# szcompressor/sz

Measured on AMD Instinct MI355X. Metric: compression GB/s (input), 512^3 float32 ABS 1e-4, higher is better.
Workload: dtype f32

## Files before the change

### include/szhip.h

```cpp
#ifndef SZHIP_H
#define SZHIP_H
#include <stddef.h>
#include <stdint.h>
#ifdef __cplusplus
extern "C" {
#endif

#define SZHIP_OK            0
#define SZHIP_ERR_NODEVICE -1
#define SZHIP_ERR_ARG      -2
#define SZHIP_ERR_UNSUP    -3
#define SZHIP_ERR_STREAM   -4
#define SZHIP_ERR_INTERNAL -5
#define SZHIP_CONSTANT      1

#define SZHIP_F32 0
#define SZHIP_F64 1

typedef struct szhip_ctx szhip_ctx;

typedef struct szhip_params {
    int      sample_distance;
    float    pred_threshold;
    unsigned max_quant_intervals;
    unsigned quantization_intervals;
    unsigned flags;
} szhip_params;
#define SZHIP_RANGE_FROM_DATA 1u

typedef struct szhip_stats {
    double ms_total;
    double ms_prequant;
    double ms_quant;
    double ms_entropy;
    double ms_host;
    uint64_t n_elements, n_blocks, n_reg_blocks, n_unpred;
    unsigned intervals; int use_mean;
    uint64_t out_bytes;
    uint64_t quant_kernel_launches;
    double vmin, vmax;
    int chain_overlapped;
    int quant_kernel;
    int packing;
    int book_on_device;
} szhip_stats;

int  szhip_create(szhip_ctx **ctx, int device);
typedef struct szhip_pool szhip_pool;
int  szhip_pool_create(szhip_pool **pool, int device, int lanes);
void szhip_pool_destroy(szhip_pool *pool);
int  szhip_pool_submit(szhip_pool *pool, int dtype, const void *data, int data_on_device, size_t r0, size_t r1, size_t r2, double eb,
                       const szhip_params *params, const unsigned char *meta, size_t meta_len, int out_on_device,
                       unsigned char *out_buf, size_t out_cap, int *ticket);
int  szhip_pool_wait(szhip_pool *pool, int ticket, unsigned char **out, size_t *out_size, szhip_stats *stats);

void szhip_destroy(szhip_ctx *ctx);
const char *szhip_last_error(szhip_ctx *ctx);

int szhip_stage_input(szhip_ctx *ctx, const void *host_data, size_t bytes, void **device_ptr);

int szhip_minmax(szhip_ctx *ctx, int dtype, const void *data, int data_on_device, size_t n, double *vmin, double *vmax);

int szhip_compress(szhip_ctx *ctx, int dtype, const void *data, int data_on_device,
                   size_t r0, size_t r1, size_t r2, double eb, const szhip_params *params,
                   const unsigned char *meta, size_t meta_len,
                   int out_on_device, unsigned char **out, size_t *out_size, szhip_stats *stats);

int szhip_decompress(szhip_ctx *ctx, int dtype, const unsigned char *stream, int stream_on_device, size_t stream_len,
                     size_t body_off, size_t r0, size_t r1, size_t r2,
                     void *out, int out_on_device, szhip_stats *stats);

int szhip_compress_sz14(szhip_ctx *ctx, int dtype, const void *data, int data_on_device,
                        size_t r0, size_t r1, size_t r2, double eb, double value_range, double median,
                        const szhip_params *params, const unsigned char *meta, size_t meta_len,
                        int out_on_device, unsigned char **out, size_t *out_size, szhip_stats *stats);
int szhip_decompress_sz14(szhip_ctx *ctx, int dtype, const unsigned char *stream, int stream_on_device, size_t stream_len,
                          size_t body_off, size_t r0, size_t r1, size_t r2, void *out, int out_on_device, szhip_stats *stats);

int szhip_compress_omp(szhip_ctx *ctx, int dtype, const void *data, int data_on_device, size_t r0, size_t r1, size_t r2, double eb,
                       int thread_num, const szhip_params *params, const unsigned char *meta, size_t meta_len,
                       int out_on_device, unsigned char **out, size_t *out_size, szhip_stats *stats);
int szhip_decompress_omp(szhip_ctx *ctx, int dtype, const unsigned char *stream, int stream_on_device, size_t stream_len,
                         size_t body_off, size_t r0, size_t r1, size_t r2, void *out, int out_on_device, szhip_stats *stats);

typedef struct szhip_pwr {
    uint64_t segment_size;
    const unsigned char *signs_blob;
    uint32_t signs_blob_size;
    double min_log_value;
    unsigned char rad_expo;
    unsigned char msst19;
    unsigned char plus_bits;
    double median_stored;
} szhip_pwr;
int szhip_pwr_prepare(szhip_ctx *ctx, int dtype, const void *data, int data_on_device, size_t n, double vmin, double vmax, double pwr_ratio,
                      void **d_log, unsigned char *signs_host, int *positive, double *real_precision, double *value_range, double *median,
                      double *min_log_value);
int szhip_msst_prepare(szhip_ctx *ctx, int dtype, const void *data, int data_on_device, size_t n, double vmax, double pwr_ratio,
                       void **d_prepared, unsigned char *signs_host, int *positive, double *near_zero, double *median_log, double *min_log_value);
int szhip_compress_sz14_pwr(szhip_ctx *ctx, int dtype, const void *data, int data_on_device,
                            size_t r0, size_t r1, size_t r2, double eb, double value_range, double median,
                            const szhip_params *params, const unsigned char *meta, size_t meta_len, const szhip_pwr *pwr,
                            int out_on_device, unsigned char **out, size_t *out_size, szhip_stats *stats);
int szhip_sz14_pwr_locate(int dtype, const unsigned char *stream, size_t stream_len, size_t body_off, size_t *blob_off, size_t *blob_size,
                          double *min_log_value);
int szhip_decompress_sz14_pwr(szhip_ctx *ctx, int dtype, const unsigned char *stream, int stream_on_device, size_t stream_len,
                              size_t body_off, size_t r0, size_t r1, size_t r2, const unsigned char *signs_host, void *out,
                              int out_on_device, szhip_stats *stats);

typedef struct szhip_book_record {
// ... 17 lines not shown
```

### sz_amd/api.py

```python
import ctypes
import os
import subprocess

import numpy as np

ABS, REL, VR_REL, ABS_AND_REL, ABS_OR_REL, PSNR, NORM, PW_REL = 0, 1, 1, 2, 3, 4, 5, 10
SZ_FLOAT, SZ_DOUBLE = 0, 1
SZ_BEST_SPEED, SZ_BEST_COMPRESSION, SZ_DEFAULT_COMPRESSION = 0, 1, 2
SZ_SCES, SZ_NSCS = 0, -1

_HERE = os.path.dirname(os.path.abspath(__file__))
_CSRC = os.path.join(_HERE, "csrc")


def lib_path():
    return os.environ.get("SZ_AMD_LIB") or os.path.join(_CSRC, "libszhip.so")


class SZError(RuntimeError):
    pass


class sz_params(ctypes.Structure):
    _fields_ = [("dataType", ctypes.c_int), ("max_quant_intervals", ctypes.c_uint),
# ... 29 lines not shown
class szhip_book_record(ctypes.Structure):
    _fields_ = [("n_nodes", ctypes.c_uint32), ("tree_bytes", ctypes.c_uint32), ("max_len", ctypes.c_uint32), ("status", ctypes.c_uint32),
                ("total_bits", ctypes.c_uint64), ("total_unpred", ctypes.c_uint64)]


class szhost_meta(ctypes.Structure):
    _fields_ = [("data_type", ctypes.c_int), ("err_mode", ctypes.c_int), ("abs_bound", ctypes.c_double),
                ("rel_ratio", ctypes.c_double), ("psnr", ctypes.c_double), ("pwr_ratio", ctypes.c_double), ("vmin", ctypes.c_double),
                ("vmax", ctypes.c_double), ("opt_quant_mode", ctypes.c_int), ("data_endian", ctypes.c_int),
                ("sz_mode", ctypes.c_int), ("gzip_mode", ctypes.c_int), ("sample_distance", ctypes.c_int),
                ("pred_threshold", ctypes.c_float), ("sol_id", ctypes.c_int), ("max_quant_intervals", ctypes.c_uint),
                ("quantization_intervals", ctypes.c_uint), ("protect_value_range", ctypes.c_int)]


def build_library(force=False):
    if force:
        subprocess.check_call(["make", "-s", "-C", _CSRC, "clean"])
    subprocess.check_call(["make", "-s", "-C", _CSRC])
    return lib_path()


_lib = None


def lib():
    global _lib
    if _lib is not None:
        return _lib
    p = lib_path()
    if not os.path.exists(p):
        raise SZError(f"{p} is missing: build it with `python -c 'import __graft_entry__ as g; g.build()'` "
                      "(hipcc --offload-arch=gfx950); there is no CPU fallback")
    _lib = _bind(ctypes.CDLL(p))
    return _lib


def _bind(L):
    sz = ctypes.c_size_t
    L.SZ_Init.argtypes = [ctypes.c_char_p]; L.SZ_Init.restype = ctypes.c_int
    L.SZ_Init_Params.argtypes = [ctypes.POINTER(sz_params)]; L.SZ_Init_Params.restype = ctypes.c_int
    L.SZ_Finalize.argtypes = []; L.SZ_Finalize.restype = None
    L.SZ_compress.argtypes = [ctypes.c_int, ctypes.c_void_p, ctypes.POINTER(sz)] + [sz] * 5
    L.SZ_compress.restype = ctypes.c_void_p
    L.SZ_compress_args.argtypes = [ctypes.c_int, ctypes.c_void_p, ctypes.POINTER(sz), ctypes.c_int,
                                   ctypes.c_double, ctypes.c_double, ctypes.c_double] + [sz] * 5
    L.SZ_compress_args.restype = ctypes.c_void_p
    L.SZ_decompress.argtypes = [ctypes.c_int, ctypes.c_void_p, sz] + [sz] * 5
    L.SZ_decompress.restype = ctypes.c_void_p
    L.SZ_hip_last_stats.argtypes = [ctypes.POINTER(szhip_stats)]; L.SZ_hip_last_stats.restype = ctypes.c_int
    L.SZ_hip_set_device.argtypes = [ctypes.c_int]
    L.szhip_create.argtypes = [ctypes.POINTER(ctypes.c_void_p), ctypes.c_int]; L.szhip_create.restype = ctypes.c_int
    L.szhip_destroy.argtypes = [ctypes.c_void_p]; L.szhip_destroy.restype = None
    L.szhip_last_error.argtypes = [ctypes.c_void_p]; L.szhip_last_error.restype = ctypes.c_char_p
    L.szhip_minmax.argtypes = [ctypes.c_void_p, ctypes.c_int, ctypes.c_void_p, ctypes.c_int, sz,
                               ctypes.POINTER(ctypes.c_double), ctypes.POINTER(ctypes.c_double)]
    L.szhip_minmax.restype = ctypes.c_int
    L.szhip_compress.argtypes = [ctypes.c_void_p, ctypes.c_int, ctypes.c_void_p, ctypes.c_int, sz, sz, sz, ctypes.c_double,
                                 ctypes.POINTER(szhip_params), ctypes.c_char_p, sz, ctypes.c_int,
                                 ctypes.POINTER(ctypes.c_void_p), ctypes.POINTER(sz), ctypes.POINTER(szhip_stats)]
    L.szhip_compress.restype = ctypes.c_int
    if hasattr(L, "szhip_pool_create"):
        L.szhip_pool_create.argtypes = [ctypes.POINTER(ctypes.c_void_p), ctypes.c_int, ctypes.c_int]; L.szhip_pool_create.restype = ctypes.c_int
        L.szhip_pool_destroy.argtypes = [ctypes.c_void_p]; L.szhip_pool_destroy.restype = None
        L.szhip_pool_submit.argtypes = [ctypes.c_void_p, ctypes.c_int, ctypes.c_void_p, ctypes.c_int, sz, sz, sz, ctypes.c_double,
                                        ctypes.POINTER(szhip_params), ctypes.c_char_p, sz, ctypes.c_int, ctypes.c_void_p, sz, ctypes.POINTER(ctypes.c_int)]
        L.szhip_pool_submit.restype = ctypes.c_int
        L.szhip_pool_wait.argtypes = [ctypes.c_void_p, ctypes.c_int, ctypes.POINTER(ctypes.c_void_p), ctypes.POINTER(sz), ctypes.POINTER(szhip_stats)]
        L.szhip_pool_wait.restype = ctypes.c_int
    L.szhip_decompress.argtypes = [ctypes.c_void_p, ctypes.c_int, ctypes.c_void_p, ctypes.c_int, sz, sz, sz, sz, sz,
                                   ctypes.c_void_p, ctypes.c_int, ctypes.POINTER(szhip_stats)]
    L.szhip_decompress.restype = ctypes.c_int
    L.szhip_compress_sz14.argtypes = [ctypes.c_void_p, ctypes.c_int, ctypes.c_void_p, ctypes.c_int, sz, sz, sz, ctypes.c_double,
                                      ctypes.c_double, ctypes.c_double, ctypes.POINTER(szhip_params), ctypes.c_char_p, sz, ctypes.c_int,
                                      ctypes.POINTER(ctypes.c_void_p), ctypes.POINTER(sz), ctypes.POINTER(szhip_stats)]
    L.szhip_compress_sz14.restype = ctypes.c_int
    L.szhip_decompress_sz14.argtypes = [ctypes.c_void_p, ctypes.c_int, ctypes.c_void_p, ctypes.c_int, sz, sz, sz, sz, sz,
                                        ctypes.c_void_p, ctypes.c_int, ctypes.POINTER(szhip_stats)]
    L.szhip_decompress_sz14.restype = ctypes.c_int
    L.szhip_debug_fetch.argtypes = [ctypes.c_void_p, ctypes.c_int, ctypes.c_void_p, sz]; L.szhip_debug_fetch.restype = ctypes.c_int
    if hasattr(L, "szhip_compress_omp"):
        L.szhip_compress_omp.argtypes = [ctypes.c_void_p, ctypes.c_int, ctypes.c_void_p, ctypes.c_int, sz, sz, sz, ctypes.c_double, ctypes.c_int,
                                         ctypes.POINTER(szhip_params), ctypes.c_char_p, sz, ctypes.c_int,
                                         ctypes.POINTER(ctypes.c_void_p), ctypes.POINTER(sz), ctypes.POINTER(szhip_stats)]
        L.szhip_compress_omp.restype = ctypes.c_int
        L.szhip_decompress_omp.argtypes = [ctypes.c_void_p, ctypes.c_int, ctypes.c_void_p, ctypes.c_int, sz, sz, sz, sz, sz,
                                           ctypes.c_void_p, ctypes.c_int, ctypes.POINTER(szhip_stats)]
        L.szhip_decompress_omp.restype = ctypes.c_int
    if hasattr(L, "szhip_huff_book"):
        L.szhip_huff_book.argtypes = [ctypes.c_void_p, ctypes.c_void_p, ctypes.c_uint, ctypes.c_void_p, sz, ctypes.c_void_p, ctypes.c_void_p,
                                      ctypes.POINTER(szhip_book_record)]
        L.szhip_huff_book.restype = ctypes.c_int
    L.szhost_write_meta.argtypes = [ctypes.POINTER(szhost_meta), ctypes.c_ubyte, ctypes.c_char_p]
    L.szhost_write_meta.restype = sz
    L.free.argtypes = [ctypes.c_void_p]
    return L


def _dims5(shape):
    d = list(shape)[::-1] + [0] * (5 - len(shape))
    return d[4], d[3], d[2], d[1], d[0]


def _dtype_code(a):
    if a.dtype == np.float32:
        return SZ_FLOAT
    if a.dtype == np.float64:
# ... 105 lines not shown
        if self._h:
            lib().szhip_pool_destroy(self._h)
            self._h = ctypes.c_void_p()

    def __del__(self):
        try:
            self.close()
        except Exception:
            pass

    def submit(self, ptr, on_device, shape3, dtype, eb, meta, params, out_ptr, out_cap):
        t = ctypes.c_int(-1)
        p = params or szhip_params(100, 0.99, 65536, 0)
        rc = lib().szhip_pool_submit(self._h, 0 if np.dtype(dtype) == np.float32 else 1, ptr, int(on_device), shape3[0], shape3[1], shape3[2], eb,
                                     ctypes.byref(p), meta, len(meta), 2, out_ptr, out_cap, ctypes.byref(t))
        if rc != 0:
            raise SZError(f"szhip_pool_submit failed ({rc})")
        self._keep[t.value] = (p, meta)
        return t.value

    def wait(self, ticket):
        out = ctypes.c_void_p(); n = ctypes.c_size_t(0); st = szhip_stats()
        rc = lib().szhip_pool_wait(self._h, ticket, ctypes.byref(out), ctypes.byref(n), ctypes.byref(st))
        self._keep.pop(ticket, None)
        if rc == 1:
            return 0, st
        if rc != 0:
            raise SZError(f"pooled szhip_compress failed ({rc})")
        return n.value, st


class HipContext:

    def __init__(self, device=0):
        self._h = ctypes.c_void_p()
        rc = lib().szhip_create(ctypes.byref(self._h), device)
        if rc != 0:
            raise SZError(f"szhip_create failed ({rc}): no usable HIP device; there is no CPU fallback")

    def close(self):
        if self._h:
            lib().szhip_destroy(self._h)
            self._h = ctypes.c_void_p()

    def __del__(self):
        try:
            self.close()
        except Exception:
            pass

    def _err(self, rc, what):
        raise SZError(f"{what} failed ({rc}): {lib().szhip_last_error(self._h).decode(errors='replace')}")

    def minmax(self, ptr, on_device, n, dtype):
        lo, hi = ctypes.c_double(), ctypes.c_double()
        rc = lib().szhip_minmax(self._h, 0 if np.dtype(dtype) == np.float32 else 1, ptr, int(on_device), n,
                                ctypes.byref(lo), ctypes.byref(hi))
        if rc:
            self._err(rc, "szhip_minmax")
        return lo.value, hi.value

    def compress(self, ptr, on_device, shape3, dtype, eb, meta, params=None, out_on_device=False):
        p = params or szhip_params(100, 0.99, 65536, 0)
        out = ctypes.c_void_p()
        n = ctypes.c_size_t(0)
        st = szhip_stats()
        rc = lib().szhip_compress(self._h, 0 if np.dtype(dtype) == np.float32 else 1, ptr, int(on_device), shape3[0], shape3[1],
                                  shape3[2], eb, ctypes.byref(p), meta, len(meta), int(out_on_device), ctypes.byref(out),
                                  ctypes.byref(n), ctypes.byref(st))
        if rc == 1:
            return None, 0, st
        if rc:
            self._err(rc, "szhip_compress")
        if out_on_device:
            return out.value, n.value, st
        b = ctypes.string_at(out.value, n.value)
        lib().free(out)
        return b, n.value, st

    def compress_omp(self, ptr, on_device, shape3, dtype, eb, thread_num, meta, params=None, out_on_device=False):
        p = params or szhip_params(100, 0.99, 65536, 0)
        out = ctypes.c_void_p()
        n = ctypes.c_size_t(0)
        st = szhip_stats()
        rc = lib().szhip_compress_omp(self._h, 0 if np.dtype(dtype) == np.float32 else 1, ptr, int(on_device), shape3[0], shape3[1], shape3[2],
                                      eb, thread_num, ctypes.byref(p), meta, len(meta), int(out_on_device), ctypes.byref(out), ctypes.byref(n),
                                      ctypes.byref(st))
        if rc:
            self._err(rc, "szhip_compress_omp")
        if out_on_device:
            return out.value, n.value, st
        b = ctypes.string_at(out.value, n.value)
        lib().free(out)
        return b, n.value, st

    def decompress_omp(self, stream_ptr, stream_on_device, stream_len, body_off, shape3, dtype, out_ptr, out_on_device):
        st = szhip_stats()
        rc = lib().szhip_decompress_omp(self._h, 0 if np.dtype(dtype) == np.float32 else 1, stream_ptr, int(stream_on_device), stream_len,
                                        body_off, shape3[0], shape3[1], shape3[2], out_ptr, int(out_on_device), ctypes.byref(st))
        if rc:
            self._err(rc, "szhip_decompress_omp")
        return st

    def huff_book(self, hist, on_device=False, intervals=None, tree_cap=None):
        if on_device:
            ptr, k = hist, int(intervals)
# ... 26 lines not shown
```

### sz_amd/csrc/szhip.hip

```cpp
#include <hip/hip_runtime.h>
#include <algorithm>
#include <array>
#include <cmath>
#include <cstdio>
#include <cstdlib>
#include <cstring>
#include <atomic>
#include <chrono>
#include <ctime>
#include <condition_variable>
#include <deque>
#include <functional>
#include <mutex>
#include <thread>
#include <vector>
#include "../../include/szhip.h"
#include "szhost.h"
#include "szhip_kernels.h"

namespace {

struct DevBuf { void *p = nullptr; size_t cap = 0; };

double now_ms()
// ... 62 lines not shown
    void arm() { { std::lock_guard<std::mutex> lk(m); if (phase.load() == 0) phase.store(1); } cv.notify_all(); }
    void disarm() { std::lock_guard<std::mutex> lk(m); if (phase.load() == 1) phase.store(0); }
    void submit(int ncoef, std::function<void(int)> c, std::function<void(int)> sec)
    {
        n = ncoef; chain = std::move(c); section = std::move(sec);
        stage1.store(0); stage2.store(0);
        arm();
        seq.fetch_add(1, std::memory_order_release);
    }
    void wait_chains() { while (stage1.load(std::memory_order_acquire) < n) pause(); }
    void wait_all() { while (stage2.load(std::memory_order_acquire) < 4) std::this_thread::yield(); }
    ~szhip_chain_pool()
    {
        { std::lock_guard<std::mutex> lk(m); phase.store(2); }
        cv.notify_all();
        for (auto &t : th) if (t.joinable()) t.join();
    }
};

constexpr int SZH_STAGE_T = 4;
struct szhip_ctx {
    int device = 0;
    int cus = 256;
    hipStream_t stream = nullptr;
    hipStream_t stream2 = nullptr;
    hipEvent_t ev_in = nullptr, ev_fit = nullptr, ev_feed = nullptr, ev_sec = nullptr;
    int settle_probes = 0, settle_rejected = 0;
    hipStream_t stream3 = nullptr;
    hipEvent_t ev_perm = nullptr;
    hipEvent_t ev[6] = {nullptr, nullptr, nullptr, nullptr, nullptr, nullptr};
    char err[512] = {0};
    unsigned epoch = 0;
    bool hdec_sync_rounds = false, hdec_unconverged = false;
    bool gate = false;
    unsigned long long *hdec_res = nullptr;
    DevBuf lor_bits, reg_flags, reg_rank, coef_compact, in, out, codes_nat, codes_blk, coef, blk_lor, faceI, faceJ, rb_down, rb_right, rb_vals, pt_flags, feed_word, progress, order, small, hist, col_zeros, col_zeros64,
        seg_bits, seg_zeros, seg_bitoff, seg_zoff, seg_hist, seg_tab, col_off, partial, samples, unpred, stream_buf, chunk_bits, chunk_off, code_tab, len_tab, dec_tab,
        starts, ends, counts, offs, dirty, zcnt, zpos, pwr_log, pwr_signs, pwr_small, coef_dec, msst_ptab, msst_cells, msst_rec, msst_pe, book_tree, book_rec, book_stage;
    void *pinned = nullptr; size_t pinned_cap = 0;
    void *pinned2 = nullptr; size_t pinned2_cap = 0;
    void *stage_buf[SZH_STAGE_T][2] = {};
    hipEvent_t stage_ev[SZH_STAGE_T][2] = {};
    void *pinned3 = nullptr; size_t pinned3_cap = 0;
    int streams_independent = -1;
    void *coh = nullptr; size_t coh_cap = 0;
    int order_nI = -1, order_nJ = -1;
    bool wave_timeout = false, ticket_atomic = false;
    bool coef_late = false, no_chain_overlap = false;
    bool book_declined = false, no_dev_book = false;
    unsigned long long *book_pin = nullptr;
    std::vector<int> chain_codes; std::vector<unsigned char> chain_unpred;
    unsigned char *sec_pin[4] = {nullptr, nullptr, nullptr, nullptr}; size_t sec_pin_cap[4] = {0, 0, 0, 0};
    szhip_chain_pool *chain_pool = nullptr;
};

namespace {

#include "szhip_rt.inc"
#include "szhip_sz21.inc"
#include "szhip_sz14.inc"
#include "szhip_pwr.inc"
#include "szhip_omp.inc"

}

template <class F>
static int with_ticket_fallback(szhip_ctx *ctx, F &&run)
{
    ctx->wave_timeout = false; ctx->hdec_unconverged = false; ctx->coef_late = false; ctx->book_declined = false;
    auto again = [&]() {
        if (ctx->stream3) hipStreamSynchronize(ctx->stream3); hipStreamSynchronize(ctx->stream2); hipStreamSynchronize(ctx->stream);
        return run();
    };
    int rc = run();
    if (rc == SZHIP_ERR_INTERNAL && ctx->book_declined && !ctx->no_dev_book) {
        ctx->no_dev_book = true; ctx->wave_timeout = false; rc = again(); ctx->no_dev_book = false;
    }
    if (rc == SZHIP_OK && !ctx->no_chain_overlap && tune_int("SZ_HIP_TEST_CHAIN_FALLBACK", 0)) { ctx->coef_late = true; rc = SZHIP_ERR_INTERNAL; }
    if (rc == SZHIP_ERR_INTERNAL && ctx->coef_late && !ctx->no_chain_overlap) {
        ctx->no_chain_overlap = true; ctx->wave_timeout = false; rc = again();
    }
    if (rc == SZHIP_ERR_INTERNAL && ctx->hdec_unconverged && !ctx->hdec_sync_rounds) {
        ctx->hdec_sync_rounds = true; ctx->wave_timeout = false; rc = again(); ctx->hdec_sync_rounds = false;
    }
    if (rc == SZHIP_OK && !ctx->ticket_atomic && tune_int("SZ_HIP_TEST_TICKET_FALLBACK", 0)) { ctx->wave_timeout = true; rc = SZHIP_ERR_INTERNAL; }
    if (rc == SZHIP_ERR_INTERNAL && ctx->wave_timeout && !ctx->ticket_atomic) {
        ctx->ticket_atomic = true; rc = again();
    }
    return rc;
}


extern "C" {


static int create_ctx(szhip_ctx **out, int device)
{
    if (!out) return SZHIP_ERR_ARG;
    int count = 0;
    hipError_t e = hipGetDeviceCount(&count);
    if (e != hipSuccess || count <= 0) {
        fprintf(stderr, "szhip: no HIP device available (%s); this library has no CPU fallback\n", hipGetErrorString(e));
        return SZHIP_ERR_NODEVICE;
    }
    if (device < 0 || device >= count) return SZHIP_ERR_ARG;
    szhip_ctx *ctx = new szhip_ctx();
    ctx->device = device;
    { int c = 0; if (hipDeviceGetAttribute(&c, hipDeviceAttributeMultiprocessorCount, device) == hipSuccess && c > 0) ctx->cus = c; }
    if (hipSetDevice(device) != hipSuccess || hipStreamCreateWithFlags(&ctx->stream, hipStreamNonBlocking) != hipSuccess) {
        delete ctx; return SZHIP_ERR_NODEVICE;
    }
    for (int i = 0; i < 6; ++i) if (hipEventCreate(&ctx->ev[i]) != hipSuccess) { delete ctx; return SZHIP_ERR_NODEVICE; }
    if (hipStreamCreateWithFlags(&ctx->stream2, hipStreamNonBlocking) != hipSuccess || hipEventCreateWithFlags(&ctx->ev_in, hipEventDisableTiming) != hipSuccess ||
        hipEventCreateWithFlags(&ctx->ev_fit, hipEventDisableTiming) != hipSuccess ||
        hipEventCreateWithFlags(&ctx->ev_feed, hipEventDisableTiming) != hipSuccess ||
        hipEventCreateWithFlags(&ctx->ev_sec, hipEventDisableTiming) != hipSuccess) { delete ctx; return SZHIP_ERR_NODEVICE; }
    *out = ctx;
    return SZHIP_OK;
}

int szhip_create(szhip_ctx **out, int device)
{
    const int rc = create_ctx(out, device);
    if (rc == SZHIP_OK) settle_streams(*out, nullptr, 0);
    return rc;
}

void szhip_destroy(szhip_ctx *ctx)
{
    if (!ctx) return;
    hipSetDevice(ctx->device);
    hipStreamSynchronize(ctx->stream);
    delete ctx->chain_pool; ctx->chain_pool = nullptr;
    DevBuf *bufs[] = {&ctx->lor_bits, &ctx->reg_flags, &ctx->reg_rank, &ctx->coef_compact, &ctx->in, &ctx->out, &ctx->codes_nat, &ctx->codes_blk, &ctx->coef, &ctx->blk_lor, &ctx->faceI, &ctx->faceJ, &ctx->rb_down, &ctx->rb_right, &ctx->rb_vals, &ctx->pt_flags, &ctx->feed_word, &ctx->progress,
                      &ctx->order, &ctx->small, &ctx->hist, &ctx->col_zeros, &ctx->col_zeros64, &ctx->seg_bits, &ctx->seg_zeros, &ctx->seg_bitoff, &ctx->seg_zoff, &ctx->seg_hist, &ctx->seg_tab, &ctx->col_off, &ctx->partial,
                      &ctx->samples, &ctx->unpred, &ctx->stream_buf, &ctx->chunk_bits, &ctx->chunk_off, &ctx->code_tab,
                      &ctx->len_tab, &ctx->dec_tab, &ctx->starts, &ctx->ends, &ctx->counts, &ctx->offs, &ctx->dirty, &ctx->zcnt, &ctx->zpos,
                      &ctx->pwr_log, &ctx->pwr_signs, &ctx->pwr_small, &ctx->coef_dec, &ctx->msst_ptab, &ctx->msst_cells, &ctx->msst_rec, &ctx->msst_pe, &ctx->book_tree, &ctx->book_rec, &ctx->book_stage};
    for (DevBuf *b : bufs) if (b->p) hipFree(b->p);
    if (ctx->pinned) hipHostFree(ctx->pinned);
    if (ctx->pinned2) hipHostFree(ctx->pinned2);
    if (ctx->pinned3) hipHostFree(ctx->pinned3);
    if (ctx->coh) hipHostFree(ctx->coh);
    if (ctx->hdec_res) hipHostFree(ctx->hdec_res);
    if (ctx->book_pin) hipHostFree(ctx->book_pin);
    for (int w = 0; w < SZH_STAGE_T; ++w) for (int k = 0; k < 2; ++k) { if (ctx->stage_buf[w][k]) hipHostFree(ctx->stage_buf[w][k]); if (ctx->stage_ev[w][k]) hipEventDestroy(ctx->stage_ev[w][k]); }
    for (int i = 0; i < 6; ++i) if (ctx->ev[i]) hipEventDestroy(ctx->ev[i]);
    if (ctx->ev_in) hipEventDestroy(ctx->ev_in);
    if (ctx->ev_fit) hipEventDestroy(ctx->ev_fit);
    if (ctx->ev_feed) hipEventDestroy(ctx->ev_feed);
    if (ctx->ev_sec) hipEventDestroy(ctx->ev_sec);
    for (int e = 0; e < 4; ++e) if (ctx->sec_pin[e]) hipHostFree(ctx->sec_pin[e]);
    if (ctx->stream2) hipStreamDestroy(ctx->stream2);
    if (ctx->stream3) hipStreamDestroy(ctx->stream3);
    if (ctx->ev_perm) hipEventDestroy(ctx->ev_perm);
    if (ctx->stream) hipStreamDestroy(ctx->stream);
    delete ctx;
}

const char *szhip_last_error(szhip_ctx *ctx) { return ctx ? ctx->err : "no context"; }

struct szhip_pool_job {
    int dtype; const void *data; int on_dev; size_t r0, r1, r2; double eb; szhip_params prm; const unsigned char *meta; size_t meta_len;
    int out_on_device; unsigned char *out; size_t out_size; szhip_stats stats; int rc; bool done;
};
struct szhip_pool {
    std::vector<szhip_ctx *> ctx;
    std::vector<std::thread> workers;
    std::mutex mu;
    std::condition_variable cv_work, cv_done;
    std::deque<int> queue;
    std::vector<szhip_pool_job> jobs;
    std::vector<bool> used;
    bool stop = false;
};
static void szhip_pool_worker(szhip_pool *p, int lane)
{
    for (;;) {
        int t;
        {
            std::unique_lock<std::mutex> lk(p->mu);
            p->cv_work.wait(lk, [&] { return p->stop || !p->queue.empty(); });
            if (p->queue.empty()) return;
            t = p->queue.front(); p->queue.pop_front();
        }
        szhip_pool_job &j = p->jobs[t];
        j.rc = szhip_compress(p->ctx[lane], j.dtype, j.data, j.on_dev, j.r0, j.r1, j.r2, j.eb, &j.prm, j.meta, j.meta_len, j.out_on_device,
                              &j.out, &j.out_size, &j.stats);
        { std::lock_guard<std::mutex> lk(p->mu); j.done = true; }
        p->cv_done.notify_all();
    }
}
int szhip_pool_create(szhip_pool **out, int device, int lanes)
{
    if (!out || lanes < 1 || lanes > 16) return SZHIP_ERR_ARG;
    szhip_pool *p = new szhip_pool();
    for (int i = 0; i < lanes; ++i) {
        szhip_ctx *c = nullptr;
        const int rc = create_ctx(&c, device);
        if (rc != SZHIP_OK) { for (szhip_ctx *x : p->ctx) szhip_destroy(x); delete p; return rc; }
        c->gate = lanes > 1;
        { std::vector<hipStream_t> mains; for (szhip_ctx *x : p->ctx) { mains.push_back(x->stream); mains.push_back(x->stream2); } settle_streams(c, mains.data(), (int)mains.size(), lanes == 1); }
        p->ctx.push_back(c);
    }
    p->jobs.resize(64); p->used.assign(64, false);
    for (int i = 0; i < lanes; ++i) p->workers.emplace_back(szhip_pool_worker, p, i);
    *out = p;
    return SZHIP_OK;
}
void szhip_pool_destroy(szhip_pool *p)
{
    if (!p) return;
    { std::lock_guard<std::mutex> lk(p->mu); p->stop = true; }
// ... 268 lines not shown
```

### sz_amd/csrc/szhip_kernels.h

```cpp
#pragma once
#include <hip/hip_runtime.h>
#include "szh_core.h"
#include "szh_pencil.h"
#include "szh_bufio.h"

typedef unsigned long long u64;

#ifdef SZH_HIPSIM
#define SZH_DYN_SMEM(name) char *name = hipsim_dyn_smem()
#else
#define SZH_DYN_SMEM(name) extern __shared__ __attribute__((aligned(16))) char name[]
#endif

__device__ __forceinline__ u64 ord_enc(float v)
{
    unsigned u = __float_as_uint(v);
    u = (u & 0x80000000u) ? ~u : (u | 0x80000000u);
    return (u64)u;
}
__device__ __forceinline__ u64 ord_enc(double v)
{
    u64 u = (u64)__double_as_longlong(v);
    u = (u & 0x8000000000000000ull) ? ~u : (u | 0x8000000000000000ull);
    return u;
// ... 210 lines not shown
            if (I < a.nI && J < a.nJ) szh_pencil_run<T, DEC, B, MS>(a, I, J, L);
        } else if (w == NP) szh_tile_store<T, B>(a, TI, TJ, L);
        else szh_tile_fill<T, B>(a, TI, TJ, L);
        if (!a.persist) break;
    }
}

template <class T> struct GlobAcc {
    const T *p; int64_t d0, d1;
    __device__ T operator()(int i, int j, int k) const { return p[i * d0 + j * d1 + k]; }
    __device__ T operator()(int j, int k) const { return p[j * d1 + k]; }
};

template <class T>
__global__ __launch_bounds__(256) void k_fit_select(szh_geom3 G, const T *__restrict__ data, T *coef, uint8_t *blk_lor,
                                                    T noise, int use_mean, T mean, u64 *minmax)
{
    __shared__ u64 red[8];
    const int lane = threadIdx.x & 63, wid = threadIdx.x >> 6;
    const int64_t b = (int64_t)blockIdx.x * 256 + threadIdx.x;
    u64 lmin = ~0ull, lmax = 0ull;
    if (b < G.nblocks) {
        const int nb2 = G.g2.num, nb1 = G.g1.num;
        const int b2 = (int)(b % nb2);
        const int64_t c = b / nb2;
        const int b1 = (int)(c % nb1), b0 = (int)(c / nb1);
        const int s0 = szh_blk_size(G.g0, b0), s1 = szh_blk_size(G.g1, b1), s2 = szh_blk_size(G.g2, b2);
        const GlobAcc<T> A{data + (int64_t)szh_blk_start(G.g0, b0) * G.d0 + (int64_t)szh_blk_start(G.g1, b1) * G.d1 + szh_blk_start(G.g2, b2),
                           G.d0, G.d1};
        T c4[4];
        auto range = [&](T v) { const u64 oe = ord_enc(v); const bool num = v == v; lmin = num && oe < lmin ? oe : lmin; lmax = num && oe > lmax ? oe : lmax; };
        int reg;
        if (G.ndim == 2) {
            c4[0] = 0;
            szh_fit_block_2d<T>(A, s1, s2, c4 + 1, range);
            reg = szh_select_block_2d<T>(A, s1, s2, c4 + 1, noise);
        } else {
            szh_fit_block<T>(A, s0, s1, s2, c4, range);
            reg = szh_select_block<T>(A, s0, s1, s2, c4, noise, use_mean, mean);
        }
        for (int e = 0; e < 4; ++e) coef[(int64_t)e * G.nblocks + b] = c4[e];
        blk_lor[b] = reg ? 0 : 1;
    }
    lmin = wave_min_u64(lmin); lmax = wave_max_u64(lmax);
    if (lane == 0) { red[wid] = lmin; red[4 + wid] = lmax; }
    __syncthreads();
    if (threadIdx.x == 0) {
        u64 mn = red[0], mx = red[4];
        for (int w = 1; w < 4; ++w) { mn = red[w] < mn ? red[w] : mn; mx = red[4 + w] > mx ? red[4 + w] : mx; }
        atomicMin(&minmax[0], mn); atomicMax(&minmax[1], mx);
    }
}

template <class T>
__global__ __launch_bounds__(256) void k_minmax(const T *__restrict__ data, int64_t n, u64 *minmax)
{
    __shared__ u64 red[8];
    u64 lmin = ~0ull, lmax = 0ull;
    for (int64_t i = (int64_t)blockIdx.x * 256 + threadIdx.x; i < n; i += (int64_t)gridDim.x * 256) {
        const T v = data[i]; const u64 e = ord_enc(v); const bool num = v == v;
        lmin = num && e < lmin ? e : lmin; lmax = num && e > lmax ? e : lmax;
    }
    lmin = wave_min_u64(lmin); lmax = wave_max_u64(lmax);
    if ((threadIdx.x & 63) == 0) { red[threadIdx.x >> 6] = lmin; red[4 + (threadIdx.x >> 6)] = lmax; }
    __syncthreads();
    if (threadIdx.x == 0) {
        u64 mn = red[0], mx = red[4];
        for (int w = 1; w < 4; ++w) { mn = red[w] < mn ? red[w] : mn; mx = red[4 + w] > mx ? red[4 + w] : mx; }
        atomicMin(&minmax[0], mn); atomicMax(&minmax[1], mx);
    }
}

template <class T>
__global__ __launch_bounds__(256) void k_gather_mean(const T *__restrict__ data, szh_meanwalk w, int64_t count, T *out)
{
    const int64_t m = (int64_t)blockIdx.x * 256 + threadIdx.x;
    if (m < count) out[m] = data[szh_meanwalk_pos(w, m)];
}

#define SZH_LDS_RADIUS_BINS 4096
template <class T, bool FREQ>
__global__ __launch_bounds__(256) void k_sample(szh_geom3 G, const T *__restrict__ data, int64_t nrows, int sd, double ebD, T mean,
                                                unsigned max_radius, unsigned *radius_hist, unsigned *freq_hist, u64 *within)
{
    __shared__ unsigned sh_r[SZH_LDS_RADIUS_BINS];
    __shared__ unsigned sh_f[FREQ ? 8192 : 1];
    for (int i = threadIdx.x; i < SZH_LDS_RADIUS_BINS; i += 256) sh_r[i] = 0;
    if (FREQ) for (int i = threadIdx.x; i < 8192; i += 256) sh_f[i] = 0;
    __syncthreads();
    const int64_t rpp = G.g1.count - 1, r2 = G.g2.count;
    const bool two_d = G.ndim == 2;
    unsigned w = 0;
    for (int64_t ridx = (int64_t)blockIdx.x * 256 + threadIdx.x; ridx < nrows; ridx += (int64_t)gridDim.x * 256) {
        const int64_t n1 = two_d ? 0 : ridx / rpp + 1, n2 = two_d ? ridx + 1 : ridx - (n1 - 1) * rpp + 1;
        const int64_t c0 = two_d ? szh_sample_col0_2d(n2, sd) : sd - ((n1 + n2) % sd);
        const int64_t origin = n1 * G.d0 + n2 * r2;
        for (int64_t m = 0;; ++m) {
            const int64_t col = c0 + m * sd;
            if (m > 0 && col >= r2) break;
            const int64_t pos = origin + col;
            if (pos >= G.n) break;
            unsigned ri; int fi, we;
            szh_sample_point<T>(data, pos, r2, two_d ? 0 : G.d0, ebD, mean, max_radius, &ri, &fi, &we);
            if (ri < SZH_LDS_RADIUS_BINS) atomicAdd(&sh_r[ri], 1u); else atomicAdd(&radius_hist[ri], 1u);
            if (FREQ) atomicAdd(&sh_f[fi], 1u);
            w += (unsigned)we;
// ... 1152 lines not shown
```

### sz_amd/csrc/szhip_rt.inc

```

#define HIPCHK(call)                                                                                   \
    do {                                                                                               \
        hipError_t e_ = (call);                                                                        \
        if (e_ != hipSuccess) {                                                                        \
            snprintf(ctx->err, sizeof(ctx->err), "%s failed: %s (%s:%d)", #call, hipGetErrorString(e_), __FILE__, __LINE__); \
            fprintf(stderr, "szhip: %s\n", ctx->err);                                                  \
            return SZHIP_ERR_NODEVICE;                                                                 \
        }                                                                                              \
    } while (0)

#define FAIL(code, ...)                                                                                \
    do {                                                                                               \
        snprintf(ctx->err, sizeof(ctx->err), __VA_ARGS__);                                             \
        fprintf(stderr, "szhip: %s\n", ctx->err);                                                      \
        return (code);                                                                                 \
    } while (0)
#define FAIL_PUBLISHED(code, ...)                                                                      \
    do {                                                                                               \
        if (!out_on_device && out && *out) { free(*out); *out = nullptr; }                              \
        if (out_size) *out_size = 0;                                                                   \
        FAIL(code, __VA_ARGS__);                                                                       \
    } while (0)

int ensure(szhip_ctx *ctx, DevBuf &b, size_t bytes, bool zero_new = false)
{
    if (bytes == 0) bytes = 16;
    if (b.cap >= bytes) return SZHIP_OK;
    if (b.p) { HIPCHK(hipStreamSynchronize(ctx->stream)); HIPCHK(hipFree(b.p)); b.p = nullptr; b.cap = 0; }
    size_t cap = bytes + bytes / 8 + 256;
    HIPCHK(hipMalloc(&b.p, cap));
    b.cap = cap;
    if (zero_new) HIPCHK(hipMemsetAsync(b.p, 0, cap, ctx->stream));
    return SZHIP_OK;
}

#define TRY(x) do { int rc_ = (x); if (rc_ != SZHIP_OK) return rc_; } while (0)

int ensure_host(szhip_ctx *ctx, void *&p, size_t &have, size_t bytes, hipStream_t user, unsigned flags = hipHostMallocDefault)
{
    if (have >= bytes) return SZHIP_OK;
    if (p) { HIPCHK(hipStreamSynchronize(user)); HIPCHK(hipHostFree(p)); p = nullptr; have = 0; }
    size_t cap = bytes + bytes / 4 + 4096;
    HIPCHK(hipHostMalloc(&p, cap, flags));
    have = cap;
    return SZHIP_OK;
}
int ensure_pinned(szhip_ctx *ctx, size_t bytes) { return ensure_host(ctx, ctx->pinned, ctx->pinned_cap, bytes, ctx->stream); }
int ensure_pinned2(szhip_ctx *ctx, size_t bytes) { return ensure_host(ctx, ctx->pinned2, ctx->pinned2_cap, bytes, ctx->stream2); }
int ensure_pinned3(szhip_ctx *ctx, size_t bytes) { return ensure_host(ctx, ctx->pinned3, ctx->pinned3_cap, bytes, ctx->stream); }
int ensure_coherent(szhip_ctx *ctx, size_t bytes)
{
    const size_t had = ctx->coh_cap;
    TRY(ensure_host(ctx, ctx->coh, ctx->coh_cap, bytes, ctx->stream, hipHostMallocCoherent | hipHostMallocMapped));
    if (ctx->coh_cap != had) memset(ctx->coh, 0, ctx->coh_cap);
    return SZHIP_OK;
}

enum { SM_MINMAX = 0, SM_WITHIN = 2, SM_MEANCNT = 3, SM_TOTAL_UNPRED = 4, SM_TOTAL_BITS = 5, SM_TICKET = 6, SM_ERR = 7,
       SM_CHANGED = 8, SM_MEANSUM = 9, SM_TOTAL_SYM = 10, SM_NREG = 11, SM_SCRATCH = 12, SM_COUNT = 16 };

int probe_streams(szhip_ctx *ctx)
{
    if (ctx->streams_independent >= 0) return SZHIP_OK;
    TRY(ensure_coherent(ctx, 256));
    TRY(ensure(ctx, ctx->small, SM_COUNT * 8));
    volatile unsigned long long *flag = (volatile unsigned long long *)((char *)ctx->coh + 128);
    unsigned long long *src = (unsigned long long *)((char *)ctx->coh + 192);
    *flag = 0; *src = 1;
    HIPCHK(hipStreamSynchronize(ctx->stream)); HIPCHK(hipStreamSynchronize(ctx->stream2));
    u64 *sm = (u64 *)ctx->small.p;
    hipLaunchKernelGGL(k_probe_wait, dim3(1), dim3(1), 0, ctx->stream, (const unsigned long long *)flag, (unsigned long long *)(sm + SM_SCRATCH));
    HIPCHK(hipGetLastError());
    HIPCHK(hipMemcpyAsync(sm + SM_SCRATCH + 1, src, 8, hipMemcpyHostToDevice, ctx->stream2));
    const double t0 = now_ms();
    HIPCHK(hipStreamSynchronize(ctx->stream2));
    const double waited = now_ms() - t0;
    *flag = 1;
    HIPCHK(hipStreamSynchronize(ctx->stream));
    ctx->streams_independent = waited < 2.0 ? 1 : 0;
    return SZHIP_OK;
}

static int probe_pair(szhip_ctx *ctx, hipStream_t a, hipStream_t b, int *shared)
{
    TRY(ensure_coherent(ctx, 256));
    TRY(ensure(ctx, ctx->small, SM_COUNT * 8));
    volatile unsigned long long *flag = (volatile unsigned long long *)((char *)ctx->coh + 128);
    *flag = 0;
    HIPCHK(hipStreamSynchronize(a)); HIPCHK(hipStreamSynchronize(b));
    u64 *sm = (u64 *)ctx->small.p;
    hipLaunchKernelGGL(k_probe_wait, dim3(1), dim3(1), 0, a, (const unsigned long long *)flag, (unsigned long long *)(sm + SM_SCRATCH));
    HIPCHK(hipGetLastError());
    hipLaunchKernelGGL(k_probe_touch, dim3(1), dim3(1), 0, b, (unsigned long long *)(sm + SM_SCRATCH + 1));
    HIPCHK(hipGetLastError());
// ... 62 lines not shown
    HIPCHK(hipStreamSynchronize(st));
    const size_t nchunks = (bytes + chunk - 1) / chunk;
    std::atomic<int> failed(0);
    const int device = ctx->device;
    auto worker = [&](int w) {
        if (hipSetDevice(device) != hipSuccess) { failed = 1; return; }
        size_t pend_off[2] = {0, 0}, pend_len[2] = {0, 0};
        bool pend[2] = {false, false};
        int k = 0;
        for (size_t c = (size_t)w; c < nchunks && !failed; c += (size_t)nthr, k ^= 1) {
            const size_t off = c * chunk, len = std::min(chunk, bytes - off);
            if (to_device) {
                if (pend[k] && hipEventSynchronize(ctx->stage_ev[w][k]) != hipSuccess) { failed = 1; return; }
                memcpy(ctx->stage_buf[w][k], (const char *)src + off, len);
                if (hipMemcpyAsync((char *)dst + off, ctx->stage_buf[w][k], len, hipMemcpyHostToDevice, st) != hipSuccess ||
                    hipEventRecord(ctx->stage_ev[w][k], st) != hipSuccess) { failed = 1; return; }
                pend[k] = true;
            } else {
                if (pend[k]) {
                    if (hipEventSynchronize(ctx->stage_ev[w][k]) != hipSuccess) { failed = 1; return; }
                    memcpy((char *)dst + pend_off[k], ctx->stage_buf[w][k], pend_len[k]);
                }
                if (hipMemcpyAsync(ctx->stage_buf[w][k], (const char *)src + off, len, hipMemcpyDeviceToHost, st) != hipSuccess ||
                    hipEventRecord(ctx->stage_ev[w][k], st) != hipSuccess) { failed = 1; return; }
                pend[k] = true; pend_off[k] = off; pend_len[k] = len;
            }
        }
        for (int q = 0; q < 2; ++q, k ^= 1) {
            if (!pend[k]) continue;
            if (hipEventSynchronize(ctx->stage_ev[w][k]) != hipSuccess) { failed = 1; return; }
            if (!to_device) memcpy((char *)dst + pend_off[k], ctx->stage_buf[w][k], pend_len[k]);
        }
    };
    std::vector<std::thread> th;
    for (int w = 1; w < nthr; ++w) th.emplace_back(worker, w);
    worker(0);
    for (auto &t : th) t.join();
    if (failed) FAIL(SZHIP_ERR_NODEVICE, "staged %s copy failed", to_device ? "host-to-device" : "device-to-host");
    return SZHIP_OK;
}

int tune_int(const char *name, int def)
{
    const char *e = getenv(name);
    return e ? atoi(e) : def;
}

int scan_u64(szhip_ctx *ctx, const u64 *in, int64_t n, u64 *out, u64 *total_dev, hipStream_t on = nullptr)
{
    const hipStream_t sst = on ? on : ctx->stream;
    const int64_t nblk = (n + SZH_SCAN_TILE - 1) / SZH_SCAN_TILE;
    TRY(ensure(ctx, ctx->partial, (size_t)(nblk + 1) * 8));
    u64 *partial = (u64 *)ctx->partial.p;
    hipLaunchKernelGGL(k_scan_partials, dim3((unsigned)nblk), dim3(256), 0, sst, in, n, partial);
    hipLaunchKernelGGL(k_scan_single, dim3(1), dim3(256), 0, sst, partial, nblk, total_dev);
    hipLaunchKernelGGL(k_scan_final, dim3((unsigned)nblk), dim3(256), 0, sst, in, n, (const u64 *)partial, out);
    HIPCHK(hipGetLastError());
    return SZHIP_OK;
}

constexpr size_t SZH_PERM_TILE_BYTES = 32 * 1024;
int choose_segb(const szh_geom3 &G, size_t elem, size_t budget)
{
    const size_t rows = (size_t)G.g0.early * G.g1.early;
    size_t per_block = rows * (size_t)G.g2.early * elem;
    int segb = (int)(budget / (per_block ? per_block : 1));
    if (segb < 1) segb = 1;
    if (segb > 32) segb = 32;
    if (segb > G.g2.num) segb = G.g2.num;
    return segb;
}
size_t tile_bytes(const szh_geom3 &G, int segb, size_t elem)
{
    const size_t rows = (size_t)G.g0.early * G.g1.early;
    const size_t kp = ((size_t)segb * G.g2.early + 31) & ~(size_t)7;
    return rows * kp * elem + 16;
}

int prepare_pencil(szhip_ctx *ctx, const szh_geom3 &G, int nw, int tpi, int tpj, int *nI_out, int *nJ_out, int *ntiles_out)
{
    const int nI = (G.g0.count + 7) / 8, nJ = (G.g1.count + 7) / 8;
    if (nI > 65535 || nJ > 65535) FAIL(SZHIP_ERR_UNSUP, "dimension too large for the pencil grid");
    const size_t rowg = (size_t)G.g2.count * nw * sizeof(u64);
    TRY(ensure(ctx, ctx->faceI, (size_t)nI * nJ * 9 * rowg + 64, true));
    TRY(ensure(ctx, ctx->faceJ, (size_t)nI * nJ * 8 * rowg + 64, true));
    TRY(ensure(ctx, ctx->progress, (size_t)nI * nJ * 2 * sizeof(u64), true));
    const int nTI = (nI + tpi - 1) / tpi, nTJ = (nJ + tpj - 1) / tpj;
    if (ctx->order_nI != nTI || ctx->order_nJ != nTJ) {
        std::vector<unsigned> ord((size_t)nTI * nTJ);
        szh_fill_pencil_order(nTI, nTJ, ord.data());
        TRY(ensure(ctx, ctx->order, ord.size() * 4));
        HIPCHK(hipMemcpyAsync(ctx->order.p, ord.data(), ord.size() * 4, hipMemcpyHostToDevice, ctx->stream));
        HIPCHK(hipStreamSynchronize(ctx->stream));
        ctx->order_nI = nTI; ctx->order_nJ = nTJ;
    }
    *nI_out = nI; *nJ_out = nJ; *ntiles_out = nTI * nTJ;
    return SZHIP_OK;
}

constexpr int SZH_FILL_BACKOFF = 4;
template <class T> static int pencil_wide(const szh_geom3 &G, int nJ)
{
    using TS = szh_tile_shape<T>;
    return (double)TS::TPI * nJ * 9.0 * (double)G.g2.count * szh_gran<T>::NW * 8.0 < 4.0e9 && (double)TS::TPJ * 9.0 * (double)G.g2.count * szh_gran<T>::NW * 8.0 < 4.0e9;
}
template <class QA> static unsigned pencil_grid(szhip_ctx *ctx, QA &a, int ntiles)
{
    const int cap = ctx->gate ? 512 : 0;
    a.persist = cap > 0 && cap < ntiles;
    return (unsigned)(a.persist ? cap : ntiles);
}
template <class T> bool beam_applies(const szh_geom3 &G, const void *base, size_t reg_count)
{
    if (!tune_int("SZ_HIP_BEAM", 1)) return false;
    (void)reg_count;
    if (G.ndim != 3) return false;
    if (G.g2.count < 4 || (G.g2.count & 3) != 0 || ((uintptr_t)base & 15) != 0) return false;
    if ((double)G.n * sizeof(T) >= 4.0e9) return false;
    const szh_bm::grid_t g = szh_bm::make_grid(G);
    if (g.nKB > 65535 || g.nJG > 65535) return false;
    return (double)szh_bm::kface_words<T>(G) * 8.0 < 4.0e9 && (double)szh_bm::jface_words<T>(G) * 8.0 < 4.0e9;
}
template <class T, bool DEC>
int launch_beam(szhip_ctx *ctx, const szh_geom3 &G, szh_qargs<T> a, hipStream_t st, size_t reg_count, bool feed = false)
{
    const szh_bm::grid_t g = szh_bm::make_grid(G);
    const size_t tiles = (size_t)g.nKB * g.nJG;
    TRY(ensure(ctx, ctx->rb_down, szh_bm::kface_words<T>(G) * sizeof(u64) + 64, true));
    TRY(ensure(ctx, ctx->rb_right, szh_bm::jface_words<T>(G) * sizeof(u64) + 64, true));
    a.faceI = (szh_u64 *)ctx->rb_down.p; a.faceJ = (szh_u64 *)ctx->rb_right.p;
    a.nI = g.nKB; a.nJ = g.nJG;
    if (a.ticket_mode == 2) a.ticket_mode = 1;
    if (ctx->gate) a.ticket_mode = 0;
#ifdef SZH_SYNC_LAUNCH
    const unsigned wgs = (unsigned)tiles;
#else
    const int per_cu = sizeof(T) == 4 ? 2 : 1;
    const unsigned wgs = (unsigned)std::min<size_t>(tiles, (size_t)ctx->cus * per_cu);
#endif
    const bool hasreg = reg_count != 0;
    if (hasreg) {
        TRY(ensure(ctx, ctx->pt_flags, (size_t)G.n + 64));
#ifdef SZH_SYNC_LAUNCH
        const bool prepared = feed;
#else
        const bool prepared = false;
#endif
        if (!prepared) HIPCHK(hipMemsetAsync(ctx->pt_flags.p, 0, (size_t)G.n, st));
        a.ptflags = (const uint8_t *)ctx->pt_flags.p;
        const unsigned rgrid = (unsigned)(G.g0.num * G.g1.num);
        if (!DEC) {
            TRY(ensure(ctx, ctx->rb_vals, (size_t)G.n * sizeof(T) + 64));
            a.xr = (const T *)ctx->rb_vals.p;
            if (feed) {
                TRY(ensure(ctx, ctx->feed_word, 256));
                if (!prepared) HIPCHK(hipMemsetAsync(ctx->feed_word.p, 0, 256, st));
                a.reg_ready = (const unsigned *)ctx->feed_word.p;
                HIPCHK(hipEventRecord(ctx->ev_feed, st));
                HIPCHK(hipStreamWaitEvent(ctx->stream2, ctx->ev_feed, 0));
            } else
            hipLaunchKernelGGL((k_reg_points<T, 0>), dim3(rgrid), dim3(256), 0, st, G, a.blk_lor, a.coef, a.coef_stride, a.data, (T *)ctx->rb_vals.p, a.codes, (uint8_t *)ctx->pt_flags.p,
                               a.eb, a.recip, a.cap, a.radius, 0);
        } else
            hipLaunchKernelGGL((k_reg_points<T, 2>), dim3(rgrid), dim3(256), 0, st, G, a.blk_lor, a.coef, a.coef_stride, (const T *)nullptr, a.out, a.codes, (uint8_t *)ctx->pt_flags.p,
                               a.eb, a.recip, a.cap, a.radius, 0);
        HIPCHK(hipGetLastError());
    }
    const dim3 grid(wgs), block(szh_bm::WPG * 64);
    if (hasreg) {
        if (a.use_mean) hipLaunchKernelGGL((k_beam<T, DEC, true, true>), grid, block, 0, st, a);
        else hipLaunchKernelGGL((k_beam<T, DEC, false, true>), grid, block, 0, st, a);
    } else {
        if (a.use_mean) hipLaunchKernelGGL((k_beam<T, DEC, true, false>), grid, block, 0, st, a);
        else hipLaunchKernelGGL((k_beam<T, DEC, false, false>), grid, block, 0, st, a);
    }
    HIPCHK(hipGetLastError());
    return SZHIP_OK;
}

template <class T>
int feed_beam_slice(szhip_ctx *ctx, const szh_geom3 &G, const szh_qargs<T> &a, hipStream_t s2, const T *hcoef, size_t reg_count, size_t r_lo, size_t r_hi,
                    int b0_lo, int b0_hi, int planes_end, const u64 *reg_rank, int64_t nb)
{
    if (r_hi > r_lo)
        for (int e = 0; e < 4; ++e)
            HIPCHK(hipMemcpyAsync((T *)ctx->coef_compact.p + (size_t)e * reg_count + r_lo, hcoef + (size_t)e * reg_count + r_lo, (r_hi - r_lo) * sizeof(T), hipMemcpyHostToDevice, s2));
    const int64_t blk_lo = (int64_t)b0_lo * G.g1.num * G.g2.num, blk_hi = std::min<int64_t>(nb, (int64_t)b0_hi * G.g1.num * G.g2.num);
    if (r_hi > r_lo && blk_hi > blk_lo) {
        hipLaunchKernelGGL((k_move_coef<T, 1>), dim3((unsigned)((nb + 255) / 256)), dim3(256), 0, s2, a.blk_lor, reg_rank, nb, (int64_t)reg_count, (T *)a.coef, (T *)ctx->coef_compact.p);
        hipLaunchKernelGGL((k_reg_points<T, 0>), dim3((unsigned)((b0_hi - b0_lo) * G.g1.num)), dim3(256), 0, s2, G, a.blk_lor, a.coef, a.coef_stride, a.data, (T *)ctx->rb_vals.p,
                           a.codes, (uint8_t *)ctx->pt_flags.p, a.eb, a.recip, a.cap, a.radius, b0_lo);
    }
    hipLaunchKernelGGL(k_store_u32, dim3(1), dim3(1), 0, s2, (unsigned *)ctx->feed_word.p, (unsigned)planes_end);
    HIPCHK(hipGetLastError());
    return SZHIP_OK;
}

template <class T> double ord_dec(u64 e);
template <> double ord_dec<float>(u64 e)
{
    unsigned u = (unsigned)e;
    u = (u & 0x80000000u) ? (u & 0x7fffffffu) : ~u;
    float f; memcpy(&f, &u, 4); return (double)f;
}
template <> double ord_dec<double>(u64 e)
{
    u64 u = (e & 0x8000000000000000ull) ? (e & 0x7fffffffffffffffull) : ~e;
    double d; memcpy(&d, &u, 8); return d;
}

template <class T>
int minmax_impl(szhip_ctx *ctx, const void *data, int on_dev, size_t n, double *vmin, double *vmax)
{
    const T *d_in = (const T *)data;
    if (!on_dev) {
        TRY(ensure(ctx, ctx->in, n * sizeof(T)));
        HIPCHK(hipMemcpyAsync(ctx->in.p, data, n * sizeof(T), hipMemcpyHostToDevice, ctx->stream));
        d_in = (const T *)ctx->in.p;
    }
    TRY(ensure(ctx, ctx->small, SM_COUNT * 8));
    u64 *sm = (u64 *)ctx->small.p;
    u64 init[2] = {~0ull, 0ull};
    HIPCHK(hipMemcpyAsync(sm + SM_MINMAX, init, 16, hipMemcpyHostToDevice, ctx->stream));
    int grid = (int)std::min<int64_t>(((int64_t)n + 255) / 256, 2048);
    hipLaunchKernelGGL((k_minmax<T>), dim3(grid), dim3(256), 0, ctx->stream, d_in, (int64_t)n, sm + SM_MINMAX);
    HIPCHK(hipGetLastError());
    u64 res[2];
    HIPCHK(hipMemcpyAsync(res, sm + SM_MINMAX, 16, hipMemcpyDeviceToHost, ctx->stream));
    HIPCHK(hipStreamSynchronize(ctx->stream));
    *vmin = ord_dec<T>(res[0]); *vmax = ord_dec<T>(res[1]);
    return SZHIP_OK;
}
```

### sz_amd/csrc/szhip_sz21.inc

```
static bool book_declines(unsigned rec_status, unsigned long long plan_status, int test_switch) { return rec_status != 0 || plan_status != 0 || test_switch != 0; }

static int hist_rshift(unsigned intervals, size_t cap_bins) { int r = 0; while (r < 6 && ((size_t)intervals << (r + 1)) <= cap_bins) ++r; return r; }

struct sz21_plan {
    bool use_beam = false;
    bool segenc = false;
    bool seghist = false;
    bool dev_book = false;
    bool sliced = false;
    int slices_req = 1;
    int se_vw = 1, se_segb = 0, se_nseg = 0, se_nrmax = szh_se::NR; size_t se_tile = 0;
    int sh_rshift = 0;
    bool revise(unsigned enc_maxlen) { if (!segenc || enc_maxlen <= 32) return false; segenc = false; seghist = false; return true; }
};
template <class T>
sz21_plan sz21_make_plan(const szhip_ctx *ctx, const szh_geom3 &G, unsigned intervals, size_t reg_count, bool beam_ok, bool overlap, bool feed, size_t meta_len)
{
    sz21_plan P;
    const int64_t n = G.n;
    P.use_beam = !overlap && beam_ok;
    const int segenc_sw = tune_int("SZ_HIP_SEGENC", 1);
    P.segenc = G.ndim == 3 && segenc_sw != 0 && (!feed || segenc_sw == 2);
    P.se_vw = (G.g2.count % 8) == 0 ? 8 : ((G.g2.count % 4) == 0 ? 4 : 1);
    if (P.segenc) {
        bool ok = intervals < 65536 && (double)n < 4.0e9;
        if ((int64_t)G.g0.late * G.g1.late * G.g2.late < 32) ok = false;
        const size_t fixed = ((size_t)intervals + 1) * 8 + 16 + szh_se::seg_window_words(G, 32) * 4 + 64;
        const size_t lds_cap = (size_t)63 * 1024, want = (size_t)std::max(4, tune_int("SZ_HIP_SEG_TILE_KB", 14)) * 1024;
        if (ok && fixed + szh_se::seg_tile_bytes(G, 1, P.se_vw) > lds_cap) ok = false;
        if (ok) {
            const size_t budget = std::min(lds_cap - fixed, std::max(want, szh_se::seg_tile_bytes(G, 1, P.se_vw)));
            int sb = 1;
            while (sb < G.g2.num && szh_se::seg_tile_bytes(G, sb + 1, P.se_vw) <= budget && szh_se::seg_pieces_per_thread(G, sb + 1, P.se_vw) <= (size_t)szh_se::PF) ++sb;
            sb = (G.g2.num + (G.g2.num + sb - 1) / sb - 1) / ((G.g2.num + sb - 1) / sb);
            if (const int f = tune_int("SZ_HIP_SEG_SEGB", 0)) sb = std::max(1, std::min(f, sb));
            P.se_segb = sb;
            P.se_nseg = (G.g2.num + sb - 1) / sb;
            P.se_tile = szh_se::seg_tile_bytes(G, sb, P.se_vw);
            const int rows_typ = (2 * G.g0.split > G.g0.num ? G.g0.early : G.g0.late) * (2 * G.g1.split > G.g1.num ? G.g1.early : G.g1.late);
            const int runs_typ = std::max(1, sb * rows_typ), rounds_typ = (runs_typ + 256 * szh_se::NR - 1) / (256 * szh_se::NR);
            P.se_nrmax = std::max(1, std::min(szh_se::NR, (runs_typ + 256 * rounds_typ - 1) / (256 * rounds_typ)));
            if ((double)G.g0.num * G.g1.num >= 2.0e9) ok = false;
        }
        P.segenc = ok;
    }
    P.seghist = P.segenc && intervals <= SZH_COL_HBINS && tune_int("SZ_HIP_SEGHIST", 1) != 0;
    if (P.seghist) P.sh_rshift = hist_rshift(intervals, 4096);
    P.dev_book = P.segenc && reg_count == 0 && !ctx->no_dev_book && tune_int("SZ_HIP_DEV_BOOK", 0) != 0 && G.g0.num * G.g1.num <= 1024 * SZH_COL_SCAN_PER &&
                 tune_int("SZ_HIP_SEG_SCAN1", 1) != 0 && meta_len + 8 + 4 + sizeof(T) + 1 + sizeof(T) <= 3072;
    P.slices_req = tune_int("SZ_HIP_SLICES", ctx->gate ? tune_int("SZ_HIP_SLICES_POOL", 2) : 4);
    P.sliced = P.use_beam && P.slices_req > 1 && !P.seghist;
    return P;
}

template <class T>
struct sz21_call {
    static constexpr int is_double = sizeof(T) == 8;
    static constexpr int64_t LINE = 128 / (int64_t)sizeof(T);
    szhip_ctx *const ctx; const szhip_params *const prm; const unsigned char *meta; const size_t meta_len; const int out_on_device; unsigned char **const out; size_t *const out_size;
    const double eb_in; const T eb; const hipStream_t st;
    const bool two_d;
    const szh_geom3 G; const int ncoef, ncols; const int64_t n, nb;
    const double t_begin = now_ms(); double host_ms = 0;
    const int tp_on = tune_int("SZ_HIP_TIMING", 0); double tp_t[32]; const char *tp_n[32]; int tp_k = 0;
    szhip_stats S;
    const T *d_in = nullptr; u64 *sm = nullptr; T *d_coef = nullptr; uint8_t *d_lor = nullptr; uint16_t *d_nat = nullptr, *d_blk = nullptr; unsigned *d_hist = nullptr, *h_hist = nullptr;
    T noise = 0; bool fit_tile = false; int ft_nseg = 0;
    size_t ind_bytes = 0; unsigned char *ind_bits = nullptr; u64 *nreg_h = nullptr, *minmax_h = nullptr;
    unsigned intervals = 0; int use_mean = 0; T mean = 0; size_t reg_count = 0;
    std::vector<unsigned char> meta_own;
    sz21_plan P;
    unsigned *tile_done = nullptr; size_t beam_words = 0;
    int perm_segb = 1, perm_nseg = 1; size_t perm_lds = 0;
    std::vector<szh_se::seg_t> se_segs; std::vector<u64> tab_code; std::vector<uint8_t> tab_len;
    unsigned enc_maxlen = 0; bool enc32 = false; size_t lds_e32 = 0;
    unsigned char *hdr = nullptr; size_t pre_len = 0, sections_total = 0, hdr_len = 0, unpred_bytes = 0, total_len = 0; u64 total_bits = 0, total_unpred = 0;
    u64 h_small[SM_COUNT];
    bool synced = false;
    szhost_coeffs cf;
    size_t sec_len[4] = {0, 0, 0, 0};
    std::vector<std::thread> section_threads;
    std::atomic<int> section_failed{0};
    std::vector<unsigned char> all_reg_keep;
    std::vector<uint32_t> blk_of_rank;
    size_t chain_done[4] = {0, 0, 0, 0};
    size_t chain_avail = 0;
    double chain_t0[4] = {0, 0, 0, 0}, chain_t1[4] = {0, 0, 0, 0};
    bool overlap = false, feed = false, two_pieces = false;
    fed_call_guard fed_guard;
    T *hcoef = nullptr;
    bool pool_busy = false;
    bool cf_own = false;
    sz21_call(szhip_ctx *c, size_t r0, size_t r1, size_t r2, double eb_, const szhip_params *p, const unsigned char *m, size_t ml, int ood, unsigned char **o, size_t *os)
        : ctx(c), prm(p), meta(m), meta_len(ml), out_on_device(ood), out(o), out_size(os), eb_in(eb_), eb((T)eb_), st(c->stream), two_d(r0 == 0),
          G(r0 == 0 ? szh_make_geom2((int)r1, (int)r2) : szh_make_geom3((int)r0, (int)r1, (int)r2)), ncoef(r0 == 0 ? 3 : 4), ncols(G.g0.num * G.g1.num), n(G.n), nb(G.nblocks)
    {
        memset(&S, 0, sizeof(S)); memset(&cf, 0, sizeof(cf));
        S.n_elements = (uint64_t)n; S.n_blocks = (uint64_t)nb;
    }
    ~sz21_call() {
        join_sections();
        if (ctx->chain_pool) ctx->chain_pool->disarm();
        if (cf_own) for (int e = 0; e < 4; ++e) { cf.codes[e] = nullptr; cf.unpred[e] = nullptr; }
        szhost_coeffs_free(&cf);
    }
    void join_sections() {
        for (auto &x : section_threads) if (x.joinable()) x.join();
        if (pool_busy && ctx->chain_pool) { ctx->chain_pool->wait_all(); pool_busy = false; }
    }
    void TP(const char *nm) { if (tp_on && tp_k < 32) { tp_t[tp_k] = now_ms() - t_begin; tp_n[tp_k++] = nm; } }
    void print_trace() const { if (tp_on) { for (int i = 0; i < tp_k; ++i) fprintf(stderr, "%s %.2f | ", tp_n[i], tp_t[i]); fprintf(stderr, "\n"); } }
    bool is_lorenzo(int64_t bb) const { return (ind_bits[bb >> 3] >> (7 - (bb & 7))) & 1; }
    size_t count_lorenzo(int64_t bb, int64_t b_end) const {
        size_t ones = 0;
        for (; bb < b_end && (bb & 7); ++bb) ones += is_lorenzo(bb);
        for (; bb + 64 <= b_end; bb += 64) { uint64_t w8; memcpy(&w8, ind_bits + (bb >> 3), 8); ones += (size_t)__builtin_popcountll(w8); }
        for (; bb < b_end; ++bb) ones += is_lorenzo(bb);
        return ones;
    }
    size_t chains_done() const {
        size_t p = reg_count;
        for (int e = 0; e < ncoef; ++e) { const size_t d = __atomic_load_n(&chain_done[e], __ATOMIC_ACQUIRE); if (d < p) p = d; }
        return p;
    }
    int launch_fit(hipStream_t s_, int um, T mn) {
        if (fit_tile) hipLaunchKernelGGL((k_fit_tile<T>), dim3((unsigned)((int64_t)ncols * ft_nseg)), dim3(64), 0, s_, G, d_in, d_coef, d_lor, noise, um, mn, sm + SM_MINMAX, ft_nseg);
        else hipLaunchKernelGGL((k_fit_select<T>), dim3((unsigned)((nb + 255) / 256)), dim3(256), 0, s_, G, d_in, d_coef, d_lor, noise, um, mn, sm + SM_MINMAX);
        HIPCHK(hipGetLastError());
        return SZHIP_OK;
    }
    int launch_pack_lor(hipStream_t s_) {
        hipLaunchKernelGGL(k_pack_lor, dim3((unsigned)((ind_bytes + 255) / 256)), dim3(256), 0, s_, (const uint8_t *)d_lor, nb, (uint8_t *)ctx->lor_bits.p, sm + SM_NREG);
        HIPCHK(hipGetLastError());
        HIPCHK(hipMemcpyAsync(ind_bits, ctx->lor_bits.p, ind_bytes, hipMemcpyDeviceToHost, s_));
        HIPCHK(hipMemcpyAsync(nreg_h, sm + SM_NREG, 8, hipMemcpyDeviceToHost, s_));
        return SZHIP_OK;
    }
    int stage_and_fit(const void *data, int data_on_device) {
        d_in = (const T *)data;
        if (!data_on_device) {
            TRY(ensure(ctx, ctx->in, (size_t)n * sizeof(T)));
            TRY(staged_copy(ctx, ctx->in.p, data, (size_t)n * sizeof(T), true));
            d_in = (const T *)ctx->in.p;
        }
        TRY(ensure(ctx, ctx->small, SM_COUNT * 8));
        sm = (u64 *)ctx->small.p;
        HIPCHK(hipMemsetAsync(sm, 0, SM_COUNT * 8, st));
        static const u64 minmax_init[2] = {~0ull, 0ull};
        HIPCHK(hipMemcpyAsync(sm + SM_MINMAX, minmax_init, 16, hipMemcpyHostToDevice, st));
        TRY(ensure(ctx, ctx->coef, (size_t)nb * 4 * sizeof(T)));
        TRY(ensure(ctx, ctx->blk_lor, (size_t)nb));
        d_coef = (T *)ctx->coef.p;
        d_lor = (uint8_t *)ctx->blk_lor.p;
        HIPCHK(hipEventRecord(ctx->ev[0], st));
        TP("ev0");
        HIPCHK(hipEventRecord(ctx->ev_in, st));
        HIPCHK(hipStreamWaitEvent(ctx->stream2, ctx->ev_in, 0));
        noise = (T)((double)eb * (two_d ? 0.81 : 1.22));
        fit_tile = !two_d && szh_ft::applies<T>(G, d_in) && tune_int("SZ_HIP_FIT_TILE", 0) != 0;
        ft_nseg = (G.g2.num + szh_ft::shape<T>::SEGB - 1) / szh_ft::shape<T>::SEGB;
        TRY(launch_fit(ctx->stream2, 0, (T)0));
        ind_bytes = ((size_t)nb + 7) / 8;
        TRY(ensure(ctx, ctx->lor_bits, ind_bytes + 8));
        TRY(ensure_pinned2(ctx, ind_bytes + 32));
        ind_bits = (unsigned char *)ctx->pinned2 + 32;
        nreg_h = (u64 *)ctx->pinned2;
        minmax_h = (u64 *)ctx->pinned2 + 2;
        TRY(launch_pack_lor(ctx->stream2));
        HIPCHK(hipMemcpyAsync(minmax_h, sm + SM_MINMAX, 16, hipMemcpyDeviceToHost, ctx->stream2));
        HIPCHK(hipEventRecord(ctx->ev_fit, ctx->stream2));
        return SZHIP_OK;
    }
    int choose_intervals() {
        intervals = prm->quantization_intervals;
        const unsigned max_radius = prm->max_quant_intervals / 2;
        if (intervals == 0) {
            const int64_t md = (int64_t)(int)std::sqrt((double)n);
            const szh_meanwalk w = two_d ? szh_make_meanwalk(n, INT64_MAX / 2, INT64_MAX / 2, md) : szh_make_meanwalk(n, G.d0, G.g2.count, md);
            int64_t M = 0, M_hi = n / std::max<int64_t>(md - 2, 1) + 2;
            while (szh_meanwalk_pos(w, M_hi) < n) M_hi *= 2;
            while (M < M_hi) { int64_t mid = (M + M_hi) / 2; if (szh_meanwalk_pos(w, mid) >= n) M_hi = mid; else M = mid + 1; }
            TRY(ensure(ctx, ctx->samples, (size_t)M * sizeof(T)));
            TRY(ensure_pinned(ctx, std::max<size_t>((size_t)M * sizeof(T), (size_t)(max_radius + 8192) * 4 + 64)));
            hipLaunchKernelGGL((k_gather_mean<T>), dim3((unsigned)((M + 255) / 256)), dim3(256), 0, st, d_in, w, M, (T *)ctx->samples.p);
            HIPCHK(hipGetLastError());
            HIPCHK(hipMemcpyAsync(ctx->pinned, ctx->samples.p, (size_t)M * sizeof(T), hipMemcpyDeviceToHost, st));
            TP("mean enqueued");
            HIPCHK(hipStreamSynchronize(st));
            TP("mean on host");
            double h0 = now_ms();
            const double smean = szhost_seq_mean(is_double, ctx->pinned, (size_t)M);
            host_ms += now_ms() - h0;
            TRY(ensure(ctx, ctx->hist, (size_t)(max_radius + 8192) * 4 + 64));
            unsigned *d_rh = (unsigned *)ctx->hist.p, *d_fh = d_rh + max_radius;
            HIPCHK(hipMemsetAsync(d_rh, 0, (size_t)(max_radius + 8192) * 4, st));
            const int64_t nrows = szh_sample_row_limit(G, prm->sample_distance);
            if (!two_d && (G.g0.count <= 1 || G.g1.count <= 1)) {
                hipLaunchKernelGGL((k_sample_walk<T, true>), dim3(1), dim3(64), 0, st, G, d_in, prm->sample_distance, (double)eb, (T)smean, max_radius, d_rh, d_fh, sm + SM_WITHIN);
                HIPCHK(hipGetLastError());
            } else if (nrows > 0) {
                int grid = (int)std::min<int64_t>((nrows + 255) / 256, 1024);
                hipLaunchKernelGGL((k_sample<T, true>), dim3(grid), dim3(256), 0, st, G, d_in, nrows, prm->sample_distance, (double)eb, (T)smean, max_radius, d_rh, d_fh, sm + SM_WITHIN);
                HIPCHK(hipGetLastError());
            }
            unsigned *s_hist = (unsigned *)ctx->pinned;
            u64 within = 0;
            HIPCHK(hipMemcpyAsync(s_hist, d_rh, (size_t)(max_radius + 8192) * 4, hipMemcpyDeviceToHost, st));
            HIPCHK(hipMemcpyAsync(&within, sm + SM_WITHIN, 8, hipMemcpyDeviceToHost, st));
            TP("sample enqueued");
            HIPCHK(hipStreamSynchronize(st));
            TP("sample on host");
            h0 = now_ms();
            u64 sample_count = 0;
            for (unsigned i = 0; i < max_radius; ++i) sample_count += s_hist[i];
            szhost_decision dec;
            szhost_decide(is_double, s_hist, max_radius, s_hist + max_radius, sample_count, within, prm->pred_threshold, (double)eb, smean, &dec);
            host_ms += now_ms() - h0;
            intervals = dec.intervals; use_mean = two_d ? 0 : dec.use_mean;
            if (use_mean) {
                T *d_sum = (T *)(sm + SM_MEANSUM);
                hipLaunchKernelGGL((k_mean_seq<T>), dim3(1), dim3(64), 0, st, d_in, n, (T)dec.dense_pos, eb, d_sum, sm + SM_MEANCNT);
                HIPCHK(hipGetLastError());
                T hsum = 0; u64 hcnt = 0;
                HIPCHK(hipMemcpyAsync(&hsum, d_sum, sizeof(T), hipMemcpyDeviceToHost, st));
                HIPCHK(hipMemcpyAsync(&hcnt, sm + SM_MEANCNT, 8, hipMemcpyDeviceToHost, st));
                HIPCHK(hipStreamSynchronize(st));
                if (hcnt > 0) mean = hsum / (T)hcnt;
            }
        }
        if (intervals > 65536 || intervals < 4) FAIL(SZHIP_ERR_UNSUP, "quantization interval count %u outside [4,65536]", intervals);
        S.intervals = intervals; S.use_mean = use_mean;
        return SZHIP_OK;
    }
    int join_fit() {
        HIPCHK(hipStreamWaitEvent(st, ctx->ev_fit, 0));
        if (use_mean) {
            TRY(launch_fit(st, use_mean, mean));
            HIPCHK(hipMemsetAsync(sm + SM_NREG, 0, 8, st));
            TRY(launch_pack_lor(st));
            HIPCHK(hipStreamSynchronize(st));
        } else HIPCHK(hipEventSynchronize(ctx->ev_fit));
        TP("fit joined");
        reg_count = (size_t)*nreg_h;
        S.n_reg_blocks = reg_count;
        if (reg_count == 0 && ctx->chain_pool) ctx->chain_pool->disarm();
        meta_own.assign(meta, meta + meta_len);
        if (prm->flags & SZHIP_RANGE_FROM_DATA) {
            if (meta_len < 4 + 20 + 2 * sizeof(T)) FAIL(SZHIP_ERR_ARG, "parameter bytes too short for a range field");
            const T lo = (T)ord_dec<T>(minmax_h[0]), hi = (T)ord_dec<T>(minmax_h[1]);
            const T range = hi - lo, top = lo + range;
            unsigned char *q = meta_own.data() + 4 + 20;
            if (is_double) { szhost_put_f64be(q, (double)lo); szhost_put_f64be(q + 8, (double)top); }
            else { szhost_put_f32be(q, (float)lo); szhost_put_f32be(q + 4, (float)top); }
            S.vmin = (double)lo; S.vmax = (double)hi;
            if ((double)range <= eb_in) {
                HIPCHK(hipStreamSynchronize(ctx->stream2)); HIPCHK(hipStreamSynchronize(st));
                *out = nullptr; *out_size = 0;
                S.ms_total = now_ms() - t_begin;
                return SZHIP_CONSTANT;
            }
        }
        meta = meta_own.data();
        return SZHIP_OK;
    }
    void make_section(int e) {
        std::vector<uint32_t> h32(65536, 0);
        for (size_t i = 0; i < reg_count; ++i) h32[(size_t)cf.codes[e][i]]++;
        szhost_huff *ch = szhost_huff_build(131072, h32.data(), nullptr, 65536);
        if (!ch) { section_failed = 1; return; }
        const size_t tb = szhost_huff_tree_size(ch);
        const size_t enc_cap = (size_t)((ch->total_bits + 7) / 8) + 16;
        if (sizeof(T) + 12 + tb + 8 + enc_cap + 4 + cf.unpred_count[e] * sizeof(T) > ctx->sec_pin_cap[e]) { szhost_huff_free(ch); section_failed = 1; return; }
        unsigned char *const sec0 = ctx->sec_pin[e];
        unsigned char *q = sec0;
        if (is_double) szhost_put_f64be(q, cf.prec[e]); else szhost_put_f32be(q, (float)cf.prec[e]);
        q += sizeof(T);
        szhost_put_u32be(q, 32768); q += 4;
        szhost_put_u32be(q, (uint32_t)tb); q += 4;
        szhost_put_u32be(q, (uint32_t)ch->n_nodes); q += 4;
        szhost_huff_tree_write(ch, q); q += tb;
        const size_t enc = szhost_huff_encode_i32(ch, cf.codes[e], reg_count, q + 8);
        szhost_put_u64be(q, enc); q += 8 + enc;
        szhost_put_u32be(q, (uint32_t)cf.unpred_count[e]); q += 4;
        memcpy(q, cf.unpred[e], cf.unpred_count[e] * sizeof(T)); q += cf.unpred_count[e] * sizeof(T);
        sec_len[e] = (size_t)(q - sec0);
        szhost_huff_free(ch);
    }
    int prepare_chains() {
        for (int e = 0; e < ncoef; ++e) {
            const size_t bound = sizeof(T) + 12 + (13 * 2 * std::min<size_t>(reg_count, 65536) + 16) + 8 + (8 * reg_count + 16) + 4 + reg_count * sizeof(T) + 64;
            if (ctx->sec_pin_cap[e] < bound) {
                HIPCHK(hipStreamSynchronize(ctx->stream2)); HIPCHK(hipStreamSynchronize(st));
                if (ctx->sec_pin[e]) { HIPCHK(hipHostFree(ctx->sec_pin[e])); ctx->sec_pin[e] = nullptr; ctx->sec_pin_cap[e] = 0; }
                HIPCHK(hipHostMalloc((void **)&ctx->sec_pin[e], bound + bound / 8, hipHostMallocDefault));
                ctx->sec_pin_cap[e] = bound + bound / 8;
            }
        }
        TRY(ensure(ctx, ctx->reg_flags, (size_t)nb * 8));
        TRY(ensure(ctx, ctx->reg_rank, (size_t)nb * 8));
        TRY(ensure(ctx, ctx->coef_compact, reg_count * 4 * sizeof(T)));
        hipLaunchKernelGGL(k_reg_flags, dim3((unsigned)((nb + 255) / 256)), dim3(256), 0, st, (const uint8_t *)d_lor, nb, (u64 *)ctx->reg_flags.p);
        TRY(scan_u64(ctx, (const u64 *)ctx->reg_flags.p, nb, (u64 *)ctx->reg_rank.p, sm + SM_SCRATCH));
        hipLaunchKernelGGL((k_move_coef<T, 0>), dim3((unsigned)((nb + 255) / 256)), dim3(256), 0, st, (const uint8_t *)d_lor, (const u64 *)ctx->reg_rank.p, nb, (int64_t)reg_count, d_coef, (T *)ctx->coef_compact.p);
        HIPCHK(hipGetLastError());
#ifndef SZH_SYNC_LAUNCH
        overlap = !beam_applies<T>(G, d_in, reg_count) && !two_d && !ctx->gate && !ctx->no_chain_overlap && g_compress_calls.load() <= 1;
        if (overlap) { TRY(probe_streams(ctx)); overlap = ctx->streams_independent == 1; }
#endif
        feed = beam_applies<T>(G, d_in, reg_count) && !ctx->gate && !ctx->no_chain_overlap && g_compress_calls.load() <= 1 && tune_int("SZ_HIP_BEAM_FEED", 1) &&
               G.g0.num >= 2 && reg_count >= (size_t)tune_int("SZ_HIP_FEED_MIN_REG", 65536);
#ifndef SZH_SYNC_LAUNCH
        feed = feed && (G.d0 % 128) == 0;
        if (feed) { TRY(probe_streams(ctx)); feed = ctx->streams_independent == 1; }
#endif
        if (feed) feed = fed_guard.try_raise();
        TRY(ensure_pinned3(ctx, reg_count * 4 * sizeof(T) + (overlap ? ((size_t)nb + 64) * 4 * sizeof(T) + 256 : 0)));
        hcoef = (T *)ctx->pinned3;
        return SZHIP_OK;
    }
    int run_chains() {
        chain_avail = reg_count;
        struct AvailAll {
            size_t *p; size_t v;
            ~AvailAll() { __atomic_store_n(p, v, __ATOMIC_RELEASE); }
        } avail_all{&chain_avail, reg_count};
        const size_t first_piece = (size_t)std::max(1, tune_int("SZ_HIP_CHAIN_EARLY_PIECE", 32768));
        two_pieces = feed && reg_count >= 4 * first_piece;
        if (two_pieces) {
            for (int e = 0; e < 4; ++e)
                HIPCHK(hipMemcpyAsync(hcoef + (size_t)e * reg_count, (const T *)ctx->coef_compact.p + (size_t)e * reg_count, first_piece * sizeof(T), hipMemcpyDeviceToHost, st));
            HIPCHK(hipEventRecord(ctx->ev_sec, st));
            for (int e = 0; e < 4; ++e)
                HIPCHK(hipMemcpyAsync(hcoef + (size_t)e * reg_count + first_piece, (const T *)ctx->coef_compact.p + (size_t)e * reg_count + first_piece, (reg_count - first_piece) * sizeof(T), hipMemcpyDeviceToHost, st));
            chain_avail = 0;
            HIPCHK(hipEventSynchronize(ctx->ev_sec));
            __atomic_store_n(&chain_avail, first_piece, __ATOMIC_RELEASE);
        } else {
            HIPCHK(hipMemcpyAsync(hcoef, ctx->coef_compact.p, reg_count * 4 * sizeof(T), hipMemcpyDeviceToHost, st));
            HIPCHK(hipStreamSynchronize(st));
        }
        TP("coef on host");
        double h0 = now_ms();
        all_reg_keep.assign(reg_count, 0);
        TP("chain begin");
        const unsigned char *const ind = all_reg_keep.data();
        T *const chain_in = hcoef + (two_d ? reg_count : 0);
        szhost_coeff_chain_begin(is_double, ind, reg_count, (double)eb, G.g0.late, G.g1.late, G.g2.late, ncoef, &cf);
        if (ctx->chain_codes.size() < reg_count * 4) ctx->chain_codes.resize(reg_count * 4 + reg_count / 4);
        if (ctx->chain_unpred.size() < reg_count * 4 * sizeof(T)) ctx->chain_unpred.resize((reg_count * 4 + reg_count / 4) * sizeof(T));
        for (int e = 0; e < 4; ++e) {
            free(cf.codes[e]); free(cf.unpred[e]);
            cf.codes[e] = ctx->chain_codes.data() + (size_t)e * reg_count;
            cf.unpred[e] = ctx->chain_unpred.data() + (size_t)e * reg_count * sizeof(T);
        }
        cf_own = true;
        if (overlap) {
            blk_of_rank.resize(reg_count);
            size_t r = 0;
            for (int64_t bb = 0; bb < nb && r < reg_count; ++bb) if (!is_lorenzo(bb)) blk_of_rank[r++] = (uint32_t)bb;
            if (r != reg_count) FAIL(SZHIP_ERR_INTERNAL, "indicator bits and regression-block count disagree");
            for (int e = 0; e < 4; ++e) chain_done[e] = 0;
            for (int e = 0; e < ncoef; ++e)
                section_threads.emplace_back([this, e, chain_in, ind] {
                    szhost_coeff_chain_one_p(is_double, chain_in, ind, reg_count, use_mean, e, &cf, &chain_done[e]);
                    make_section(e);
                });
        } else {
            if (!ctx->chain_pool) { ctx->chain_pool = new szhip_chain_pool(); ctx->chain_pool->start(); }
            pool_busy = true;
            for (int e = 0; e < 4; ++e) chain_done[e] = feed && e >= ncoef ? reg_count : 0;
            const size_t *const avail_ptr = two_pieces ? &chain_avail : nullptr;
            ctx->chain_pool->submit(ncoef, [this, chain_in, ind, avail_ptr](int e) {
                    chain_t0[e] = now_ms() - t_begin;
                    szhost_coeff_chain_one_pa(is_double, chain_in, ind, reg_count, use_mean, e, &cf, feed ? &chain_done[e] : nullptr, avail_ptr);
                    chain_t1[e] = now_ms() - t_begin;
                }, [this](int e) { make_section(e); });
            if (two_pieces) {
                HIPCHK(hipStreamSynchronize(st));
                __atomic_store_n(&chain_avail, reg_count, __ATOMIC_RELEASE);
            }
            if (!feed) ctx->chain_pool->wait_chains();
        }
        if (!feed) host_ms += now_ms() - h0;
        TP("chain done");
        if (tp_on) fprintf(stderr, "chain threads: %.2f-%.2f %.2f-%.2f %.2f-%.2f %.2f-%.2f | ", chain_t0[0], chain_t1[0], chain_t0[1], chain_t1[1], chain_t0[2], chain_t1[2], chain_t0[3], chain_t1[3]);
        if (!overlap && !feed) {
            HIPCHK(hipMemcpyAsync(ctx->coef_compact.p, hcoef, reg_count * 4 * sizeof(T), hipMemcpyHostToDevice, st));
            hipLaunchKernelGGL((k_move_coef<T, 1>), dim3((unsigned)((nb + 255) / 256)), dim3(256), 0, st, (const uint8_t *)d_lor, (const u64 *)ctx->reg_rank.p, nb, (int64_t)reg_count, d_coef, (T *)ctx->coef_compact.p);
            HIPCHK(hipGetLastError());
        }
        return SZHIP_OK;
    }
    int feed_slices(const szh_qargs<T> &a) {
        const double h1 = now_ms();
        const int NF = std::max(2, std::min(G.g0.num, 12));
        const int64_t per_row = (int64_t)G.g1.num * G.g2.num;
        size_t r_lo = 0; int b0_lo = 0;
        for (int sl = 0; sl < NF; ++sl) {
            const int b0_hi = sl == NF - 1 ? G.g0.num : std::max(b0_lo, (int)((int64_t)G.g0.num * (sl + 1) / NF));
            if (b0_hi == b0_lo && sl != NF - 1) continue;
            size_t r_hi = reg_count;
            if (b0_hi < G.g0.num) r_hi = r_lo + ((size_t)(b0_hi - b0_lo) * per_row - count_lorenzo(b0_lo * per_row, b0_hi * per_row));
            unsigned idle = 0;
            while (chains_done() < r_hi) {
                szhip_chain_pool::pause();
                if (++idle > (1u << 28)) FAIL(SZHIP_ERR_INTERNAL, "coefficient chain made no progress");
            }
            const int planes_end = b0_hi >= G.g0.num ? G.g0.count : szh_blk_start(G.g0, b0_hi);
            TRY((feed_beam_slice<T>(ctx, G, a, ctx->stream2, hcoef, reg_count, r_lo, r_hi, b0_lo, b0_hi, planes_end, (const u64 *)ctx->reg_rank.p, nb)));
            r_lo = r_hi; b0_lo = b0_hi;
        }
        host_ms += now_ms() - h1;
        S.chain_overlapped = 2;
        return SZHIP_OK;
    }
    int ship_coefs(unsigned epoch, szh_u64 *coh_prog, T *dec, int64_t nbp) {
        const double h1 = now_ms();
        const szh_u64 tag = (szh_u64)(epoch & 0xffffffu) << 40;
        T *const full = (T *)(((uintptr_t)(hcoef + reg_count * 4) + 127) & ~(uintptr_t)127);
        const size_t chunk = std::max<size_t>(2048, reg_count / 32);
        size_t shipped = 0; int64_t sent = 0;
        int idle = 0;
        while (sent < nb) {
            const size_t p = chains_done();
            if (p > shipped && (p - shipped >= chunk || p == reg_count)) {
                for (int e = 0; e < ncoef; ++e)
                    for (size_t r = shipped; r < p; ++r) full[(size_t)e * nbp + blk_of_rank[r]] = hcoef[(size_t)e * reg_count + r];
                shipped = p;
                const int64_t fin = p == reg_count ? nb : (int64_t)blk_of_rank[p];
                const int64_t upto = fin == nb ? nb : fin / LINE * LINE;
                if (upto > sent) {
                    for (int e = 0; e < ncoef; ++e)
                        HIPCHK(hipMemcpyAsync(dec + (size_t)e * nbp + sent, full + (size_t)e * nbp + sent, (size_t)(upto - sent) * sizeof(T), hipMemcpyHostToDevice, ctx->stream2));
                    HIPCHK(hipStreamSynchronize(ctx->stream2));
                    __atomic_store_n(coh_prog, tag | (szh_u64)upto, __ATOMIC_RELEASE);
                    sent = upto;
                }
                idle = 0;
            } else if (++idle > 200000) FAIL(SZHIP_ERR_INTERNAL, "coefficient chain made no progress");
            else std::this_thread::sleep_for(std::chrono::microseconds(10));
        }
        host_ms += now_ms() - h1;
        S.chain_overlapped = 1;
        TP("coefficients shipped");
        return SZHIP_OK;
    }
    int launch_sweep() {
        TRY(ensure(ctx, ctx->codes_nat, (size_t)n * 2 + 64));
        TRY(ensure(ctx, ctx->codes_blk, (size_t)n * 2 + 64));
        d_nat = (uint16_t *)ctx->codes_nat.p; d_blk = (uint16_t *)ctx->codes_blk.p;
        int nI, nJ, ntiles;
        using TS = szh_tile_shape<T>;
        TRY(prepare_pencil(ctx, G, szh_gran<T>::NW, TS::TPI, TS::TPJ, &nI, &nJ, &ntiles));
        const szh_bm::grid_t bgrid = szh_bm::make_grid(G);
        beam_words = (size_t)bgrid.nKB * bgrid.nJG * szh_bm::WPG;
        if (P.sliced) {
            TRY(ensure_coherent(ctx, 512 + beam_words * 4));
            tile_done = (unsigned *)((char *)ctx->coh + 512);
            if (!ctx->stream3) HIPCHK(hipStreamCreateWithFlags(&ctx->stream3, hipStreamNonBlocking));
            if (!ctx->ev_perm) HIPCHK(hipEventCreateWithFlags(&ctx->ev_perm, hipEventDisableTiming));
        }
        szh_qargs<T> a; memset(&a, 0, sizeof(a));
        a.tile_done = tile_done; a.pub_lines = 32;
        a.G = G; a.data = d_in; a.out = nullptr; a.codes = d_nat; a.blk_lor = d_lor; a.coef = d_coef; a.coef_stride = nb;
        a.eb = eb; a.recip = 1 / eb; a.mean = mean; a.cap = (int)intervals; a.radius = (int)intervals / 2; a.use_mean = use_mean;
        a.faceI = (szh_u64 *)ctx->faceI.p; a.faceJ = (szh_u64 *)ctx->faceJ.p; a.epoch = ++ctx->epoch;
        a.nI = nI; a.nJ = nJ; a.order = (const unsigned *)ctx->order.p; a.no_reg = reg_count == 0;
        a.ticket = (unsigned *)(sm + SM_TICKET); a.err = (unsigned *)(sm + SM_ERR); a.ticket_mode = ctx->ticket_atomic ? 0 : tune_int("SZ_HIP_TICKET_MODE", 2);
        a.progress = (szh_u64 *)ctx->progress.p; a.backoff = SZH_FILL_BACKOFF; a.wide = pencil_wide<T>(G, nJ);
        a.coef_progress = nullptr;
        szh_u64 *coh_prog = nullptr;
        T *dec = nullptr;
        const int64_t nbp = (nb + LINE - 1) / LINE * LINE;
        if (overlap) {
            TRY(ensure_coherent(ctx, 256));
            TRY(ensure(ctx, ctx->coef_dec, (size_t)nbp * 4 * sizeof(T)));
            coh_prog = (szh_u64 *)ctx->coh;
            dec = (T *)ctx->coef_dec.p;
            a.coef_progress = coh_prog;
            a.coef = dec; a.coef_stride = nbp;
        }
        HIPCHK(hipEventRecord(ctx->ev[2], st));
        if (P.use_beam) {
#ifdef SZH_SYNC_LAUNCH
            if (feed) {
                TRY(ensure(ctx, ctx->pt_flags, (size_t)G.n + 64)); TRY(ensure(ctx, ctx->rb_vals, (size_t)G.n * sizeof(T) + 64)); TRY(ensure(ctx, ctx->feed_word, 256));
                HIPCHK(hipMemsetAsync(ctx->pt_flags.p, 0, (size_t)G.n, st));
                TRY(feed_slices(a));
                TRY((launch_beam<T, false>(ctx, G, a, st, reg_count, true)));
            } else
#endif
            TRY((launch_beam<T, false>(ctx, G, a, st, reg_count, feed)));
            S.quant_kernel = 2;
#ifndef SZH_SYNC_LAUNCH
            if (feed) TRY(feed_slices(a));
#endif
        } else {
            const unsigned pgrid = pencil_grid(ctx, a, ntiles);
            hipLaunchKernelGGL((k_pencil<T, false>), dim3(pgrid), dim3((TS::TPI * TS::TPJ + 2) * 64), 0, st, a);
            HIPCHK(hipGetLastError());
        }
        HIPCHK(hipEventRecord(ctx->ev[3], st));
        TP("pencil launched");
        S.quant_kernel_launches = 1;
        if (overlap) TRY(ship_coefs(a.epoch, coh_prog, dec, nbp));
        return SZHIP_OK;
    }
    int launch_hist() {
        HIPCHK(hipEventRecord(ctx->ev_in, st));
        HIPCHK(hipStreamWaitEvent(ctx->stream2, ctx->ev_in, 0));
        HIPCHK(hipMemsetAsync(d_hist, 0, (size_t)intervals * 4, ctx->stream2));
        const int use_lds = intervals <= 16384, rshift = use_lds ? hist_rshift(intervals, 16384) : 0;
        const size_t lds = use_lds ? ((size_t)intervals << rshift) * 4 : 16;
        int grid = (int)std::min<int64_t>((n / 8 + 255) / 256 + 1, 2048);
        hipLaunchKernelGGL(k_hist_u16, dim3(grid), dim3(256), lds, ctx->stream2, (const uint16_t *)d_nat, n, intervals, rshift, use_lds, d_hist, (int64_t)0);
        HIPCHK(hipGetLastError());
        HIPCHK(hipMemcpyAsync(h_hist, d_hist, (size_t)intervals * 4, hipMemcpyDeviceToHost, ctx->stream2));
        HIPCHK(hipEventRecord(ctx->ev_fit, ctx->stream2));
        return SZHIP_OK;
    }
    int prepare_permute() {
        perm_segb = choose_segb(G, 2, SZH_PERM_TILE_BYTES);
        perm_nseg = (G.g2.num + perm_segb - 1) / perm_segb;
        TRY(ensure(ctx, ctx->zcnt, (size_t)ncols * perm_nseg * 4));
        TRY(ensure(ctx, ctx->zpos, (size_t)ncols * perm_nseg * SZH_ZCAP * 4));
        const size_t tile_el = (tile_bytes(G, perm_segb, 2) + 1) / 2;
        perm_lds = ((tile_el + 1) & ~(size_t)1) * 2 + 16;
        return SZHIP_OK;
    }
    void launch_permute(hipStream_t s_, int col0, int cols) {
        hipLaunchKernelGGL((k_permute<0>), dim3((unsigned)cols, std::min(perm_nseg, std::max(1, tune_int("SZ_HIP_PERM_Y", 1)))), dim3(256), perm_lds, s_, G, (const uint16_t *)d_nat, d_blk,
                           (unsigned *)ctx->col_zeros.p, perm_segb, (unsigned *)ctx->zcnt.p, (unsigned *)ctx->zpos.p, col0);
    }
    int scan_col_zeros(hipStream_t s_) {
        hipLaunchKernelGGL(k_u32_to_u64, dim3((ncols + 255) / 256), dim3(256), 0, s_, (const unsigned *)ctx->col_zeros.p, (int64_t)ncols, (u64 *)ctx->col_zeros64.p);
        return scan_u64(ctx, (const u64 *)ctx->col_zeros64.p, ncols, (u64 *)ctx->col_off.p, sm + SM_TOTAL_UNPRED, s_);
    }
    int permute_all() {
        HIPCHK(hipMemsetAsync(ctx->col_zeros.p, 0, (size_t)ncols * 4, st));
        TRY(prepare_permute());
        launch_permute(st, 0, ncols);
        HIPCHK(hipGetLastError());
        return scan_col_zeros(st);
    }
    int hist_and_order_sliced() {
        const int NS = std::min(P.slices_req, G.g0.num);
        TRY(prepare_permute());
        const int use_lds = intervals <= 16384, rshift = use_lds ? hist_rshift(intervals, 16384) : 0;
        const size_t hist_lds = use_lds ? ((size_t)intervals << rshift) * 4 : 16;
        HIPCHK(hipMemsetAsync(d_hist, 0, (size_t)intervals * 4, ctx->stream2));
        HIPCHK(hipMemsetAsync(ctx->col_zeros.p, 0, (size_t)ncols * 4, ctx->stream3));
        const unsigned tag = (ctx->epoch & 0xfffu) << 20;
        bool sweep_over = false;
        int b0_done = 0;
        int64_t hist_first = 0;
        for (int sl = 0; sl < NS; ++sl) {
            const int b0_hi = sl == NS - 1 ? G.g0.num : std::max(b0_done, (int)((int64_t)G.g0.num * (sl + 1) / NS));
            const int rows_need = b0_hi >= G.g0.num ? G.g0.count : szh_blk_start(G.g0, b0_hi);
            size_t first_late = 0;
            unsigned spins = 0;
            while (!sweep_over && first_late < beam_words) {
                const unsigned wv = __atomic_load_n(&tile_done[first_late], __ATOMIC_ACQUIRE);
                if ((wv & 0xfff00000u) == tag && (int)(wv & 0xfffffu) >= rows_need) { ++first_late; continue; }
                szhip_chain_pool::pause();
                if ((++spins & 127u) == 0) {
                    const hipError_t q = hipEventQuery(ctx->ev[3]);
                    if (q == hipSuccess) { sweep_over = true; break; }
                    if (q != hipErrorNotReady) HIPCHK(q);
                }
            }
            if (b0_hi > b0_done) {
                const int64_t h_lo = hist_first, h_hi = b0_hi >= G.g0.num ? (int64_t)n : ((int64_t)rows_need * G.d0) / 8 * 8;
                hist_first = h_hi;
                const int grid = (int)std::min<int64_t>(((h_hi - h_lo) / 8 + 255) / 256 + 1, 2048);
                if (h_hi > h_lo) hipLaunchKernelGGL(k_hist_u16, dim3(grid), dim3(256), hist_lds, ctx->stream2, (const uint16_t *)d_nat, h_hi, intervals, rshift, use_lds, d_hist, h_lo);
                if (!P.segenc) launch_permute(ctx->stream3, b0_done * G.g1.num, (b0_hi - b0_done) * G.g1.num);
                HIPCHK(hipGetLastError());
                b0_done = b0_hi;
            }
        }
        HIPCHK(hipMemcpyAsync(h_hist, d_hist, (size_t)intervals * 4, hipMemcpyDeviceToHost, ctx->stream2));
        HIPCHK(hipEventRecord(ctx->ev_fit, ctx->stream2));
        if (!P.segenc) TRY(scan_col_zeros(ctx->stream3));
        HIPCHK(hipEventRecord(ctx->ev_perm, ctx->stream3));
        return SZHIP_OK;
    }
    int hist_and_order() {
        TRY(ensure(ctx, ctx->hist, (size_t)(65536 + 8192) * 4 + 64));
        d_hist = (unsigned *)ctx->hist.p;
        TRY(ensure_pinned(ctx, (size_t)intervals * 4 + 64));
        h_hist = (unsigned *)ctx->pinned;
        if (P.seghist) {
            TRY(ensure(ctx, ctx->seg_hist, (size_t)ncols * intervals * 4));
            HIPCHK(hipMemsetAsync(d_hist, 0, (size_t)intervals * 4, st));
            hipLaunchKernelGGL(k_col_hist, dim3((unsigned)ncols), dim3(256), ((size_t)intervals * 4) << P.sh_rshift, st, G, (const uint16_t *)d_nat, intervals, P.sh_rshift, P.se_vw, (unsigned *)ctx->seg_hist.p);
            hipLaunchKernelGGL(k_hist_reduce, dim3((unsigned)std::min<int64_t>(64, ncols)), dim3(256), 0, st, (const unsigned *)ctx->seg_hist.p, intervals, (int64_t)ncols, d_hist);
            HIPCHK(hipGetLastError());
            if (!P.dev_book) {
                HIPCHK(hipMemcpyAsync(h_hist, d_hist, (size_t)intervals * 4, hipMemcpyDeviceToHost, st));
                HIPCHK(hipEventRecord(ctx->ev_fit, st));
            }
        } else if (!P.sliced) TRY(launch_hist());
        TRY(ensure(ctx, ctx->col_zeros, (size_t)ncols * 4));
        TRY(ensure(ctx, ctx->col_zeros64, (size_t)ncols * 8));
        TRY(ensure(ctx, ctx->col_off, (size_t)ncols * 8));
        if (P.sliced) TRY(hist_and_order_sliced());
        else if (!P.segenc) TRY(permute_all());
        return SZHIP_OK;
    }
    unsigned char *put_front(unsigned char *q) const {
        memcpy(q, meta, meta_len); q += meta_len;
        szhost_put_u64be(q, (uint64_t)n); q += 8;
        szhost_put_u32be(q, (uint32_t)G.block_size); q += 4;
        if (is_double) szhost_put_f64be(q, (double)eb); else szhost_put_f32be(q, (float)eb);
        return q + sizeof(T);
    }
    int upload_segments() {
        se_segs.resize((size_t)P.se_nseg);
        for (int q = 0; q < P.se_nseg; ++q) se_segs[(size_t)q] = szh_se::make_seg(G, 1, q, P.se_segb, P.se_vw);
        TRY(ensure(ctx, ctx->seg_tab, se_segs.size() * sizeof(szh_se::seg_t)));
        HIPCHK(hipMemcpyAsync(ctx->seg_tab.p, se_segs.data(), se_segs.size() * sizeof(szh_se::seg_t), hipMemcpyHostToDevice, st));
        return SZHIP_OK;
    }
    template <class F>
    int pack_columns(unsigned char *d_stream, u64 base_bits, const u64 *d_plan, unsigned maxlen, F &&between) {
        const int64_t nent = (int64_t)ncols;
        TRY(ensure(ctx, ctx->seg_bits, (size_t)nent * 8)); TRY(ensure(ctx, ctx->seg_zeros, (size_t)nent * 8));
        TRY(ensure(ctx, ctx->seg_bitoff, (size_t)nent * 8)); TRY(ensure(ctx, ctx->seg_zoff, (size_t)nent * 8));
        u64 *const bits = (u64 *)ctx->seg_bits.p, *const zeros = (u64 *)ctx->seg_zeros.p, *const bitoff = (u64 *)ctx->seg_bitoff.p, *const zoff = (u64 *)ctx->seg_zoff.p;
        const size_t lb = intervals <= 16384 ? (size_t)intervals : 16;
        if (P.seghist) hipLaunchKernelGGL(k_col_bits_h, dim3((unsigned)((nent + 255) / 256)), dim3(256), 0, st, (const unsigned *)ctx->seg_hist.p, (const uint8_t *)ctx->len_tab.p, intervals, nent, bits, zeros);
        else hipLaunchKernelGGL(k_col_bits, dim3((unsigned)nent), dim3(256), lb, st, G, (const uint16_t *)d_nat, (const uint8_t *)ctx->len_tab.p, intervals, P.se_vw, bits, zeros);
        if (nent <= 1024 * SZH_COL_SCAN_PER && tune_int("SZ_HIP_SEG_SCAN1", 1))
            hipLaunchKernelGGL(k_col_scan, dim3(1), dim3(1024), 0, st, (const u64 *)bits, (const u64 *)zeros, (int)nent, bitoff, zoff, sm + SM_TOTAL_BITS, sm + SM_TOTAL_UNPRED, base_bits, (unsigned *)d_stream, d_plan);
        else {
            TRY(scan_u64(ctx, (const u64 *)bits, nent, bitoff, sm + SM_TOTAL_BITS));
            TRY(scan_u64(ctx, (const u64 *)zeros, nent, zoff, sm + SM_TOTAL_UNPRED));
            hipLaunchKernelGGL(k_col_bounds, dim3((unsigned)((nent + 1 + 255) / 256)), dim3(256), 0, st, (const u64 *)bitoff, nent, (const u64 *)(sm + SM_TOTAL_BITS), base_bits, (unsigned *)d_stream);
        }
        HIPCHK(hipGetLastError());
        TRY(between());
        const unsigned win = (unsigned)szh_se::seg_window_words(G, std::max(1u, maxlen), P.se_nrmax);
        const size_t lds = ((size_t)intervals + 1) * 8 + P.se_tile + 16 + (size_t)win * 4;
        auto encode = [&](auto kernel) {
            hipLaunchKernelGGL(kernel, dim3((unsigned)nent), dim3(256), lds, st, G, (const uint16_t *)d_nat, (const u64 *)ctx->code_tab.p, intervals, (const szh_se::seg_t *)ctx->seg_tab.p, P.se_nseg, P.se_vw,
                               P.se_nrmax, P.se_tile, win, (const u64 *)bitoff, (const u64 *)zoff, base_bits, (unsigned *)d_stream, d_in, (T *)ctx->unpred.p, d_plan);
        };
        if (G.g2.num >= 2 && G.g2.early <= szh_se::INNER && G.g2.late >= szh_se::INNER - 1) encode(k_col_encode<T, true>);
        else encode(k_col_encode<T, false>);
        HIPCHK(hipGetLastError());
        return SZHIP_OK;
    }
    int enqueue_readback() {
        HIPCHK(hipEventRecord(ctx->ev[4], st));
        TP("encode launched");
        HIPCHK(hipMemcpyAsync(h_small, sm, SM_COUNT * 8, hipMemcpyDeviceToHost, st));
        return SZHIP_OK;
    }
    int deliver(unsigned char *d_stream, size_t len, bool in_place) {
        if (out_on_device == 2) {
            if (!*out || *out_size < len) FAIL(SZHIP_ERR_ARG, "caller's device buffer too small (%zu < %zu)", *out_size, len);
            if (!in_place) { HIPCHK(hipMemcpyAsync(*out, d_stream, len, hipMemcpyDeviceToDevice, st)); synced = false; }
            if (!synced) HIPCHK(hipStreamSynchronize(st));
        } else if (out_on_device) {
            if (!synced) HIPCHK(hipStreamSynchronize(st));
            *out = d_stream;
        } else {
            unsigned char *h = (unsigned char *)malloc(len ? len : 1);
            if (!h) FAIL(SZHIP_ERR_INTERNAL, "out of host memory");
            const int rc_copy = staged_copy(ctx, h, d_stream, len, false);
            if (rc_copy != SZHIP_OK) { free(h); return rc_copy; }
            *out = h;
        }
        *out_size = len;
        synced = true;
        return SZHIP_OK;
    }
    int check_final(bool declined, unsigned book_status, u64 bits, u64 unpred) {
        if ((unsigned)h_small[SM_ERR] == 2) { ctx->coef_late = true; FAIL(SZHIP_ERR_INTERNAL, "wavefront kernel: the regression coefficients did not arrive"); }
        if ((unsigned)h_small[SM_ERR] != 0) { ctx->wave_timeout = true; FAIL(SZHIP_ERR_INTERNAL, "wavefront kernel: halo wait timed out"); }
        if (declined) {
            ctx->book_declined = true;
            snprintf(ctx->err, sizeof(ctx->err), "device code book declined (status %u)", book_status);
            return SZHIP_ERR_INTERNAL;
        }
        if ((bits > 0 && h_small[SM_TOTAL_BITS] != bits) || h_small[SM_TOTAL_UNPRED] != unpred)
            FAIL(SZHIP_ERR_INTERNAL, "entropy stage mismatch (bits %llu vs %llu, unpredictable %llu vs %llu)", (unsigned long long)h_small[SM_TOTAL_BITS],
                 (unsigned long long)bits, (unsigned long long)h_small[SM_TOTAL_UNPRED], (unsigned long long)unpred);
        return SZHIP_OK;
    }
    void finish_stats(size_t len, u64 unpred, int packing, int book_on_device) {
        float ms = 0;
        hipEventElapsedTime(&ms, ctx->ev[0], ctx->ev[1]); S.ms_prequant = ms;
        hipEventElapsedTime(&ms, ctx->ev[2], ctx->ev[3]); S.ms_quant = ms;
        hipEventElapsedTime(&ms, ctx->ev[3], ctx->ev[4]); S.ms_entropy = ms;
        S.n_unpred = unpred; S.ms_host = host_ms; S.ms_total = now_ms() - t_begin; S.out_bytes = len; S.packing = packing; S.book_on_device = book_on_device;
    }
    int encode_with_device_book() {
        const size_t bk_front = meta_len + 8 + 4 + sizeof(T), bk_mid = 1 + sizeof(T);
        if (!P.seghist) HIPCHK(hipStreamWaitEvent(st, ctx->ev_fit, 0));
        if (!ctx->book_pin) HIPCHK(hipHostMalloc((void **)&ctx->book_pin, 4096, hipHostMallocDefault));
        unsigned char *const blob = (unsigned char *)ctx->book_pin + 256;
        unsigned char *const mid = put_front(blob);
        mid[0] = (unsigned char)use_mean; memcpy(mid + 1, &mean, sizeof(T));
        const size_t plan_fixed = bk_front + 12 + bk_mid + ind_bytes + 8;
        const size_t tree_cap = 1 + (size_t)9 * (2 * SZH_BOOK_CAP - 1);
        const size_t unpred_cap = std::min((size_t)n * sizeof(T), (size_t)n * sizeof(T) / 4 + 65536);
        const bool in_place = out_on_device == 2 && *out && *out_size >= plan_fixed + tree_cap + 64 && ((uintptr_t)*out & 15) == 0 && tune_int("SZ_HIP_OUT_IN_PLACE", 1);
        const size_t stream_cap = in_place ? *out_size : plan_fixed + tree_cap + (size_t)n * sizeof(T) + 65536;
        if (!in_place) TRY(ensure(ctx, ctx->stream_buf, stream_cap));
        unsigned char *d_stream = in_place ? (unsigned char *)*out : (unsigned char *)ctx->stream_buf.p;
        TRY(ensure(ctx, ctx->book_stage, bk_front + bk_mid)); TRY(ensure(ctx, ctx->book_tree, tree_cap)); TRY(ensure(ctx, ctx->book_rec, 32 + SZH_PLAN_COUNT * 8));
        TRY(ensure(ctx, ctx->code_tab, (size_t)intervals * 8)); TRY(ensure(ctx, ctx->len_tab, (size_t)intervals));
        TRY(ensure(ctx, ctx->unpred, unpred_cap + 64));
        szh_book_rec *const d_rec = (szh_book_rec *)ctx->book_rec.p;
        u64 *const d_plan = (u64 *)((char *)ctx->book_rec.p + 32);
        HIPCHK(hipMemcpyAsync(ctx->book_stage.p, blob, bk_front + bk_mid, hipMemcpyHostToDevice, st));
        hipLaunchKernelGGL(k_huff_book, dim3(1), dim3(256), 0, st, (const unsigned *)d_hist, intervals, SZH_BOOK_TAB_SEG, (unsigned char *)ctx->book_tree.p, (unsigned)tree_cap,
                           (u64 *)ctx->code_tab.p, (uint8_t *)ctx->len_tab.p, d_rec, d_plan, (u64)plan_fixed, (unsigned)sizeof(T), (u64)stream_cap, (u64)unpred_cap);
        HIPCHK(hipGetLastError());
        TRY(upload_segments());
        TRY(pack_columns(d_stream, 0, (const u64 *)d_plan, 32u, [&]() -> int {
            hipLaunchKernelGGL(k_book_tail, dim3((unsigned)std::min<size_t>(64, (plan_fixed + tree_cap + 255) / 256)), dim3(256), 0, st, d_stream, (const unsigned char *)ctx->book_stage.p, (unsigned)bk_front,
                               (unsigned)bk_mid, intervals, (const unsigned char *)ctx->lor_bits.p, ind_bytes, (const unsigned char *)ctx->book_tree.p, (const szh_book_rec *)d_rec, (const u64 *)d_plan);
            return SZHIP_OK;
        }));
        hipLaunchKernelGGL((k_book_unpred<T>), dim3((unsigned)std::min<size_t>(256, (unpred_cap / sizeof(T) + 255) / 256)), dim3(256), 0, st, d_stream, (const T *)ctx->unpred.p, (const szh_book_rec *)d_rec, (const u64 *)d_plan);
        HIPCHK(hipGetLastError());
        TRY(enqueue_readback());
        HIPCHK(hipMemcpyAsync(ctx->book_pin, ctx->book_rec.p, 32 + SZH_PLAN_COUNT * 8, hipMemcpyDeviceToHost, st));
        HIPCHK(hipStreamSynchronize(st));
        synced = true;
        TP("final sync");
        szh_book_rec rec; memcpy(&rec, ctx->book_pin, sizeof(rec));
        const u64 *const plan = (const u64 *)ctx->book_pin + 4;
        print_trace();
        TRY(check_final(book_declines(rec.status, plan[SZH_PLAN_STATUS], tune_int("SZ_HIP_TEST_BOOK_FALLBACK", 0)), rec.status ? rec.status : (unsigned)plan[SZH_PLAN_STATUS],
                        rec.total_bits, rec.total_unpred));
        const size_t len = (size_t)plan[SZH_PLAN_TOTAL_LEN];
        TRY(deliver(d_stream, len, in_place));
        finish_stats(len, rec.total_unpred, 1, 1);
        return SZHIP_OK;
    }
    int build_host_book() {
        TP("permute launched");
        HIPCHK(hipEventSynchronize(ctx->ev_fit));
        TP("hist on host");
        double h0 = now_ms();
        szhost_huff *hf = szhost_huff_build(2 * (int)intervals, h_hist, nullptr, intervals);
        host_ms += now_ms() - h0;
        total_unpred = h_hist[0];
        if (!hf) FAIL(SZHIP_ERR_INTERNAL, "Huffman build failed");
        TP("tree built");
        join_sections();
        TP("sections joined");
        if (section_failed) { szhost_huff_free(hf); FAIL(SZHIP_ERR_INTERNAL, "coefficient Huffman build failed"); }
        for (int e = 0; e < ncoef; ++e) sections_total += sec_len[e];
        h0 = now_ms();
        const size_t tree_bytes = szhost_huff_tree_size(hf);
        pre_len = meta_len + 8 + 4 + sizeof(T) + 4 + 4 + 4 + tree_bytes + 1 + sizeof(T) + ind_bytes;
        hdr_len = pre_len + sections_total + 8;
        unpred_bytes = (size_t)total_unpred * sizeof(T);
        total_len = hdr_len + unpred_bytes + (size_t)((hf->total_bits + 7) / 8);
        { const int rc = ensure_pinned(ctx, pre_len + 8 + 64); if (rc != SZHIP_OK) { szhost_huff_free(hf); return rc; } }
        hdr = (unsigned char *)ctx->pinned;
        memset(hdr, 0, pre_len + 8);
        unsigned char *q = put_front(hdr);
        szhost_put_u32be(q, intervals); q += 4;
        szhost_put_u32be(q, (uint32_t)tree_bytes); q += 4;
        szhost_put_u32be(q, (uint32_t)hf->n_nodes); q += 4;
        szhost_huff_tree_write(hf, q); q += tree_bytes;
        *q++ = (unsigned char)use_mean;
        memcpy(q, &mean, sizeof(T)); q += sizeof(T);
        memcpy(q, ind_bits, ind_bytes); q += ind_bytes;
        const uint64_t tu = total_unpred; memcpy(q, &tu, 8);
        tab_code.resize(intervals); tab_len.resize(intervals);
        for (unsigned s = 0; s < intervals; ++s) { tab_code[s] = hf->code[s]; tab_len[s] = hf->len[s]; }
        total_bits = hf->total_bits;
        szhost_huff_free(hf);
        for (unsigned s = 0; s < intervals; ++s) enc_maxlen = std::max<unsigned>(enc_maxlen, tab_len[s]);
        lds_e32 = (size_t)intervals * 8 + ((size_t)SZH_E32_ROUND * enc_maxlen / 32 + 4) * 4 + 16;
        enc32 = enc_maxlen >= 1 && enc_maxlen <= 32 && lds_e32 <= 60 * 1024 && tune_int("SZ_HIP_ENC32", 1);
        if (P.revise(enc_maxlen)) {
            if (P.sliced) HIPCHK(hipStreamWaitEvent(st, ctx->ev_perm, 0));
            TRY(permute_all());
        }
        if (P.segenc) TRY(upload_segments());
        if (P.segenc) for (unsigned s = 0; s < intervals; ++s) tab_code[s] = (tab_code[s] << 32) | tab_len[s] | (s == 0 ? 0x10000u : 0u);
        else if (enc32) for (unsigned s = 0; s < intervals; ++s) tab_code[s] = (tab_code[s] << 8) | tab_len[s];
        host_ms += now_ms() - h0;
        TRY(ensure(ctx, ctx->code_tab, (size_t)intervals * 8));
        TRY(ensure(ctx, ctx->len_tab, (size_t)intervals));
        HIPCHK(hipMemcpyAsync(ctx->code_tab.p, tab_code.data(), (size_t)intervals * 8, hipMemcpyHostToDevice, st));
        HIPCHK(hipMemcpyAsync(ctx->len_tab.p, tab_len.data(), (size_t)intervals, hipMemcpyHostToDevice, st));
        return SZHIP_OK;
    }
    int copy_header(unsigned char *d_stream) {
        HIPCHK(hipMemcpyAsync(d_stream, hdr, pre_len, hipMemcpyHostToDevice, st));
        HIPCHK(hipMemcpyAsync(d_stream + pre_len + sections_total, hdr + pre_len, 8, hipMemcpyHostToDevice, st));
        if (sections_total) {
            const hipStream_t ssec = ctx->stream3 ? ctx->stream3 : ctx->stream2;
            HIPCHK(hipEventRecord(ctx->ev_feed, st));
            HIPCHK(hipStreamWaitEvent(ssec, ctx->ev_feed, 0));
            size_t off = pre_len;
            for (int e = 0; e < ncoef; ++e) { HIPCHK(hipMemcpyAsync(d_stream + off, ctx->sec_pin[e], sec_len[e], hipMemcpyHostToDevice, ssec)); off += sec_len[e]; }
            HIPCHK(hipEventRecord(ctx->ev_sec, ssec));
        }
        return SZHIP_OK;
    }
    int pack_block_ordered(unsigned char *d_stream) {
        const u64 base_bits = (u64)(hdr_len + unpred_bytes) * 8;
        if (P.sliced) HIPCHK(hipStreamWaitEvent(st, ctx->ev_perm, 0));
        if (total_unpred > 0) {
            TRY(ensure(ctx, ctx->unpred, unpred_bytes));
            HIPCHK(hipEventRecord(ctx->ev_in, st));
            HIPCHK(hipStreamWaitEvent(ctx->stream2, ctx->ev_in, 0));
            hipLaunchKernelGGL((k_unpred<T, 0>), dim3(ncols), dim3(256), 0, ctx->stream2, G, (const uint16_t *)d_blk, (const unsigned *)ctx->col_zeros.p,
                               (const u64 *)ctx->col_off.p, d_in, (T *)ctx->unpred.p, (T *)nullptr, (const unsigned *)ctx->zcnt.p, (const unsigned *)ctx->zpos.p, perm_segb, perm_nseg);
            HIPCHK(hipGetLastError());
            HIPCHK(hipEventRecord(ctx->ev_fit, ctx->stream2));
        }
        if (total_bits > 0) {
            const int64_t nchunks = (n + SZH_ENC_CHUNK - 1) / SZH_ENC_CHUNK;
            TRY(ensure(ctx, ctx->chunk_bits, (size_t)nchunks * 8 + 64));
            TRY(ensure(ctx, ctx->chunk_off, (size_t)nchunks * 8));
            hipLaunchKernelGGL(k_chunk_bits, dim3((unsigned)((nchunks + SZH_CB_PER - 1) / SZH_CB_PER)), dim3(256), 0, st, (const uint16_t *)d_blk, n, (const uint8_t *)ctx->len_tab.p, intervals, (u64 *)ctx->chunk_bits.p);
            TRY(scan_u64(ctx, (const u64 *)ctx->chunk_bits.p, nchunks, (u64 *)ctx->chunk_off.p, sm + SM_TOTAL_BITS));
            if (enc32) {
                const int64_t nrounds = (n + SZH_E32_ROUND - 1) / SZH_E32_ROUND;
                hipLaunchKernelGGL(k_encode32, dim3((unsigned)((nrounds + SZH_E32_PER - 1) / SZH_E32_PER)), dim3(256), lds_e32, st, (const uint16_t *)d_blk, n, (const u64 *)ctx->code_tab.p,
                                   intervals, (const u64 *)ctx->chunk_off.p, base_bits, (unsigned *)d_stream);
            } else
                hipLaunchKernelGGL(k_encode, dim3((unsigned)((nchunks + SZH_ENC_PER - 1) / SZH_ENC_PER)), dim3(256), 0, st, (const uint16_t *)d_blk, n, (const u64 *)ctx->code_tab.p,
                                   (const uint8_t *)ctx->len_tab.p, intervals, (const u64 *)ctx->chunk_off.p, base_bits, (unsigned *)d_stream);
            HIPCHK(hipGetLastError());
        }
        if (total_unpred > 0) HIPCHK(hipStreamWaitEvent(st, ctx->ev_fit, 0));
        return SZHIP_OK;
    }
    int encode_with_host_book() {
        TRY(build_host_book());
        const bool in_place = out_on_device == 2 && *out && *out_size >= total_len + 64 && ((uintptr_t)*out & 15) == 0 && tune_int("SZ_HIP_OUT_IN_PLACE", 1);
        if (!in_place) TRY(ensure(ctx, ctx->stream_buf, total_len + 64));
        unsigned char *d_stream = in_place ? (unsigned char *)*out : (unsigned char *)ctx->stream_buf.p;
        if (P.segenc) {
            TRY(pack_columns(d_stream, (u64)(hdr_len + unpred_bytes) * 8, (const u64 *)nullptr, enc_maxlen, [&]() -> int {
                TRY(copy_header(d_stream));
                return ensure(ctx, ctx->unpred, unpred_bytes + 64);
            }));
        } else {
            HIPCHK(hipMemsetAsync(d_stream, 0, total_len + 64, st));
            TRY(copy_header(d_stream));
            TRY(pack_block_ordered(d_stream));
        }
        if (total_unpred > 0) HIPCHK(hipMemcpyAsync(d_stream + hdr_len, ctx->unpred.p, unpred_bytes, hipMemcpyDeviceToDevice, st));
        if (sections_total) HIPCHK(hipStreamWaitEvent(st, ctx->ev_sec, 0));
        TRY(enqueue_readback());
        TRY(deliver(d_stream, total_len, in_place));
        TP("final sync");
        print_trace();
        const int rc = check_final(false, 0, total_bits, total_unpred);
        if (rc != SZHIP_OK) {
            if (!out_on_device && *out) { free(*out); *out = nullptr; }
            *out_size = 0;
            return rc;
        }
        finish_stats(total_len, total_unpred, P.segenc ? 1 : 0, 0);
        return SZHIP_OK;
    }
};

template <class T>
int compress_impl(szhip_ctx *ctx, const void *data, int data_on_device, size_t r0, size_t r1, size_t r2, double eb_in, const szhip_params *prm, const unsigned char *meta, size_t meta_len, int out_on_device,
                  unsigned char **out, size_t *out_size, szhip_stats *stats)
{
    sz21_call<T> c(ctx, r0, r1, r2, eb_in, prm, meta, meta_len, out_on_device, out, out_size);
    int rc = c.stage_and_fit(data, data_on_device);
    if (rc == SZHIP_OK) rc = c.choose_intervals();
    if (rc == SZHIP_OK) rc = c.join_fit();
    if (rc == SZHIP_CONSTANT && stats) *stats = c.S;
    if (rc != SZHIP_OK) return rc;
    if (ctx->chain_pool) ctx->chain_pool->arm();
    if (c.reg_count > 0) { TRY(c.prepare_chains()); TRY(c.run_chains()); }
    HIPCHK(hipEventRecord(ctx->ev[1], c.st));
    c.TP("ev1");
    c.P = sz21_make_plan<T>(ctx, c.G, c.intervals, c.reg_count, beam_applies<T>(c.G, c.d_in, c.reg_count), c.overlap, c.feed, meta_len);
    TRY(c.launch_sweep());
    TRY(c.hist_and_order());
    TRY(c.P.dev_book ? c.encode_with_device_book() : c.encode_with_host_book());
    if (stats) *stats = c.S;
    return SZHIP_OK;
}

#define HDEC_CHECK(ctx) do { if ((ctx)->hdec_res[1] != 0 || (tune_int("SZ_HIP_TEST_HDEC_FALLBACK", 0) && !(ctx)->hdec_sync_rounds)) { (ctx)->hdec_unconverged = true; \
         \
        snprintf((ctx)->err, sizeof((ctx)->err), "Huffman decode: %llu start guesses still moving after two rounds", (ctx)->hdec_res[1]); return SZHIP_ERR_INTERNAL; } } while (0)
int huff_decode_device(szhip_ctx *ctx, u64 *sm, const unsigned char *d_bits, unsigned bytes_before, u64 total_bits, const std::vector<uint32_t> &dtab, int n_nodes,
                       int single_symbol, int64_t n, uint16_t *d_out_codes, u64 *total_sym_host)
{
    if (!ctx->hdec_res) HIPCHK(hipHostMalloc((void **)&ctx->hdec_res, 64, hipHostMallocDefault));
    ctx->hdec_res[0] = (u64)n; ctx->hdec_res[1] = 0;
    *total_sym_host = (u64)n;
    hipStream_t st = ctx->stream;
    if (single_symbol >= 0) {
        hipLaunchKernelGGL(k_fill_u16, dim3((unsigned)((n + 255) / 256)), dim3(256), 0, st, d_out_codes, n, (uint16_t)single_symbol);
        HIPCHK(hipGetLastError());
    } else {
        const int64_t nsub = (int64_t)((total_bits + SZH_SUBSEQ_BITS - 1) / SZH_SUBSEQ_BITS);
        if (nsub == 0) FAIL(SZHIP_ERR_STREAM, "empty Huffman payload");
        const size_t lut_off = (dtab.size() * 4 + 63) / 64 * 64;
        TRY(ensure(ctx, ctx->dec_tab, lut_off + SZH_LUT_BYTES));
        HIPCHK(hipMemcpyAsync(ctx->dec_tab.p, dtab.data(), dtab.size() * 4, hipMemcpyHostToDevice, st));
        hipLaunchKernelGGL(k_hdec_build_lut, dim3(SZH_LUT_SIZE / 256), dim3(256), 0, st, (const unsigned *)ctx->dec_tab.p, (uint4 *)((char *)ctx->dec_tab.p + lut_off));
        TRY(ensure(ctx, ctx->starts, (size_t)nsub * 8)); TRY(ensure(ctx, ctx->ends, (size_t)nsub * 8));
        TRY(ensure(ctx, ctx->counts, (size_t)nsub * 8)); TRY(ensure(ctx, ctx->offs, (size_t)nsub * 8));
        TRY(ensure(ctx, ctx->dirty, (size_t)nsub));
        szh_hdec_args a;
        a.bits = d_bits; a.total_bits = total_bits; a.bytes_before = bytes_before; a.table = (const unsigned *)ctx->dec_tab.p; a.n_nodes = n_nodes;
        a.table_in_lds = (size_t)n_nodes * 8 <= 13 * 1024; a.nsub = nsub;
        a.lut = (const uint4 *)((char *)ctx->dec_tab.p + lut_off);
        a.starts = (u64 *)ctx->starts.p; a.ends = (u64 *)ctx->ends.p; a.counts = (u64 *)ctx->counts.p;
        a.dirty = (unsigned char *)ctx->dirty.p; a.changed = (unsigned *)(sm + SM_CHANGED);
        const size_t lds_tab = a.table_in_lds ? (size_t)n_nodes * 8 : 16;
        const size_t lds_pass = SZH_HDEC_LDS + SZH_LUT_SIZE * 4 + lds_tab, lds_write = SZH_HDEC_LDS + SZH_LUT_SIZE * 16 + lds_tab;
        const unsigned gsub = (unsigned)((nsub + 255) / 256);
        hipLaunchKernelGGL(k_hdec_init, dim3(gsub), dim3(256), 0, st, a);
        const bool optimistic = !ctx->hdec_sync_rounds;
        constexpr int64_t opt_rounds = 3;
// ... 222 lines not shown
    }
    if (stream_on_device) TRY(copy_on_device());
    if (H.finish) finisher.th = std::thread([&] { finisher.rc = H.finish(); });
    if (tune_int("SZ_HIP_TIMING", 0)) fprintf(stderr, "[header on host %.3f ms after the call began]\n", now_ms() - t_begin);
    const T eb = H.eb, mean = H.mean;
    const unsigned intervals = H.intervals;
    const int use_mean = H.use_mean, n_nodes = H.n_nodes, single_symbol = H.single_symbol;
    const size_t reg_count = H.reg_count, unpred_off = H.unpred_off, pay_off = H.pay_off;
    const uint64_t total_unpred = H.total_unpred;
    std::vector<T> &hcoef = H.coef;
    std::vector<uint32_t> &dtab = H.dtab;
    const u64 total_bits = (u64)(stream_len - pay_off) * 8;
    S.intervals = intervals; S.use_mean = use_mean; S.n_reg_blocks = reg_count; S.n_unpred = total_unpred;
    host_ms += now_ms() - h0;

    TRY(ensure(ctx, ctx->small, SM_COUNT * 8));
    u64 *sm = (u64 *)ctx->small.p;
    HIPCHK(hipMemsetAsync(sm, 0, SM_COUNT * 8, st));
    const size_t nat_elems = (size_t)n;
    const bool dec_beam = beam_applies<T>(G, out_on_device ? (const void *)out : (const void *)nullptr, reg_count);
    TRY(ensure(ctx, ctx->codes_nat, nat_elems * 2 + 64));
    TRY(ensure(ctx, ctx->codes_blk, (size_t)n * 2 + 64));
    uint16_t *d_nat = (uint16_t *)ctx->codes_nat.p, *d_blk = (uint16_t *)ctx->codes_blk.p;

    u64 total_sym = 0;
    TRY(huff_decode_device(ctx, sm, d_stream + pay_off, (unsigned)std::min<size_t>(pay_off, 4096), total_bits, dtab, n_nodes, single_symbol, n, d_blk, &total_sym));

    const int ncols = G.g0.num * G.g1.num;
    TRY(ensure(ctx, ctx->col_zeros, (size_t)ncols * 4));
    TRY(ensure(ctx, ctx->col_zeros64, (size_t)ncols * 8));
    TRY(ensure(ctx, ctx->col_off, (size_t)ncols * 8));
    int perm_segb = 1, perm_nseg = 1;
    T *d_out = (T *)out;
    if (!out_on_device) { TRY(ensure(ctx, ctx->out, (size_t)n * sizeof(T))); d_out = (T *)ctx->out.p; }
    T *d_sweep = d_out;
    const int up_vw = (G.g2.count % 8) == 0 ? 8 : ((G.g2.count % 4) == 0 ? 4 : 1);
    int up_segb = 0, up_nseg = 0; size_t up_lds = 0;
    bool col_unpack = dec_beam && tune_int("SZ_HIP_COL_UNPACK", 1) != 0 && ((uintptr_t)d_blk & 15) == 0 && (double)n < 4.0e9;
    if (col_unpack) {
        const size_t rows_max = (size_t)G.g0.early * G.g1.early, want = (size_t)std::max(4, tune_int("SZ_HIP_UNPACK_TILE_KB", 24)) * 1024;
        int sb = 1;
        while (sb < G.g2.num && (rows_max * (size_t)(sb + 1) * G.g2.early + 16) * 2 <= want) ++sb;
        up_segb = sb; up_nseg = (G.g2.num + sb - 1) / sb;
        up_lds = ((rows_max * (size_t)sb * G.g2.early + 16) * 2 + 15) & ~(size_t)15;
        if (up_lds > 63 * 1024 || rows_max > 128) col_unpack = false;
    }
    std::vector<szh_se::seg_t> up_segs;
    if (col_unpack) {
        hipLaunchKernelGGL(k_col_zeros, dim3((unsigned)ncols), dim3(256), 0, st, G, (const uint16_t *)d_blk, (unsigned *)ctx->col_zeros.p);
        HIPCHK(hipGetLastError());
        up_segs.resize((size_t)up_nseg);
        for (int q = 0; q < up_nseg; ++q) up_segs[(size_t)q] = szh_se::make_seg(G, 1, q, up_segb, up_vw);
        TRY(ensure(ctx, ctx->seg_tab, up_segs.size() * sizeof(szh_se::seg_t)));
        HIPCHK(hipMemcpyAsync(ctx->seg_tab.p, up_segs.data(), up_segs.size() * sizeof(szh_se::seg_t), hipMemcpyHostToDevice, st));
    } else
    {
        HIPCHK(hipMemsetAsync(ctx->col_zeros.p, 0, (size_t)ncols * 4, st));
        const int segb = choose_segb(G, 2, SZH_PERM_TILE_BYTES);
        const int nseg = (G.g2.num + segb - 1) / segb;
        TRY(ensure(ctx, ctx->zcnt, (size_t)ncols * nseg * 4));
        TRY(ensure(ctx, ctx->zpos, (size_t)ncols * nseg * SZH_ZCAP * 4));
        hipLaunchKernelGGL((k_permute<1>), dim3(ncols, std::min(nseg, std::max(1, tune_int("SZ_HIP_PERM_Y", nseg)))), dim3(256), tile_bytes(G, segb, 2), st, G, (const uint16_t *)d_blk, d_nat,
                           (unsigned *)ctx->col_zeros.p, segb, (unsigned *)ctx->zcnt.p, (unsigned *)ctx->zpos.p, 0);
        perm_segb = segb; perm_nseg = nseg;
        HIPCHK(hipGetLastError());
    }
    if (col_unpack && ncols <= 1024 * SZH_COL_SCAN_PER && tune_int("SZ_HIP_SEG_SCAN1", 1)) {
        hipLaunchKernelGGL(k_col_zscan, dim3(1), dim3(1024), 0, st, (const unsigned *)ctx->col_zeros.p, (int)ncols, (u64 *)ctx->col_off.p, sm + SM_TOTAL_UNPRED);
        HIPCHK(hipGetLastError());
    } else {
        hipLaunchKernelGGL(k_u32_to_u64, dim3((ncols + 255) / 256), dim3(256), 0, st, (const unsigned *)ctx->col_zeros.p, (int64_t)ncols,
                           (u64 *)ctx->col_zeros64.p);
        TRY(scan_u64(ctx, (const u64 *)ctx->col_zeros64.p, ncols, (u64 *)ctx->col_off.p, sm + SM_TOTAL_UNPRED));
    }
    ctx->hdec_res[2] = 0;
    HIPCHK(hipMemcpyAsync(&ctx->hdec_res[2], sm + SM_TOTAL_UNPRED, 8, hipMemcpyDeviceToHost, st));
    auto decoder_checks = [&]() -> int {
        HDEC_CHECK(ctx);
        total_sym = ctx->hdec_res[0];
        const u64 zeros_found = ctx->hdec_res[2];
        if ((int64_t)total_sym < n) FAIL(SZHIP_ERR_STREAM, "Huffman payload holds %llu symbols, need %lld", (unsigned long long)total_sym, (long long)n);
        if (zeros_found != total_unpred) FAIL(SZHIP_ERR_STREAM, "stream lists %llu unpredictable values, codes need %llu",
                                              (unsigned long long)total_unpred, (unsigned long long)zeros_found);
        return SZHIP_OK;
    };
    const bool checks_last = col_unpack && tune_int("SZ_HIP_DEC_CHECKS_LAST", 1) != 0;
    if (!checks_last) {
        HIPCHK(hipStreamSynchronize(st));
        TRY(decoder_checks());
    }
    if (col_unpack) {
        TRY(ensure(ctx, ctx->unpred, (size_t)total_unpred * sizeof(T) + 64));
        if (total_unpred > 0) HIPCHK(hipMemcpyAsync(ctx->unpred.p, d_stream + unpred_off, (size_t)total_unpred * sizeof(T), hipMemcpyDeviceToDevice, st));
        hipLaunchKernelGGL((k_col_unpack<T>), dim3((unsigned)ncols), dim3(256), up_lds, st, G, (const uint16_t *)d_blk, d_nat, (const szh_se::seg_t *)ctx->seg_tab.p, up_nseg, up_vw,
                           (const u64 *)ctx->col_off.p, (const T *)ctx->unpred.p, (u64)total_unpred, d_sweep);
        HIPCHK(hipGetLastError());
    } else
    if (total_unpred > 0) {
        TRY(ensure(ctx, ctx->unpred, (size_t)total_unpred * sizeof(T)));
        HIPCHK(hipMemcpyAsync(ctx->unpred.p, d_stream + unpred_off, (size_t)total_unpred * sizeof(T), hipMemcpyDeviceToDevice, st));
        hipLaunchKernelGGL((k_unpred<T, 1>), dim3(ncols), dim3(256), 0, st, G, (const uint16_t *)d_blk, (const unsigned *)ctx->col_zeros.p,
                           (const u64 *)ctx->col_off.p, (const T *)nullptr, (T *)ctx->unpred.p, d_sweep, (const unsigned *)ctx->zcnt.p,
                           (const unsigned *)ctx->zpos.p, perm_segb, perm_nseg);
        HIPCHK(hipGetLastError());
    }
    TRY(ensure(ctx, ctx->coef, (size_t)nb * 4 * sizeof(T)));
// ... 65 lines not shown
```

Before: 380.1.

## Batch small per-call copies and fills, pin tables, add op counters

```diff
diff --git a/include/szhip.h b/include/szhip.h
--- a/include/szhip.h
+++ b/include/szhip.h
@@ -56,6 +56,7 @@
 
 void szhip_destroy(szhip_ctx *ctx);
 const char *szhip_last_error(szhip_ctx *ctx);
+int szhip_last_call_ops(szhip_ctx *ctx, unsigned out[4]);
 
 int szhip_stage_input(szhip_ctx *ctx, const void *host_data, size_t bytes, void **device_ptr);
 
diff --git a/sz_amd/api.py b/sz_amd/api.py
--- a/sz_amd/api.py
+++ b/sz_amd/api.py
@@ -105,6 +105,8 @@
     L.szhip_create.argtypes = [ctypes.POINTER(ctypes.c_void_p), ctypes.c_int]; L.szhip_create.restype = ctypes.c_int
     L.szhip_destroy.argtypes = [ctypes.c_void_p]; L.szhip_destroy.restype = None
     L.szhip_last_error.argtypes = [ctypes.c_void_p]; L.szhip_last_error.restype = ctypes.c_char_p
+    if hasattr(L, "szhip_last_call_ops"):
+        L.szhip_last_call_ops.argtypes = [ctypes.c_void_p, ctypes.POINTER(ctypes.c_uint * 4)]; L.szhip_last_call_ops.restype = ctypes.c_int
     L.szhip_minmax.argtypes = [ctypes.c_void_p, ctypes.c_int, ctypes.c_void_p, ctypes.c_int, sz,
                                ctypes.POINTER(ctypes.c_double), ctypes.POINTER(ctypes.c_double)]
     L.szhip_minmax.restype = ctypes.c_int
@@ -316,6 +318,13 @@
     def _err(self, rc, what):
         raise SZError(f"{what} failed ({rc}): {lib().szhip_last_error(self._h).decode(errors='replace')}")
 
+    def last_call_ops(self):
+        v = (ctypes.c_uint * 4)()
+        rc = lib().szhip_last_call_ops(self._h, ctypes.byref(v))
+        if rc:
+            self._err(rc, "szhip_last_call_ops")
+        return dict(copies=int(v[0]), fills=int(v[1]), launches=int(v[2]), waits=int(v[3]))
+
     def minmax(self, ptr, on_device, n, dtype):
         lo, hi = ctypes.c_double(), ctypes.c_double()
         rc = lib().szhip_minmax(self._h, 0 if np.dtype(dtype) == np.float32 else 1, ptr, int(on_device), n,
diff --git a/sz_amd/csrc/szhip.hip b/sz_amd/csrc/szhip.hip
--- a/sz_amd/csrc/szhip.hip
+++ b/sz_amd/csrc/szhip.hip
@@ -138,6 +138,13 @@
     std::vector<int> chain_codes; std::vector<unsigned char> chain_unpred;
     unsigned char *sec_pin[4] = {nullptr, nullptr, nullptr, nullptr}; size_t sec_pin_cap[4] = {0, 0, 0, 0};
     szhip_chain_pool *chain_pool = nullptr;
+    DevBuf fit_res;
+    DevBuf tabs;
+    void *tab_pin = nullptr; size_t tab_pin_cap = 0;
+    unsigned long long *words_pin = nullptr;
+    void *seg_pin = nullptr; size_t seg_pin_cap = 0;
+    unsigned long long seg_key[4] = {0, 0, 0, 0}; const void *seg_key_buf = nullptr;
+    unsigned ops[4] = {0, 0, 0, 0};
 };
 
 namespace {
@@ -222,7 +229,7 @@
                       &ctx->order, &ctx->small, &ctx->hist, &ctx->col_zeros, &ctx->col_zeros64, &ctx->seg_bits, &ctx->seg_zeros, &ctx->seg_bitoff, &ctx->seg_zoff, &ctx->seg_hist, &ctx->seg_tab, &ctx->col_off, &ctx->partial,
                       &ctx->samples, &ctx->unpred, &ctx->stream_buf, &ctx->chunk_bits, &ctx->chunk_off, &ctx->code_tab,
                       &ctx->len_tab, &ctx->dec_tab, &ctx->starts, &ctx->ends, &ctx->counts, &ctx->offs, &ctx->dirty, &ctx->zcnt, &ctx->zpos,
-                      &ctx->pwr_log, &ctx->pwr_signs, &ctx->pwr_small, &ctx->coef_dec, &ctx->msst_ptab, &ctx->msst_cells, &ctx->msst_rec, &ctx->msst_pe, &ctx->book_tree, &ctx->book_rec, &ctx->book_stage};
+                      &ctx->pwr_log, &ctx->pwr_signs, &ctx->pwr_small, &ctx->coef_dec, &ctx->msst_ptab, &ctx->msst_cells, &ctx->msst_rec, &ctx->msst_pe, &ctx->book_tree, &ctx->book_rec, &ctx->book_stage, &ctx->fit_res, &ctx->tabs};
     for (DevBuf *b : bufs) if (b->p) hipFree(b->p);
     if (ctx->pinned) hipHostFree(ctx->pinned);
     if (ctx->pinned2) hipHostFree(ctx->pinned2);
@@ -230,6 +237,9 @@
     if (ctx->coh) hipHostFree(ctx->coh);
     if (ctx->hdec_res) hipHostFree(ctx->hdec_res);
     if (ctx->book_pin) hipHostFree(ctx->book_pin);
+    if (ctx->tab_pin) hipHostFree(ctx->tab_pin);
+    if (ctx->words_pin) hipHostFree(ctx->words_pin);
+    if (ctx->seg_pin) hipHostFree(ctx->seg_pin);
     for (int w = 0; w < SZH_STAGE_T; ++w) for (int k = 0; k < 2; ++k) { if (ctx->stage_buf[w][k]) hipHostFree(ctx->stage_buf[w][k]); if (ctx->stage_ev[w][k]) hipEventDestroy(ctx->stage_ev[w][k]); }
     for (int i = 0; i < 6; ++i) if (ctx->ev[i]) hipEventDestroy(ctx->ev[i]);
     if (ctx->ev_in) hipEventDestroy(ctx->ev_in);
@@ -245,6 +255,13 @@
 }
 
 const char *szhip_last_error(szhip_ctx *ctx) { return ctx ? ctx->err : "no context"; }
+
+int szhip_last_call_ops(szhip_ctx *ctx, unsigned out[4])
+{
+    if (!ctx || !out) return SZHIP_ERR_ARG;
+    for (int i = 0; i < 4; ++i) out[i] = ctx->ops[i];
+    return SZHIP_OK;
+}
 
 struct szhip_pool_job {
     int dtype; const void *data; int on_dev; size_t r0, r1, r2; double eb; szhip_params prm; const unsigned char *meta; size_t meta_len;
diff --git a/sz_amd/csrc/szhip_kernels.h b/sz_amd/csrc/szhip_kernels.h
--- a/sz_amd/csrc/szhip_kernels.h
+++ b/sz_amd/csrc/szhip_kernels.h
@@ -286,6 +286,11 @@
     }
 }
 
+__global__ __launch_bounds__(64) void k_call_init(u64 *small, int nsmall, u64 *fit)
+{
+    for (int i = (int)threadIdx.x; i < nsmall; i += 64) small[i] = 0;
+    if (threadIdx.x < 4) fit[threadIdx.x] = threadIdx.x == 0 ? ~0ull : 0ull;
+}
 template <class T>
 __global__ __launch_bounds__(256) void k_minmax(const T *__restrict__ data, int64_t n, u64 *minmax)
 {
diff --git a/sz_amd/csrc/szhip_rt.inc b/sz_amd/csrc/szhip_rt.inc
--- a/sz_amd/csrc/szhip_rt.inc
+++ b/sz_amd/csrc/szhip_rt.inc
@@ -22,15 +22,22 @@
         FAIL(code, __VA_ARGS__);                                                                       \
     } while (0)
 
+enum { OP_COPY = 0, OP_FILL = 1, OP_LAUNCH = 2, OP_WAIT = 3 };
+static inline hipError_t op_copy(szhip_ctx *ctx, void *dst, const void *src, size_t bytes, hipMemcpyKind kind, hipStream_t s) { ++ctx->ops[OP_COPY]; return hipMemcpyAsync(dst, src, bytes, kind, s); }
+static inline hipError_t op_fill(szhip_ctx *ctx, void *dst, int v, size_t bytes, hipStream_t s) { ++ctx->ops[OP_FILL]; return hipMemsetAsync(dst, v, bytes, s); }
+static inline hipError_t op_sync(szhip_ctx *ctx, hipStream_t s) { ++ctx->ops[OP_WAIT]; return hipStreamSynchronize(s); }
+static inline hipError_t op_esync(szhip_ctx *ctx, hipEvent_t e) { ++ctx->ops[OP_WAIT]; return hipEventSynchronize(e); }
+#define OP_LAUNCH_K(...) do { ++ctx->ops[OP_LAUNCH]; hipLaunchKernelGGL(__VA_ARGS__); } while (0)
+
 int ensure(szhip_ctx *ctx, DevBuf &b, size_t bytes, bool zero_new = false)
 {
     if (bytes == 0) bytes = 16;
     if (b.cap >= bytes) return SZHIP_OK;
-    if (b.p) { HIPCHK(hipStreamSynchronize(ctx->stream)); HIPCHK(hipFree(b.p)); b.p = nullptr; b.cap = 0; }
+    if (b.p) { HIPCHK(op_sync(ctx, ctx->stream)); HIPCHK(hipFree(b.p)); b.p = nullptr; b.cap = 0; }
     size_t cap = bytes + bytes / 8 + 256;
     HIPCHK(hipMalloc(&b.p, cap));
     b.cap = cap;
-    if (zero_new) HIPCHK(hipMemsetAsync(b.p, 0, cap, ctx->stream));
+    if (zero_new) HIPCHK(op_fill(ctx, b.p, 0, cap, ctx->stream));
     return SZHIP_OK;
 }
 
@@ -39,7 +46,7 @@
 int ensure_host(szhip_ctx *ctx, void *&p, size_t &have, size_t bytes, hipStream_t user, unsigned flags = hipHostMallocDefault)
 {
     if (have >= bytes) return SZHIP_OK;
-    if (p) { HIPCHK(hipStreamSynchronize(user)); HIPCHK(hipHostFree(p)); p = nullptr; have = 0; }
+    if (p) { HIPCHK(op_sync(ctx, user)); HIPCHK(hipHostFree(p)); p = nullptr; have = 0; }
     size_t cap = bytes + bytes / 4 + 4096;
     HIPCHK(hipHostMalloc(&p, cap, flags));
     have = cap;
@@ -208,9 +215,9 @@
     const int64_t nblk = (n + SZH_SCAN_TILE - 1) / SZH_SCAN_TILE;
     TRY(ensure(ctx, ctx->partial, (size_t)(nblk + 1) * 8));
     u64 *partial = (u64 *)ctx->partial.p;
-    hipLaunchKernelGGL(k_scan_partials, dim3((unsigned)nblk), dim3(256), 0, sst, in, n, partial);
-    hipLaunchKernelGGL(k_scan_single, dim3(1), dim3(256), 0, sst, partial, nblk, total_dev);
-    hipLaunchKernelGGL(k_scan_final, dim3((unsigned)nblk), dim3(256), 0, sst, in, n, (const u64 *)partial, out);
+    OP_LAUNCH_K(k_scan_partials, dim3((unsigned)nblk), dim3(256), 0, sst, in, n, partial);
+    OP_LAUNCH_K(k_scan_single, dim3(1), dim3(256), 0, sst, partial, nblk, total_dev);
+    OP_LAUNCH_K(k_scan_final, dim3((unsigned)nblk), dim3(256), 0, sst, in, n, (const u64 *)partial, out);
     HIPCHK(hipGetLastError());
     return SZHIP_OK;
 }
@@ -246,8 +253,8 @@
         std::vector<unsigned> ord((size_t)nTI * nTJ);
         szh_fill_pencil_order(nTI, nTJ, ord.data());
         TRY(ensure(ctx, ctx->order, ord.size() * 4));
-        HIPCHK(hipMemcpyAsync(ctx->order.p, ord.data(), ord.size() * 4, hipMemcpyHostToDevice, ctx->stream));
-        HIPCHK(hipStreamSynchronize(ctx->stream));
+        HIPCHK(op_copy(ctx, ctx->order.p, ord.data(), ord.size() * 4, hipMemcpyHostToDevice, ctx->stream));
+        HIPCHK(op_sync(ctx, ctx->stream));
         ctx->order_nI = nTI; ctx->order_nJ = nTJ;
     }
     *nI_out = nI; *nJ_out = nJ; *ntiles_out = nTI * nTJ;
@@ -302,7 +309,7 @@
 #else
         const bool prepared = false;
 #endif
-        if (!prepared) HIPCHK(hipMemsetAsync(ctx->pt_flags.p, 0, (size_t)G.n, st));
+        if (!prepared) HIPCHK(op_fill(ctx, ctx->pt_flags.p, 0, (size_t)G.n, st));
         a.ptflags = (const uint8_t *)ctx->pt_flags.p;
         const unsigned rgrid = (unsigned)(G.g0.num * G.g1.num);
         if (!DEC) {
@@ -310,25 +317,25 @@
             a.xr = (const T *)ctx->rb_vals.p;
             if (feed) {
                 TRY(ensure(ctx, ctx->feed_word, 256));
-                if (!prepared) HIPCHK(hipMemsetAsync(ctx->feed_word.p, 0, 256, st));
+                if (!prepared) HIPCHK(op_fill(ctx, ctx->feed_word.p, 0, 256, st));
                 a.reg_ready = (const unsigned *)ctx->feed_word.p;
                 HIPCHK(hipEventRecord(ctx->ev_feed, st));
                 HIPCHK(hipStreamWaitEvent(ctx->stream2, ctx->ev_feed, 0));
             } else
-            hipLaunchKernelGGL((k_reg_points<T, 0>), dim3(rgrid), dim3(256), 0, st, G, a.blk_lor, a.coef, a.coef_stride, a.data, (T *)ctx->rb_vals.p, a.codes, (uint8_t *)ctx->pt_flags.p,
+            OP_LAUNCH_K((k_reg_points<T, 0>), dim3(rgrid), dim3(256), 0, st, G, a.blk_lor, a.coef, a.coef_stride, a.data, (T *)ctx->rb_vals.p, a.codes, (uint8_t *)ctx->pt_flags.p,
                                a.eb, a.recip, a.cap, a.radius, 0);
         } else
-            hipLaunchKernelGGL((k_reg_points<T, 2>), dim3(rgrid), dim3(256), 0, st, G, a.blk_lor, a.coef, a.coef_stride, (const T *)nullptr, a.out, a.codes, (uint8_t *)ctx->pt_flags.p,
+            OP_LAUNCH_K((k_reg_points<T, 2>), dim3(rgrid), dim3(256), 0, st, G, a.blk_lor, a.coef, a.coef_stride, (const T *)nullptr, a.out, a.codes, (uint8_t *)ctx->pt_flags.p,
                                a.eb, a.recip, a.cap, a.radius, 0);
         HIPCHK(hipGetLastError());
     }
     const dim3 grid(wgs), block(szh_bm::WPG * 64);
     if (hasreg) {
-        if (a.use_mean) hipLaunchKernelGGL((k_beam<T, DEC, true, true>), grid, block, 0, st, a);
-        else hipLaunchKernelGGL((k_beam<T, DEC, false, true>), grid, block, 0, st, a);
+        if (a.use_mean) OP_LAUNCH_K((k_beam<T, DEC, true, true>), grid, block, 0, st, a);
+        else OP_LAUNCH_K((k_beam<T, DEC, false, true>), grid, block, 0, st, a);
     } else {
-        if (a.use_mean) hipLaunchKernelGGL((k_beam<T, DEC, true, false>), grid, block, 0, st, a);
-        else hipLaunchKernelGGL((k_beam<T, DEC, false, false>), grid, block, 0, st, a);
+        if (a.use_mean) OP_LAUNCH_K((k_beam<T, DEC, true, false>), grid, block, 0, st, a);
+        else OP_LAUNCH_K((k_beam<T, DEC, false, false>), grid, block, 0, st, a);
     }
     HIPCHK(hipGetLastError());
     return SZHIP_OK;
@@ -340,14 +347,14 @@
 {
     if (r_hi > r_lo)
         for (int e = 0; e < 4; ++e)
-            HIPCHK(hipMemcpyAsync((T *)ctx->coef_compact.p + (size_t)e * reg_count + r_lo, hcoef + (size_t)e * reg_count + r_lo, (r_hi - r_lo) * sizeof(T), hipMemcpyHostToDevice, s2));
+            HIPCHK(op_copy(ctx, (T *)ctx->coef_compact.p + (size_t)e * reg_count + r_lo, hcoef + (size_t)e * reg_count + r_lo, (r_hi - r_lo) * sizeof(T), hipMemcpyHostToDevice, s2));
     const int64_t blk_lo = (int64_t)b0_lo * G.g1.num * G.g2.num, blk_hi = std::min<int64_t>(nb, (int64_t)b0_hi * G.g1.num * G.g2.num);
     if (r_hi > r_lo && blk_hi > blk_lo) {
-        hipLaunchKernelGGL((k_move_coef<T, 1>), dim3((unsigned)((nb + 255) / 256)), dim3(256), 0, s2, a.blk_lor, reg_rank, nb, (int64_t)reg_count, (T *)a.coef, (T *)ctx->coef_compact.p);
-        hipLaunchKernelGGL((k_reg_points<T, 0>), dim3((unsigned)((b0_hi - b0_lo) * G.g1.num)), dim3(256), 0, s2, G, a.blk_lor, a.coef, a.coef_stride, a.data, (T *)ctx->rb_vals.p,
+        OP_LAUNCH_K((k_move_coef<T, 1>), dim3((unsigned)((nb + 255) / 256)), dim3(256), 0, s2, a.blk_lor, reg_rank, nb, (int64_t)reg_count, (T *)a.coef, (T *)ctx->coef_compact.p);
+        OP_LAUNCH_K((k_reg_points<T, 0>), dim3((unsigned)((b0_hi - b0_lo) * G.g1.num)), dim3(256), 0, s2, G, a.blk_lor, a.coef, a.coef_stride, a.data, (T *)ctx->rb_vals.p,
                            a.codes, (uint8_t *)ctx->pt_flags.p, a.eb, a.recip, a.cap, a.radius, b0_lo);
     }
-    hipLaunchKernelGGL(k_store_u32, dim3(1), dim3(1), 0, s2, (unsigned *)ctx->feed_word.p, (unsigned)planes_end);
+    OP_LAUNCH_K(k_store_u32, dim3(1), dim3(1), 0, s2, (unsigned *)ctx->feed_word.p, (unsigned)planes_end);
     HIPCHK(hipGetLastError());
     return SZHIP_OK;
 }
diff --git a/sz_amd/csrc/szhip_sz21.inc b/sz_amd/csrc/szhip_sz21.inc
--- a/sz_amd/csrc/szhip_sz21.inc
+++ b/sz_amd/csrc/szhip_sz21.inc
@@ -64,6 +64,7 @@
     const double t_begin = now_ms(); double host_ms = 0;
     const int tp_on = tune_int("SZ_HIP_TIMING", 0); double tp_t[32]; const char *tp_n[32]; int tp_k = 0;
     szhip_stats S;
+    u64 *d_fit = nullptr; unsigned char *d_ind = nullptr;
     const T *d_in = nullptr; u64 *sm = nullptr; T *d_coef = nullptr; uint8_t *d_lor = nullptr; uint16_t *d_nat = nullptr, *d_blk = nullptr; unsigned *d_hist = nullptr, *h_hist = nullptr;
     T noise = 0; bool fit_tile = false; int ft_nseg = 0;
     size_t ind_bytes = 0; unsigned char *ind_bits = nullptr; u64 *nreg_h = nullptr, *minmax_h = nullptr;
@@ -72,7 +73,8 @@
     sz21_plan P;
     unsigned *tile_done = nullptr; size_t beam_words = 0;
     int perm_segb = 1, perm_nseg = 1; size_t perm_lds = 0;
-    std::vector<szh_se::seg_t> se_segs; std::vector<u64> tab_code; std::vector<uint8_t> tab_len;
+    u64 *tab_code = nullptr; uint8_t *tab_len = nullptr;
+    const u64 *d_code = nullptr; const uint8_t *d_len = nullptr;
     unsigned enc_maxlen = 0; bool enc32 = false; size_t lds_e32 = 0;
     unsigned char *hdr = nullptr; size_t pre_len = 0, sections_total = 0, hdr_len = 0, unpred_bytes = 0, total_len = 0; u64 total_bits = 0, total_unpred = 0;
     u64 h_small[SM_COUNT];
@@ -124,16 +126,15 @@
         return p;
     }
     int launch_fit(hipStream_t s_, int um, T mn) {
-        if (fit_tile) hipLaunchKernelGGL((k_fit_tile<T>), dim3((unsigned)((int64_t)ncols * ft_nseg)), dim3(64), 0, s_, G, d_in, d_coef, d_lor, noise, um, mn, sm + SM_MINMAX, ft_nseg);
-        else hipLaunchKernelGGL((k_fit_select<T>), dim3((unsigned)((nb + 255) / 256)), dim3(256), 0, s_, G, d_in, d_coef, d_lor, noise, um, mn, sm + SM_MINMAX);
+        if (fit_tile) OP_LAUNCH_K((k_fit_tile<T>), dim3((unsigned)((int64_t)ncols * ft_nseg)), dim3(64), 0, s_, G, d_in, d_coef, d_lor, noise, um, mn, d_fit, ft_nseg);
+        else OP_LAUNCH_K((k_fit_select<T>), dim3((unsigned)((nb + 255) / 256)), dim3(256), 0, s_, G, d_in, d_coef, d_lor, noise, um, mn, d_fit);
         HIPCHK(hipGetLastError());
         return SZHIP_OK;
     }
     int launch_pack_lor(hipStream_t s_) {
-        hipLaunchKernelGGL(k_pack_lor, dim3((unsigned)((ind_bytes + 255) / 256)), dim3(256), 0, s_, (const uint8_t *)d_lor, nb, (uint8_t *)ctx->lor_bits.p, sm + SM_NREG);
-        HIPCHK(hipGetLastError());
-        HIPCHK(hipMemcpyAsync(ind_bits, ctx->lor_bits.p, ind_bytes, hipMemcpyDeviceToHost, s_));
-        HIPCHK(hipMemcpyAsync(nreg_h, sm + SM_NREG, 8, hipMemcpyDeviceToHost, s_));
+        OP_LAUNCH_K(k_pack_lor, dim3((unsigned)((ind_bytes + 255) / 256)), dim3(256), 0, s_, (const uint8_t *)d_lor, nb, (uint8_t *)d_ind, d_fit + 2);
+        HIPCHK(hipGetLastError());
+        HIPCHK(op_copy(ctx, ctx->pinned2, d_fit, 32 + ind_bytes, hipMemcpyDeviceToHost, s_));
         return SZHIP_OK;
     }
     int stage_and_fit(const void *data, int data_on_device) {
@@ -145,9 +146,12 @@
         }
         TRY(ensure(ctx, ctx->small, SM_COUNT * 8));
         sm = (u64 *)ctx->small.p;
-        HIPCHK(hipMemsetAsync(sm, 0, SM_COUNT * 8, st));
-        static const u64 minmax_init[2] = {~0ull, 0ull};
-        HIPCHK(hipMemcpyAsync(sm + SM_MINMAX, minmax_init, 16, hipMemcpyHostToDevice, st));
+        ind_bytes = ((size_t)nb + 7) / 8;
+        TRY(ensure(ctx, ctx->fit_res, 32 + ind_bytes + 8));
+        d_fit = (u64 *)ctx->fit_res.p; d_ind = (unsigned char *)ctx->fit_res.p + 32;
+        if (!ctx->words_pin) HIPCHK(hipHostMalloc((void **)&ctx->words_pin, 4096, hipHostMallocDefault));
+        OP_LAUNCH_K(k_call_init, dim3(1), dim3(64), 0, st, sm, (int)SM_COUNT, d_fit);
+        HIPCHK(hipGetLastError());
         TRY(ensure(ctx, ctx->coef, (size_t)nb * 4 * sizeof(T)));
         TRY(ensure(ctx, ctx->blk_lor, (size_t)nb));
         d_coef = (T *)ctx->coef.p;
@@ -160,14 +164,11 @@
         fit_tile = !two_d && szh_ft::applies<T>(G, d_in) && tune_int("SZ_HIP_FIT_TILE", 0) != 0;
         ft_nseg = (G.g2.num + szh_ft::shape<T>::SEGB - 1) / szh_ft::shape<T>::SEGB;
         TRY(launch_fit(ctx->stream2, 0, (T)0));
-        ind_bytes = ((size_t)nb + 7) / 8;
-        TRY(ensure(ctx, ctx->lor_bits, ind_bytes + 8));
         TRY(ensure_pinned2(ctx, ind_bytes + 32));
+        minmax_h = (u64 *)ctx->pinned2;
+        nreg_h = (u64 *)ctx->pinned2 + 2;
         ind_bits = (unsigned char *)ctx->pinned2 + 32;
-        nreg_h = (u64 *)ctx->pinned2;
-        minmax_h = (u64 *)ctx->pinned2 + 2;
         TRY(launch_pack_lor(ctx->stream2));
-        HIPCHK(hipMemcpyAsync(minmax_h, sm + SM_MINMAX, 16, hipMemcpyDeviceToHost, ctx->stream2));
         HIPCHK(hipEventRecord(ctx->ev_fit, ctx->stream2));
         return SZHIP_OK;
     }
@@ -181,36 +182,37 @@
             while (szh_meanwalk_pos(w, M_hi) < n) M_hi *= 2;
             while (M < M_hi) { int64_t mid = (M + M_hi) / 2; if (szh_meanwalk_pos(w, mid) >= n) M_hi = mid; else M = mid + 1; }
             TRY(ensure(ctx, ctx->samples, (size_t)M * sizeof(T)));
-            TRY(ensure_pinned(ctx, std::max<size_t>((size_t)M * sizeof(T), (size_t)(max_radius + 8192) * 4 + 64)));
-            hipLaunchKernelGGL((k_gather_mean<T>), dim3((unsigned)((M + 255) / 256)), dim3(256), 0, st, d_in, w, M, (T *)ctx->samples.p);
+            const size_t within_off = ((size_t)(max_radius + 8192) * 4 + 7) & ~(size_t)7, res_bytes = within_off + 8;
+            TRY(ensure_pinned(ctx, std::max<size_t>((size_t)M * sizeof(T), res_bytes + 64)));
+            TRY(ensure(ctx, ctx->hist, std::max<size_t>(res_bytes, (size_t)(65536 + 8192) * 4) + 64));
+            unsigned *d_rh = (unsigned *)ctx->hist.p, *d_fh = d_rh + max_radius;
+            u64 *const d_within = (u64 *)((char *)ctx->hist.p + within_off);
+            HIPCHK(op_fill(ctx, d_rh, 0, res_bytes, st));
+            OP_LAUNCH_K((k_gather_mean<T>), dim3((unsigned)((M + 255) / 256)), dim3(256), 0, st, d_in, w, M, (T *)ctx->samples.p);
             HIPCHK(hipGetLastError());
-            HIPCHK(hipMemcpyAsync(ctx->pinned, ctx->samples.p, (size_t)M * sizeof(T), hipMemcpyDeviceToHost, st));
+            HIPCHK(op_copy(ctx, ctx->pinned, ctx->samples.p, (size_t)M * sizeof(T), hipMemcpyDeviceToHost, st));
             TP("mean enqueued");
-            HIPCHK(hipStreamSynchronize(st));
+            HIPCHK(op_sync(ctx, st));
             TP("mean on host");
             double h0 = now_ms();
             const double smean = szhost_seq_mean(is_double, ctx->pinned, (size_t)M);
             host_ms += now_ms() - h0;
-            TRY(ensure(ctx, ctx->hist, (size_t)(max_radius + 8192) * 4 + 64));
-            unsigned *d_rh = (unsigned *)ctx->hist.p, *d_fh = d_rh + max_radius;
-            HIPCHK(hipMemsetAsync(d_rh, 0, (size_t)(max_radius + 8192) * 4, st));
             const int64_t nrows = szh_sample_row_limit(G, prm->sample_distance);
             if (!two_d && (G.g0.count <= 1 || G.g1.count <= 1)) {
-                hipLaunchKernelGGL((k_sample_walk<T, true>), dim3(1), dim3(64), 0, st, G, d_in, prm->sample_distance, (double)eb, (T)smean, max_radius, d_rh, d_fh, sm + SM_WITHIN);
+                OP_LAUNCH_K((k_sample_walk<T, true>), dim3(1), dim3(64), 0, st, G, d_in, prm->sample_distance, (double)eb, (T)smean, max_radius, d_rh, d_fh, d_within);
                 HIPCHK(hipGetLastError());
             } else if (nrows > 0) {
                 int grid = (int)std::min<int64_t>((nrows + 255) / 256, 1024);
-                hipLaunchKernelGGL((k_sample<T, true>), dim3(grid), dim3(256), 0, st, G, d_in, nrows, prm->sample_distance, (double)eb, (T)smean, max_radius, d_rh, d_fh, sm + SM_WITHIN);
+                OP_LAUNCH_K((k_sample<T, true>), dim3(grid), dim3(256), 0, st, G, d_in, nrows, prm->sample_distance, (double)eb, (T)smean, max_radius, d_rh, d_fh, d_within);
                 HIPCHK(hipGetLastError());
             }
             unsigned *s_hist = (unsigned *)ctx->pinned;
-            u64 within = 0;
-            HIPCHK(hipMemcpyAsync(s_hist, d_rh, (size_t)(max_radius + 8192) * 4, hipMemcpyDeviceToHost, st));
-            HIPCHK(hipMemcpyAsync(&within, sm + SM_WITHIN, 8, hipMemcpyDeviceToHost, st));
+            HIPCHK(op_copy(ctx, s_hist, d_rh, res_bytes, hipMemcpyDeviceToHost, st));
             TP("sample enqueued");
-            HIPCHK(hipStreamSynchronize(st));
+            HIPCHK(op_sync(ctx, st));
             TP("sample on host");
             h0 = now_ms();
+            u64 within; memcpy(&within, (const char *)s_hist + within_off, 8);
             u64 sample_count = 0;
             for (unsigned i = 0; i < max_radius; ++i) sample_count += s_hist[i];
             szhost_decision dec;
@@ -219,12 +221,13 @@
             intervals = dec.intervals; use_mean = two_d ? 0 : dec.use_mean;
             if (use_mean) {
                 T *d_sum = (T *)(sm + SM_MEANSUM);
-                hipLaunchKernelGGL((k_mean_seq<T>), dim3(1), dim3(64), 0, st, d_in, n, (T)dec.dense_pos, eb, d_sum, sm + SM_MEANCNT);
+                OP_LAUNCH_K((k_mean_seq<T>), dim3(1), dim3(64), 0, st, d_in, n, (T)dec.dense_pos, eb, d_sum, sm + SM_MEANCNT);
                 HIPCHK(hipGetLastError());
-                T hsum = 0; u64 hcnt = 0;
-                HIPCHK(hipMemcpyAsync(&hsum, d_sum, sizeof(T), hipMemcpyDeviceToHost, st));
-                HIPCHK(hipMemcpyAsync(&hcnt, sm + SM_MEANCNT, 8, hipMemcpyDeviceToHost, st));
-                HIPCHK(hipStreamSynchronize(st));
+                u64 *const w = ctx->words_pin + 16;
+                HIPCHK(op_copy(ctx, w, sm, SM_COUNT * 8, hipMemcpyDeviceToHost, st));
+                HIPCHK(op_sync(ctx, st));
+                T hsum; memcpy(&hsum, w + SM_MEANSUM, sizeof(T));
+                const u64 hcnt = w[SM_MEANCNT];
                 if (hcnt > 0) mean = hsum / (T)hcnt;
             }
         }
@@ -236,10 +239,10 @@
         HIPCHK(hipStreamWaitEvent(st, ctx->ev_fit, 0));
         if (use_mean) {
             TRY(launch_fit(st, use_mean, mean));
-            HIPCHK(hipMemsetAsync(sm + SM_NREG, 0, 8, st));
+            HIPCHK(op_fill(ctx, d_fit + 2, 0, 8, st));
             TRY(launch_pack_lor(st));
-            HIPCHK(hipStreamSynchronize(st));
-        } else HIPCHK(hipEventSynchronize(ctx->ev_fit));
+            HIPCHK(op_sync(ctx, st));
+        } else HIPCHK(op_esync(ctx, ctx->ev_fit));
         TP("fit joined");
         reg_count = (size_t)*nreg_h;
         S.n_reg_blocks = reg_count;
@@ -254,7 +257,7 @@
             else { szhost_put_f32be(q, (float)lo); szhost_put_f32be(q + 4, (float)top); }
             S.vmin = (double)lo; S.vmax = (double)hi;
             if ((double)range <= eb_in) {
-                HIPCHK(hipStreamSynchronize(ctx->stream2)); HIPCHK(hipStreamSynchronize(st));
+                HIPCHK(op_sync(ctx, ctx->stream2)); HIPCHK(op_sync(ctx, st));
                 *out = nullptr; *out_size = 0;
                 S.ms_total = now_ms() - t_begin;
                 return SZHIP_CONSTANT;
@@ -290,7 +293,7 @@
         for (int e = 0; e < ncoef; ++e) {
             const size_t bound = sizeof(T) + 12 + (13 * 2 * std::min<size_t>(reg_count, 65536) + 16) + 8 + (8 * reg_count + 16) + 4 + reg_count * sizeof(T) + 64;
             if (ctx->sec_pin_cap[e] < bound) {
-                HIPCHK(hipStreamSynchronize(ctx->stream2)); HIPCHK(hipStreamSynchronize(st));
+                HIPCHK(op_sync(ctx, ctx->stream2)); HIPCHK(op_sync(ctx, st));
                 if (ctx->sec_pin[e]) { HIPCHK(hipHostFree(ctx->sec_pin[e])); ctx->sec_pin[e] = nullptr; ctx->sec_pin_cap[e] = 0; }
                 HIPCHK(hipHostMalloc((void **)&ctx->sec_pin[e], bound + bound / 8, hipHostMallocDefault));
                 ctx->sec_pin_cap[e] = bound + bound / 8;
@@ -299,9 +302,9 @@
         TRY(ensure(ctx, ctx->reg_flags, (size_t)nb * 8));
         TRY(ensure(ctx, ctx->reg_rank, (size_t)nb * 8));
         TRY(ensure(ctx, ctx->coef_compact, reg_count * 4 * sizeof(T)));
-        hipLaunchKernelGGL(k_reg_flags, dim3((unsigned)((nb + 255) / 256)), dim3(256), 0, st, (const uint8_t *)d_lor, nb, (u64 *)ctx->reg_flags.p);
+        OP_LAUNCH_K(k_reg_flags, dim3((unsigned)((nb + 255) / 256)), dim3(256), 0, st, (const uint8_t *)d_lor, nb, (u64 *)ctx->reg_flags.p);
         TRY(scan_u64(ctx, (const u64 *)ctx->reg_flags.p, nb, (u64 *)ctx->reg_rank.p, sm + SM_SCRATCH));
-        hipLaunchKernelGGL((k_move_coef<T, 0>), dim3((unsigned)((nb + 255) / 256)), dim3(256), 0, st, (const uint8_t *)d_lor, (const u64 *)ctx->reg_rank.p, nb, (int64_t)reg_count, d_coef, (T *)ctx->coef_compact.p);
+        OP_LAUNCH_K((k_move_coef<T, 0>), dim3((unsigned)((nb + 255) / 256)), dim3(256), 0, st, (const uint8_t *)d_lor, (const u64 *)ctx->reg_rank.p, nb, (int64_t)reg_count, d_coef, (T *)ctx->coef_compact.p);
         HIPCHK(hipGetLastError());
 #ifndef SZH_SYNC_LAUNCH
         overlap = !beam_applies<T>(G, d_in, reg_count) && !two_d && !ctx->gate && !ctx->no_chain_overlap && g_compress_calls.load() <= 1;
@@ -328,16 +331,16 @@
         two_pieces = feed && reg_count >= 4 * first_piece;
         if (two_pieces) {
             for (int e = 0; e < 4; ++e)
-                HIPCHK(hipMemcpyAsync(hcoef + (size_t)e * reg_count, (const T *)ctx->coef_compact.p + (size_t)e * reg_count, first_piece * sizeof(T), hipMemcpyDeviceToHost, st));
+                HIPCHK(op_copy(ctx, hcoef + (size_t)e * reg_count, (const T *)ctx->coef_compact.p + (size_t)e * reg_count, first_piece * sizeof(T), hipMemcpyDeviceToHost, st));
             HIPCHK(hipEventRecord(ctx->ev_sec, st));
             for (int e = 0; e < 4; ++e)
-                HIPCHK(hipMemcpyAsync(hcoef + (size_t)e * reg_count + first_piece, (const T *)ctx->coef_compact.p + (size_t)e * reg_count + first_piece, (reg_count - first_piece) * sizeof(T), hipMemcpyDeviceToHost, st));
+                HIPCHK(op_copy(ctx, hcoef + (size_t)e * reg_count + first_piece, (const T *)ctx->coef_compact.p + (size_t)e * reg_count + first_piece, (reg_count - first_piece) * sizeof(T), hipMemcpyDeviceToHost, st));
             chain_avail = 0;
-            HIPCHK(hipEventSynchronize(ctx->ev_sec));
+            HIPCHK(op_esync(ctx, ctx->ev_sec));
             __atomic_store_n(&chain_avail, first_piece, __ATOMIC_RELEASE);
         } else {
-            HIPCHK(hipMemcpyAsync(hcoef, ctx->coef_compact.p, reg_count * 4 * sizeof(T), hipMemcpyDeviceToHost, st));
-            HIPCHK(hipStreamSynchronize(st));
+            HIPCHK(op_copy(ctx, hcoef, ctx->coef_compact.p, reg_count * 4 * sizeof(T), hipMemcpyDeviceToHost, st));
+            HIPCHK(op_sync(ctx, st));
         }
         TP("coef on host");
         double h0 = now_ms();
@@ -376,7 +379,7 @@
                     chain_t1[e] = now_ms() - t_begin;
                 }, [this](int e) { make_section(e); });
             if (two_pieces) {
-                HIPCHK(hipStreamSynchronize(st));
+                HIPCHK(op_sync(ctx, st));
                 __atomic_store_n(&chain_avail, reg_count, __ATOMIC_RELEASE);
             }
             if (!feed) ctx->chain_pool->wait_chains();
@@ -385,8 +388,8 @@
         TP("chain done");
         if (tp_on) fprintf(stderr, "chain threads: %.2f-%.2f %.2f-%.2f %.2f-%.2f %.2f-%.2f | ", chain_t0[0], chain_t1[0], chain_t0[1], chain_t1[1], chain_t0[2], chain_t1[2], chain_t0[3], chain_t1[3]);
         if (!overlap && !feed) {
-            HIPCHK(hipMemcpyAsync(ctx->coef_compact.p, hcoef, reg_count * 4 * sizeof(T), hipMemcpyHostToDevice, st));
-            hipLaunchKernelGGL((k_move_coef<T, 1>), dim3((unsigned)((nb + 255) / 256)), dim3(256), 0, st, (const uint8_t *)d_lor, (const u64 *)ctx->reg_rank.p, nb, (int64_t)reg_count, d_coef, (T *)ctx->coef_compact.p);
+            HIPCHK(op_copy(ctx, ctx->coef_compact.p, hcoef, reg_count * 4 * sizeof(T), hipMemcpyHostToDevice, st));
+            OP_LAUNCH_K((k_move_coef<T, 1>), dim3((unsigned)((nb + 255) / 256)), dim3(256), 0, st, (const uint8_t *)d_lor, (const u64 *)ctx->reg_rank.p, nb, (int64_t)reg_count, d_coef, (T *)ctx->coef_compact.p);
             HIPCHK(hipGetLastError());
         }
         return SZHIP_OK;
@@ -431,8 +434,8 @@
                 const int64_t upto = fin == nb ? nb : fin / LINE * LINE;
                 if (upto > sent) {
                     for (int e = 0; e < ncoef; ++e)
-                        HIPCHK(hipMemcpyAsync(dec + (size_t)e * nbp + sent, full + (size_t)e * nbp + sent, (size_t)(upto - sent) * sizeof(T), hipMemcpyHostToDevice, ctx->stream2));
-                    HIPCHK(hipStreamSynchronize(ctx->stream2));
+                        HIPCHK(op_copy(ctx, dec + (size_t)e * nbp + sent, full + (size_t)e * nbp + sent, (size_t)(upto - sent) * sizeof(T), hipMemcpyHostToDevice, ctx->stream2));
+                    HIPCHK(op_sync(ctx, ctx->stream2));
                     __atomic_store_n(coh_prog, tag | (szh_u64)upto, __ATOMIC_RELEASE);
                     sent = upto;
                 }
@@ -446,6 +449,9 @@
         return SZHIP_OK;
     }
     int launch_sweep() {
+        TRY(ensure(ctx, ctx->hist, (size_t)(65536 + 8192) * 4 + 64));
+        d_hist = (unsigned *)ctx->hist.p;
+        if (P.seghist) HIPCHK(op_fill(ctx, d_hist, 0, (size_t)intervals * 4, st));
         TRY(ensure(ctx, ctx->codes_nat, (size_t)n * 2 + 64));
         TRY(ensure(ctx, ctx->codes_blk, (size_t)n * 2 + 64));
         d_nat = (uint16_t *)ctx->codes_nat.p; d_blk = (uint16_t *)ctx->codes_blk.p;
@@ -485,7 +491,7 @@
 #ifdef SZH_SYNC_LAUNCH
             if (feed) {
                 TRY(ensure(ctx, ctx->pt_flags, (size_t)G.n + 64)); TRY(ensure(ctx, ctx->rb_vals, (size_t)G.n * sizeof(T) + 64)); TRY(ensure(ctx, ctx->feed_word, 256));
-                HIPCHK(hipMemsetAsync(ctx->pt_flags.p, 0, (size_t)G.n, st));
+                HIPCHK(op_fill(ctx, ctx->pt_flags.p, 0, (size_t)G.n, st));
                 TRY(feed_slices(a));
                 TRY((launch_beam<T, false>(ctx, G, a, st, reg_count, true)));
             } else
@@ -497,7 +503,7 @@
 #endif
         } else {
             const unsigned pgrid = pencil_grid(ctx, a, ntiles);
-            hipLaunchKernelGGL((k_pencil<T, false>), dim3(pgrid), dim3((TS::TPI * TS::TPJ + 2) * 64), 0, st, a);
+            OP_LAUNCH_K((k_pencil<T, false>), dim3(pgrid), dim3((TS::TPI * TS::TPJ + 2) * 64), 0, st, a);
             HIPCHK(hipGetLastError());
         }
         HIPCHK(hipEventRecord(ctx->ev[3], st));
@@ -509,13 +515,13 @@
     int launch_hist() {
         HIPCHK(hipEventRecord(ctx->ev_in, st));
         HIPCHK(hipStreamWaitEvent(ctx->stream2, ctx->ev_in, 0));
-        HIPCHK(hipMemsetAsync(d_hist, 0, (size_t)intervals * 4, ctx->stream2));
+        HIPCHK(op_fill(ctx, d_hist, 0, (size_t)intervals * 4, ctx->stream2));
         const int use_lds = intervals <= 16384, rshift = use_lds ? hist_rshift(intervals, 16384) : 0;
         const size_t lds = use_lds ? ((size_t)intervals << rshift) * 4 : 16;
         int grid = (int)std::min<int64_t>((n / 8 + 255) / 256 + 1, 2048);
-        hipLaunchKernelGGL(k_hist_u16, dim3(grid), dim3(256), lds, ctx->stream2, (const uint16_t *)d_nat, n, intervals, rshift, use_lds, d_hist, (int64_t)0);
-        HIPCHK(hipGetLastError());
-        HIPCHK(hipMemcpyAsync(h_hist, d_hist, (size_t)intervals * 4, hipMemcpyDeviceToHost, ctx->stream2));
+        OP_LAUNCH_K(k_hist_u16, dim3(grid), dim3(256), lds, ctx->stream2, (const uint16_t *)d_nat, n, intervals, rshift, use_lds, d_hist, (int64_t)0);
+        HIPCHK(hipGetLastError());
+        HIPCHK(op_copy(ctx, h_hist, d_hist, (size_t)intervals * 4, hipMemcpyDeviceToHost, ctx->stream2));
         HIPCHK(hipEventRecord(ctx->ev_fit, ctx->stream2));
         return SZHIP_OK;
     }
@@ -529,15 +535,15 @@
         return SZHIP_OK;
     }
     void launch_permute(hipStream_t s_, int col0, int cols) {
-        hipLaunchKernelGGL((k_permute<0>), dim3((unsigned)cols, std::min(perm_nseg, std::max(1, tune_int("SZ_HIP_PERM_Y", 1)))), dim3(256), perm_lds, s_, G, (const uint16_t *)d_nat, d_blk,
+        OP_LAUNCH_K((k_permute<0>), dim3((unsigned)cols, std::min(perm_nseg, std::max(1, tune_int("SZ_HIP_PERM_Y", 1)))), dim3(256), perm_lds, s_, G, (const uint16_t *)d_nat, d_blk,
                            (unsigned *)ctx->col_zeros.p, perm_segb, (unsigned *)ctx->zcnt.p, (unsigned *)ctx->zpos.p, col0);
     }
     int scan_col_zeros(hipStream_t s_) {
-        hipLaunchKernelGGL(k_u32_to_u64, dim3((ncols + 255) / 256), dim3(256), 0, s_, (const unsigned *)ctx->col_zeros.p, (int64_t)ncols, (u64 *)ctx->col_zeros64.p);
+        OP_LAUNCH_K(k_u32_to_u64, dim3((ncols + 255) / 256), dim3(256), 0, s_, (const unsigned *)ctx->col_zeros.p, (int64_t)ncols, (u64 *)ctx->col_zeros64.p);
         return scan_u64(ctx, (const u64 *)ctx->col_zeros64.p, ncols, (u64 *)ctx->col_off.p, sm + SM_TOTAL_UNPRED, s_);
     }
     int permute_all() {
-        HIPCHK(hipMemsetAsync(ctx->col_zeros.p, 0, (size_t)ncols * 4, st));
+        HIPCHK(op_fill(ctx, ctx->col_zeros.p, 0, (size_t)ncols * 4, st));
         TRY(prepare_permute());
         launch_permute(st, 0, ncols);
         HIPCHK(hipGetLastError());
@@ -548,8 +554,8 @@
         TRY(prepare_permute());
         const int use_lds = intervals <= 16384, rshift = use_lds ? hist_rshift(intervals, 16384) : 0;
         const size_t hist_lds = use_lds ? ((size_t)intervals << rshift) * 4 : 16;
-        HIPCHK(hipMemsetAsync(d_hist, 0, (size_t)intervals * 4, ctx->stream2));
-        HIPCHK(hipMemsetAsync(ctx->col_zeros.p, 0, (size_t)ncols * 4, ctx->stream3));
+        HIPCHK(op_fill(ctx, d_hist, 0, (size_t)intervals * 4, ctx->stream2));
+        HIPCHK(op_fill(ctx, ctx->col_zeros.p, 0, (size_t)ncols * 4, ctx->stream3));
         const unsigned tag = (ctx->epoch & 0xfffu) << 20;
         bool sweep_over = false;
         int b0_done = 0;
@@ -573,31 +579,28 @@
                 const int64_t h_lo = hist_first, h_hi = b0_hi >= G.g0.num ? (int64_t)n : ((int64_t)rows_need * G.d0) / 8 * 8;
                 hist_first = h_hi;
                 const int grid = (int)std::min<int64_t>(((h_hi - h_lo) / 8 + 255) / 256 + 1, 2048);
-                if (h_hi > h_lo) hipLaunchKernelGGL(k_hist_u16, dim3(grid), dim3(256), hist_lds, ctx->stream2, (const uint16_t *)d_nat, h_hi, intervals, rshift, use_lds, d_hist, h_lo);
+                if (h_hi > h_lo) OP_LAUNCH_K(k_hist_u16, dim3(grid), dim3(256), hist_lds, ctx->stream2, (const uint16_t *)d_nat, h_hi, intervals, rshift, use_lds, d_hist, h_lo);
                 if (!P.segenc) launch_permute(ctx->stream3, b0_done * G.g1.num, (b0_hi - b0_done) * G.g1.num);
                 HIPCHK(hipGetLastError());
                 b0_done = b0_hi;
             }
         }
-        HIPCHK(hipMemcpyAsync(h_hist, d_hist, (size_t)intervals * 4, hipMemcpyDeviceToHost, ctx->stream2));
+        HIPCHK(op_copy(ctx, h_hist, d_hist, (size_t)intervals * 4, hipMemcpyDeviceToHost, ctx->stream2));
         HIPCHK(hipEventRecord(ctx->ev_fit, ctx->stream2));
         if (!P.segenc) TRY(scan_col_zeros(ctx->stream3));
         HIPCHK(hipEventRecord(ctx->ev_perm, ctx->stream3));
         return SZHIP_OK;
     }
     int hist_and_order() {
-        TRY(ensure(ctx, ctx->hist, (size_t)(65536 + 8192) * 4 + 64));
-        d_hist = (unsigned *)ctx->hist.p;
         TRY(ensure_pinned(ctx, (size_t)intervals * 4 + 64));
         h_hist = (unsigned *)ctx->pinned;
         if (P.seghist) {
             TRY(ensure(ctx, ctx->seg_hist, (size_t)ncols * intervals * 4));
-            HIPCHK(hipMemsetAsync(d_hist, 0, (size_t)intervals * 4, st));
-            hipLaunchKernelGGL(k_col_hist, dim3((unsigned)ncols), dim3(256), ((size_t)intervals * 4) << P.sh_rshift, st, G, (const uint16_t *)d_nat, intervals, P.sh_rshift, P.se_vw, (unsigned *)ctx->seg_hist.p);
-            hipLaunchKernelGGL(k_hist_reduce, dim3((unsigned)std::min<int64_t>(64, ncols)), dim3(256), 0, st, (const unsigned *)ctx->seg_hist.p, intervals, (int64_t)ncols, d_hist);
+            OP_LAUNCH_K(k_col_hist, dim3((unsigned)ncols), dim3(256), ((size_t)intervals * 4) << P.sh_rshift, st, G, (const uint16_t *)d_nat, intervals, P.sh_rshift, P.se_vw, (unsigned *)ctx->seg_hist.p);
+            OP_LAUNCH_K(k_hist_reduce, dim3((unsigned)std::min<int64_t>(64, ncols)), dim3(256), 0, st, (const unsigned *)ctx->seg_hist.p, intervals, (int64_t)ncols, d_hist);
             HIPCHK(hipGetLastError());
             if (!P.dev_book) {
-                HIPCHK(hipMemcpyAsync(h_hist, d_hist, (size_t)intervals * 4, hipMemcpyDeviceToHost, st));
+                HIPCHK(op_copy(ctx, h_hist, d_hist, (size_t)intervals * 4, hipMemcpyDeviceToHost, st));
                 HIPCHK(hipEventRecord(ctx->ev_fit, st));
             }
         } else if (!P.sliced) TRY(launch_hist());
@@ -616,10 +619,15 @@
         return q + sizeof(T);
     }
     int upload_segments() {
-        se_segs.resize((size_t)P.se_nseg);
-        for (int q = 0; q < P.se_nseg; ++q) se_segs[(size_t)q] = szh_se::make_seg(G, 1, q, P.se_segb, P.se_vw);
-        TRY(ensure(ctx, ctx->seg_tab, se_segs.size() * sizeof(szh_se::seg_t)));
-        HIPCHK(hipMemcpyAsync(ctx->seg_tab.p, se_segs.data(), se_segs.size() * sizeof(szh_se::seg_t), hipMemcpyHostToDevice, st));
+        const size_t bytes = (size_t)P.se_nseg * sizeof(szh_se::seg_t);
+        TRY(ensure(ctx, ctx->seg_tab, bytes));
+        const unsigned long long key[4] = {(unsigned long long)G.g2.count, (unsigned long long)P.se_segb, (unsigned long long)P.se_vw, (unsigned long long)P.se_nseg};
+        if (ctx->seg_key_buf == ctx->seg_tab.p && memcmp(key, ctx->seg_key, sizeof(key)) == 0) return SZHIP_OK;
+        TRY(ensure_host(ctx, ctx->seg_pin, ctx->seg_pin_cap, bytes, st));
+        szh_se::seg_t *const segs = (szh_se::seg_t *)ctx->seg_pin;
+        for (int q = 0; q < P.se_nseg; ++q) segs[q] = szh_se::make_seg(G, 1, q, P.se_segb, P.se_vw);
+        HIPCHK(op_copy(ctx, ctx->seg_tab.p, segs, bytes, hipMemcpyHostToDevice, st));
+        memcpy(ctx->seg_key, key, sizeof(key)); ctx->seg_key_buf = ctx->seg_tab.p;
         return SZHIP_OK;
     }
     template <class F>
@@ -629,21 +637,21 @@
         TRY(ensure(ctx, ctx->seg_bitoff, (size_t)nent * 8)); TRY(ensure(ctx, ctx->seg_zoff, (size_t)nent * 8));
         u64 *const bits = (u64 *)ctx->seg_bits.p, *const zeros = (u64 *)ctx->seg_zeros.p, *const bitoff = (u64 *)ctx->seg_bitoff.p, *const zoff = (u64 *)ctx->seg_zoff.p;
         const size_t lb = intervals <= 16384 ? (size_t)intervals : 16;
-        if (P.seghist) hipLaunchKernelGGL(k_col_bits_h, dim3((unsigned)((nent + 255) / 256)), dim3(256), 0, st, (const unsigned *)ctx->seg_hist.p, (const uint8_t *)ctx->len_tab.p, intervals, nent, bits, zeros);
-        else hipLaunchKernelGGL(k_col_bits, dim3((unsigned)nent), dim3(256), lb, st, G, (const uint16_t *)d_nat, (const uint8_t *)ctx->len_tab.p, intervals, P.se_vw, bits, zeros);
+        if (P.seghist) OP_LAUNCH_K(k_col_bits_h, dim3((unsigned)((nent + 255) / 256)), dim3(256), 0, st, (const unsigned *)ctx->seg_hist.p, d_len, intervals, nent, bits, zeros);
+        else OP_LAUNCH_K(k_col_bits, dim3((unsigned)nent), dim3(256), lb, st, G, (const uint16_t *)d_nat, d_len, intervals, P.se_vw, bits, zeros);
         if (nent <= 1024 * SZH_COL_SCAN_PER && tune_int("SZ_HIP_SEG_SCAN1", 1))
-            hipLaunchKernelGGL(k_col_scan, dim3(1), dim3(1024), 0, st, (const u64 *)bits, (const u64 *)zeros, (int)nent, bitoff, zoff, sm + SM_TOTAL_BITS, sm + SM_TOTAL_UNPRED, base_bits, (unsigned *)d_stream, d_plan);
+            OP_LAUNCH_K(k_col_scan, dim3(1), dim3(1024), 0, st, (const u64 *)bits, (const u64 *)zeros, (int)nent, bitoff, zoff, sm + SM_TOTAL_BITS, sm + SM_TOTAL_UNPRED, base_bits, (unsigned *)d_stream, d_plan);
         else {
             TRY(scan_u64(ctx, (const u64 *)bits, nent, bitoff, sm + SM_TOTAL_BITS));
             TRY(scan_u64(ctx, (const u64 *)zeros, nent, zoff, sm + SM_TOTAL_UNPRED));
-            hipLaunchKernelGGL(k_col_bounds, dim3((unsigned)((nent + 1 + 255) / 256)), dim3(256), 0, st, (const u64 *)bitoff, nent, (const u64 *)(sm + SM_TOTAL_BITS), base_bits, (unsigned *)d_stream);
+            OP_LAUNCH_K(k_col_bounds, dim3((unsigned)((nent + 1 + 255) / 256)), dim3(256), 0, st, (const u64 *)bitoff, nent, (const u64 *)(sm + SM_TOTAL_BITS), base_bits, (unsigned *)d_stream);
         }
         HIPCHK(hipGetLastError());
         TRY(between());
         const unsigned win = (unsigned)szh_se::seg_window_words(G, std::max(1u, maxlen), P.se_nrmax);
         const size_t lds = ((size_t)intervals + 1) * 8 + P.se_tile + 16 + (size_t)win * 4;
         auto encode = [&](auto kernel) {
-            hipLaunchKernelGGL(kernel, dim3((unsigned)nent), dim3(256), lds, st, G, (const uint16_t *)d_nat, (const u64 *)ctx->code_tab.p, intervals, (const szh_se::seg_t *)ctx->seg_tab.p, P.se_nseg, P.se_vw,
+            OP_LAUNCH_K(kernel, dim3((unsigned)nent), dim3(256), lds, st, G, (const uint16_t *)d_nat, d_code, intervals, (const szh_se::seg_t *)ctx->seg_tab.p, P.se_nseg, P.se_vw,
                                P.se_nrmax, P.se_tile, win, (const u64 *)bitoff, (const u64 *)zoff, base_bits, (unsigned *)d_stream, d_in, (T *)ctx->unpred.p, d_plan);
         };
         if (G.g2.num >= 2 && G.g2.early <= szh_se::INNER && G.g2.late >= szh_se::INNER - 1) encode(k_col_encode<T, true>);
@@ -654,16 +662,16 @@
     int enqueue_readback() {
         HIPCHK(hipEventRecord(ctx->ev[4], st));
         TP("encode launched");
-        HIPCHK(hipMemcpyAsync(h_small, sm, SM_COUNT * 8, hipMemcpyDeviceToHost, st));
+        HIPCHK(op_copy(ctx, ctx->words_pin, sm, SM_COUNT * 8, hipMemcpyDeviceToHost, st));
         return SZHIP_OK;
     }
     int deliver(unsigned char *d_stream, size_t len, bool in_place) {
         if (out_on_device == 2) {
             if (!*out || *out_size < len) FAIL(SZHIP_ERR_ARG, "caller's device buffer too small (%zu < %zu)", *out_size, len);
-            if (!in_place) { HIPCHK(hipMemcpyAsync(*out, d_stream, len, hipMemcpyDeviceToDevice, st)); synced = false; }
-            if (!synced) HIPCHK(hipStreamSynchronize(st));
+            if (!in_place) { HIPCHK(op_copy(ctx, *out, d_stream, len, hipMemcpyDeviceToDevice, st)); synced = false; }
+            if (!synced) HIPCHK(op_sync(ctx, st));
         } else if (out_on_device) {
-            if (!synced) HIPCHK(hipStreamSynchronize(st));
+            if (!synced) HIPCHK(op_sync(ctx, st));
             *out = d_stream;
         } else {
             unsigned char *h = (unsigned char *)malloc(len ? len : 1);
@@ -677,6 +685,7 @@
         return SZHIP_OK;
     }
     int check_final(bool declined, unsigned book_status, u64 bits, u64 unpred) {
+        memcpy(h_small, ctx->words_pin, sizeof(h_small));
         if ((unsigned)h_small[SM_ERR] == 2) { ctx->coef_late = true; FAIL(SZHIP_ERR_INTERNAL, "wavefront kernel: the regression coefficients did not arrive"); }
         if ((unsigned)h_small[SM_ERR] != 0) { ctx->wave_timeout = true; FAIL(SZHIP_ERR_INTERNAL, "wavefront kernel: halo wait timed out"); }
         if (declined) {
@@ -712,24 +721,25 @@
         unsigned char *d_stream = in_place ? (unsigned char *)*out : (unsigned char *)ctx->stream_buf.p;
         TRY(ensure(ctx, ctx->book_stage, bk_front + bk_mid)); TRY(ensure(ctx, ctx->book_tree, tree_cap)); TRY(ensure(ctx, ctx->book_rec, 32 + SZH_PLAN_COUNT * 8));
         TRY(ensure(ctx, ctx->code_tab, (size_t)intervals * 8)); TRY(ensure(ctx, ctx->len_tab, (size_t)intervals));
+        d_code = (const u64 *)ctx->code_tab.p; d_len = (const uint8_t *)ctx->len_tab.p;
         TRY(ensure(ctx, ctx->unpred, unpred_cap + 64));
         szh_book_rec *const d_rec = (szh_book_rec *)ctx->book_rec.p;
         u64 *const d_plan = (u64 *)((char *)ctx->book_rec.p + 32);
-        HIPCHK(hipMemcpyAsync(ctx->book_stage.p, blob, bk_front + bk_mid, hipMemcpyHostToDevice, st));
-        hipLaunchKernelGGL(k_huff_book, dim3(1), dim3(256), 0, st, (const unsigned *)d_hist, intervals, SZH_BOOK_TAB_SEG, (unsigned char *)ctx->book_tree.p, (unsigned)tree_cap,
+        HIPCHK(op_copy(ctx, ctx->book_stage.p, blob, bk_front + bk_mid, hipMemcpyHostToDevice, st));
+        OP_LAUNCH_K(k_huff_book, dim3(1), dim3(256), 0, st, (const unsigned *)d_hist, intervals, SZH_BOOK_TAB_SEG, (unsigned char *)ctx->book_tree.p, (unsigned)tree_cap,
                            (u64 *)ctx->code_tab.p, (uint8_t *)ctx->len_tab.p, d_rec, d_plan, (u64)plan_fixed, (unsigned)sizeof(T), (u64)stream_cap, (u64)unpred_cap);
         HIPCHK(hipGetLastError());
         TRY(upload_segments());
         TRY(pack_columns(d_stream, 0, (const u64 *)d_plan, 32u, [&]() -> int {
-            hipLaunchKernelGGL(k_book_tail, dim3((unsigned)std::min<size_t>(64, (plan_fixed + tree_cap + 255) / 256)), dim3(256), 0, st, d_stream, (const unsigned char *)ctx->book_stage.p, (unsigned)bk_front,
-                               (unsigned)bk_mid, intervals, (const unsigned char *)ctx->lor_bits.p, ind_bytes, (const unsigned char *)ctx->book_tree.p, (const szh_book_rec *)d_rec, (const u64 *)d_plan);
+            OP_LAUNCH_K(k_book_tail, dim3((unsigned)std::min<size_t>(64, (plan_fixed + tree_cap + 255) / 256)), dim3(256), 0, st, d_stream, (const unsigned char *)ctx->book_stage.p, (unsigned)bk_front,
+                               (unsigned)bk_mid, intervals, (const unsigned char *)d_ind, ind_bytes, (const unsigned char *)ctx->book_tree.p, (const szh_book_rec *)d_rec, (const u64 *)d_plan);
             return SZHIP_OK;
         }));
-        hipLaunchKernelGGL((k_book_unpred<T>), dim3((unsigned)std::min<size_t>(256, (unpred_cap / sizeof(T) + 255) / 256)), dim3(256), 0, st, d_stream, (const T *)ctx->unpred.p, (const szh_book_rec *)d_rec, (const u64 *)d_plan);
+        OP_LAUNCH_K((k_book_unpred<T>), dim3((unsigned)std::min<size_t>(256, (unpred_cap / sizeof(T) + 255) / 256)), dim3(256), 0, st, d_stream, (const T *)ctx->unpred.p, (const szh_book_rec *)d_rec, (const u64 *)d_plan);
         HIPCHK(hipGetLastError());
         TRY(enqueue_readback());
-        HIPCHK(hipMemcpyAsync(ctx->book_pin, ctx->book_rec.p, 32 + SZH_PLAN_COUNT * 8, hipMemcpyDeviceToHost, st));
-        HIPCHK(hipStreamSynchronize(st));
+        HIPCHK(op_copy(ctx, ctx->book_pin, ctx->book_rec.p, 32 + SZH_PLAN_COUNT * 8, hipMemcpyDeviceToHost, st));
+        HIPCHK(op_sync(ctx, st));
         synced = true;
         TP("final sync");
         szh_book_rec rec; memcpy(&rec, ctx->book_pin, sizeof(rec));
@@ -744,7 +754,7 @@
     }
     int build_host_book() {
         TP("permute launched");
-        HIPCHK(hipEventSynchronize(ctx->ev_fit));
+        HIPCHK(op_esync(ctx, ctx->ev_fit));
         TP("hist on host");
         double h0 = now_ms();
         szhost_huff *hf = szhost_huff_build(2 * (int)intervals, h_hist, nullptr, intervals);
@@ -774,7 +784,9 @@
         memcpy(q, &mean, sizeof(T)); q += sizeof(T);
         memcpy(q, ind_bits, ind_bytes); q += ind_bytes;
         const uint64_t tu = total_unpred; memcpy(q, &tu, 8);
-        tab_code.resize(intervals); tab_len.resize(intervals);
+        const size_t code_bytes = (size_t)intervals * 8;
+        { const int rc = ensure_host(ctx, ctx->tab_pin, ctx->tab_pin_cap, code_bytes + intervals + 64, st); if (rc != SZHIP_OK) { szhost_huff_free(hf); return rc; } }
+        tab_code = (u64 *)ctx->tab_pin; tab_len = (uint8_t *)ctx->tab_pin + code_bytes;
         for (unsigned s = 0; s < intervals; ++s) { tab_code[s] = hf->code[s]; tab_len[s] = hf->len[s]; }
         total_bits = hf->total_bits;
         szhost_huff_free(hf);
@@ -789,21 +801,23 @@
         if (P.segenc) for (unsigned s = 0; s < intervals; ++s) tab_code[s] = (tab_code[s] << 32) | tab_len[s] | (s == 0 ? 0x10000u : 0u);
         else if (enc32) for (unsigned s = 0; s < intervals; ++s) tab_code[s] = (tab_code[s] << 8) | tab_len[s];
         host_ms += now_ms() - h0;
-        TRY(ensure(ctx, ctx->code_tab, (size_t)intervals * 8));
-        TRY(ensure(ctx, ctx->len_tab, (size_t)intervals));
-        HIPCHK(hipMemcpyAsync(ctx->code_tab.p, tab_code.data(), (size_t)intervals * 8, hipMemcpyHostToDevice, st));
-        HIPCHK(hipMemcpyAsync(ctx->len_tab.p, tab_len.data(), (size_t)intervals, hipMemcpyHostToDevice, st));
+        TRY(ensure(ctx, ctx->tabs, code_bytes + intervals + 64));
+        d_code = (const u64 *)ctx->tabs.p; d_len = (const uint8_t *)ctx->tabs.p + code_bytes;
+        HIPCHK(op_copy(ctx, ctx->tabs.p, ctx->tab_pin, code_bytes + intervals, hipMemcpyHostToDevice, st));
         return SZHIP_OK;
     }
     int copy_header(unsigned char *d_stream) {
-        HIPCHK(hipMemcpyAsync(d_stream, hdr, pre_len, hipMemcpyHostToDevice, st));
-        HIPCHK(hipMemcpyAsync(d_stream + pre_len + sections_total, hdr + pre_len, 8, hipMemcpyHostToDevice, st));
+        if (!sections_total) HIPCHK(op_copy(ctx, d_stream, hdr, pre_len + 8, hipMemcpyHostToDevice, st));
+        else {
+            HIPCHK(op_copy(ctx, d_stream, hdr, pre_len, hipMemcpyHostToDevice, st));
+            HIPCHK(op_copy(ctx, d_stream + pre_len + sections_total, hdr + pre_len, 8, hipMemcpyHostToDevice, st));
+        }
         if (sections_total) {
             const hipStream_t ssec = ctx->stream3 ? ctx->stream3 : ctx->stream2;
             HIPCHK(hipEventRecord(ctx->ev_feed, st));
             HIPCHK(hipStreamWaitEvent(ssec, ctx->ev_feed, 0));
             size_t off = pre_len;
-            for (int e = 0; e < ncoef; ++e) { HIPCHK(hipMemcpyAsync(d_stream + off, ctx->sec_pin[e], sec_len[e], hipMemcpyHostToDevice, ssec)); off += sec_len[e]; }
+            for (int e = 0; e < ncoef; ++e) { HIPCHK(op_copy(ctx, d_stream + off, ctx->sec_pin[e], sec_len[e], hipMemcpyHostToDevice, ssec)); off += sec_len[e]; }
             HIPCHK(hipEventRecord(ctx->ev_sec, ssec));
         }
         return SZHIP_OK;
@@ -815,7 +829,7 @@
             TRY(ensure(ctx, ctx->unpred, unpred_bytes));
             HIPCHK(hipEventRecord(ctx->ev_in, st));
             HIPCHK(hipStreamWaitEvent(ctx->stream2, ctx->ev_in, 0));
-            hipLaunchKernelGGL((k_unpred<T, 0>), dim3(ncols), dim3(256), 0, ctx->stream2, G, (const uint16_t *)d_blk, (const unsigned *)ctx->col_zeros.p,
+            OP_LAUNCH_K((k_unpred<T, 0>), dim3(ncols), dim3(256), 0, ctx->stream2, G, (const uint16_t *)d_blk, (const unsigned *)ctx->col_zeros.p,
                                (const u64 *)ctx->col_off.p, d_in, (T *)ctx->unpred.p, (T *)nullptr, (const unsigned *)ctx->zcnt.p, (const unsigned *)ctx->zpos.p, perm_segb, perm_nseg);
             HIPCHK(hipGetLastError());
             HIPCHK(hipEventRecord(ctx->ev_fit, ctx->stream2));
@@ -824,15 +838,15 @@
             const int64_t nchunks = (n + SZH_ENC_CHUNK - 1) / SZH_ENC_CHUNK;
             TRY(ensure(ctx, ctx->chunk_bits, (size_t)nchunks * 8 + 64));
             TRY(ensure(ctx, ctx->chunk_off, (size_t)nchunks * 8));
-            hipLaunchKernelGGL(k_chunk_bits, dim3((unsigned)((nchunks + SZH_CB_PER - 1) / SZH_CB_PER)), dim3(256), 0, st, (const uint16_t *)d_blk, n, (const uint8_t *)ctx->len_tab.p, intervals, (u64 *)ctx->chunk_bits.p);
+            OP_LAUNCH_K(k_chunk_bits, dim3((unsigned)((nchunks + SZH_CB_PER - 1) / SZH_CB_PER)), dim3(256), 0, st, (const uint16_t *)d_blk, n, d_len, intervals, (u64 *)ctx->chunk_bits.p);
             TRY(scan_u64(ctx, (const u64 *)ctx->chunk_bits.p, nchunks, (u64 *)ctx->chunk_off.p, sm + SM_TOTAL_BITS));
             if (enc32) {
                 const int64_t nrounds = (n + SZH_E32_ROUND - 1) / SZH_E32_ROUND;
-                hipLaunchKernelGGL(k_encode32, dim3((unsigned)((nrounds + SZH_E32_PER - 1) / SZH_E32_PER)), dim3(256), lds_e32, st, (const uint16_t *)d_blk, n, (const u64 *)ctx->code_tab.p,
+                OP_LAUNCH_K(k_encode32, dim3((unsigned)((nrounds + SZH_E32_PER - 1) / SZH_E32_PER)), dim3(256), lds_e32, st, (const uint16_t *)d_blk, n, d_code,
                                    intervals, (const u64 *)ctx->chunk_off.p, base_bits, (unsigned *)d_stream);
             } else
-                hipLaunchKernelGGL(k_encode, dim3((unsigned)((nchunks + SZH_ENC_PER - 1) / SZH_ENC_PER)), dim3(256), 0, st, (const uint16_t *)d_blk, n, (const u64 *)ctx->code_tab.p,
-                                   (const uint8_t *)ctx->len_tab.p, intervals, (const u64 *)ctx->chunk_off.p, base_bits, (unsigned *)d_stream);
+                OP_LAUNCH_K(k_encode, dim3((unsigned)((nchunks + SZH_ENC_PER - 1) / SZH_ENC_PER)), dim3(256), 0, st, (const uint16_t *)d_blk, n, d_code,
+                                   d_len, intervals, (const u64 *)ctx->chunk_off.p, base_bits, (unsigned *)d_stream);
             HIPCHK(hipGetLastError());
         }
         if (total_unpred > 0) HIPCHK(hipStreamWaitEvent(st, ctx->ev_fit, 0));
@@ -849,11 +863,11 @@
                 return ensure(ctx, ctx->unpred, unpred_bytes + 64);
             }));
         } else {
-            HIPCHK(hipMemsetAsync(d_stream, 0, total_len + 64, st));
+            HIPCHK(op_fill(ctx, d_stream, 0, total_len + 64, st));
             TRY(copy_header(d_stream));
             TRY(pack_block_ordered(d_stream));
         }
-        if (total_unpred > 0) HIPCHK(hipMemcpyAsync(d_stream + hdr_len, ctx->unpred.p, unpred_bytes, hipMemcpyDeviceToDevice, st));
+        if (total_unpred > 0) HIPCHK(op_copy(ctx, d_stream + hdr_len, ctx->unpred.p, unpred_bytes, hipMemcpyDeviceToDevice, st));
         if (sections_total) HIPCHK(hipStreamWaitEvent(st, ctx->ev_sec, 0));
         TRY(enqueue_readback());
         TRY(deliver(d_stream, total_len, in_place));
@@ -874,6 +888,7 @@
 int compress_impl(szhip_ctx *ctx, const void *data, int data_on_device, size_t r0, size_t r1, size_t r2, double eb_in, const szhip_params *prm, const unsigned char *meta, size_t meta_len, int out_on_device,
                   unsigned char **out, size_t *out_size, szhip_stats *stats)
 {
+    for (unsigned &o : ctx->ops) o = 0;
     sz21_call<T> c(ctx, r0, r1, r2, eb_in, prm, meta, meta_len, out_on_device, out, out_size);
     int rc = c.stage_and_fit(data, data_on_device);
     if (rc == SZHIP_OK) rc = c.choose_intervals();
@@ -1202,6 +1217,7 @@
         up_segs.resize((size_t)up_nseg);
         for (int q = 0; q < up_nseg; ++q) up_segs[(size_t)q] = szh_se::make_seg(G, 1, q, up_segb, up_vw);
         TRY(ensure(ctx, ctx->seg_tab, up_segs.size() * sizeof(szh_se::seg_t)));
+        ctx->seg_key_buf = nullptr;
         HIPCHK(hipMemcpyAsync(ctx->seg_tab.p, up_segs.data(), up_segs.size() * sizeof(szh_se::seg_t), hipMemcpyHostToDevice, st));
     } else
     {
```

Measured after the change: 390.4 (median of 6 runs). 2.7% higher.
